# zhazorken/beom

Measured on AMD Instinct MI355X. Metric: cell-layer updates/s, higher is better.
Workload: dtype f64

## Files before the change

### beom_amd/csrc/beom_dev.h

```cpp
#pragma once
#include <hip/hip_runtime.h>
#include <stdint.h>

#include "../../include/beom_hip.h"

struct DevView {
    int ndeg, nlay, lm, mm, nsal, variant;
    int mm_glob;
    long long n1;
    int L, M, xper, yper;
    int P;
    long long ncell;
    int embedded;
    const int32_t *pk_of;
    const unsigned char *reg4;
    int reg_nx;
    const unsigned char *ngt;
    int ngt_nx;
    int joff, Mg, slab;
    int nstrip, jlo0, jhi0, jlo1, jhi1;
    const int32_t *neig, *subc;
    const double *mk_u, *mk_v, *mk_n, *mkpe, *mkpi, *fcor, *h_th, *h_to;
    const double *nudg, *fnud, *hdot, *tide, *bodf, *taus;
    double *hlay, *u, *v, *h_u, *h_v;
    double *rs[2];
    double *dmx[4], *dmy[4];
    double *u_alt, *v_alt, *hu_alt, *hv_alt;
    double *v_cc, *v_ll, *tt3d, *tb3d, *tu3d;
    double *mont, *rvor, *pvor, *dive, *d2hx, *d2hy;
    double *pcd, *qlr;
    int keep_diag;
    int keep_visc;
    int zero_visc;
    int lean_d2h;
    double *delu, *delv, *uu4, *vv4; double svis;
    const int32_t *woff;
    const int32_t *segm; int nseg;
    double *pi_s, *pi_rhs, *pi_prev;
    const double *Ow, *Os, *Osum_;
    const int32_t *sor_order, *sor_dstart;
    const int32_t *lid_rhs_start, *lid_rhs_ent;
    int sor_ndiag;
    double dl, dt, grav, rho0, beta, epsi, gamm, del1, del2, hmin, hsal, bvis, dvis, bdrg, tdrg,
        qdrg, hsbl, hbbl, uadv, ocrp, rgld, invf, w_ti;
    double rhon[BEOM_MAX_LAYERS];
    double i_dl, i_gr, i_ns, i_r0, i_r1, i_rn[BEOM_MAX_LAYERS];
    int has_hdot, has_tide, has_bodf, has_nudg, has_stress, has_wind, has_hto;
    int vel_targets_zero;
    const double *fnud_vel;
    int stress_fold, has_bot, has_top;
    const double *taus_cells;
    double rho_top, rho_bot;
    double *mo0, *mo1, *mo2;
};

struct TileMap {
    int tr0a, ntra, tr0b, ntrb, total, gx, rpx, tpx, nt, xlast, nlast, rim_first, by_tiles;
    __host__ __device__ __forceinline__ TileMap(const DevView &d, int TX, int TY) {
        gx = (d.L + TX - 1) / TX;
        tr0a = 0; ntra = 0; tr0b = 0; ntrb = 0;
        if (d.jhi0 >= d.jlo0) { tr0a = (d.jlo0 - 1) / TY; ntra = (d.jhi0 - 1) / TY - tr0a + 1; }
        if (d.nstrip > 1 && d.jhi1 >= d.jlo1) { tr0b = (d.jlo1 - 1) / TY; ntrb = (d.jhi1 - 1) / TY - tr0b + 1; }
        total = ntra + ntrb;
        nt = total * gx;
        rpx = (total + 7) / 8;
        rim_first = nt <= 4096;
        by_tiles = !rim_first && (rpx * 8 - total) * 100 > 3 * total;
        tpx = by_tiles ? (nt + 7) / 8 : rpx * gx;
        xlast = total > 0 ? (total - 1) / rpx : 0;
        nlast = total - xlast * rpx;
    }
    __host__ unsigned blocks() const { return (unsigned)(8 * tpx); }
    __device__ __forceinline__ bool locate(int b, int &ty, int &ch) const {
        const int xcd = b & 7, k = b >> 3;
        int vt;
        if (by_tiles) {
            const int v = xcd * tpx + k;
            if (v >= nt) return false;
            vt = v / gx; ch = v - vt * gx;
        } else {
            int rib = k / gx;
            const int c = k - rib * gx;
            ch = c;
            if (rim_first) {
                ch = c == 0 ? 0 : (c == 1 ? gx - 1 : c - 1);
                if (xcd == xlast && rib < nlast) rib = nlast - 1 - rib;
            }
            vt = xcd * rpx + rib;
            if (rib >= rpx || vt >= total) return false;
        }
        ty = vt < ntra ? tr0a + vt : tr0b + (vt - ntra);
        return true;
    }
};
__host__ __device__ __forceinline__ bool row_selected(const DevView &d, int j) {
    return (j >= d.jlo0 && j <= d.jhi0) || (d.nstrip > 1 && j >= d.jlo1 && j <= d.jhi1);
}
__device__ __forceinline__ bool tile_regular(const DevView &d, int x0, int y0, int ny) {
    if (!d.embedded) return true;
    const int tx = (x0 - 1) >> 6, t4 = (y0 - 1) >> 2;
    if (tx < 0 || tx >= d.reg_nx || t4 < 0 || (t4 + (ny >> 2) - 1) * 4 >= d.M) return false;
    bool r = d.reg4[(long long)t4 * d.reg_nx + tx] != 0;
    if (ny > 4) r = r && d.reg4[(long long)(t4 + 1) * d.reg_nx + tx] != 0;
    return r;
}
__device__ __forceinline__ bool slot_is_cell(const DevView &d, int ip) { return !d.embedded || d.pk_of[ip] != 0; }

__device__ __forceinline__ bool cell_slot(const DevView &d, long long ip) {
    if (ip > d.ncell) return false;
    if (d.P == 0 || ip == 0) return true;
    if (d.embedded) return d.pk_of[ip] != 0;
    return (int)((ip - 1) % d.P) < d.L;
}
__device__ __forceinline__ long long packed_index0(const DevView &d, long long ip) {
    if (d.P == 0) return ip - 1;
    if (d.embedded) return (long long)d.pk_of[ip] - 1;
    const long long r = (ip - 1) / d.P;
    return r * d.L + ((ip - 1) - r * d.P);
}

#define BEOM_BLOCK 256

template <int K> struct NbOff {
    static constexpr int di = (K == 1 || K == 2 || K == 8) ? 1 : ((K == 4 || K == 5 || K == 6) ? -1 : 0);
    static constexpr int dj = (K == 2 || K == 3 || K == 4) ? 1 : ((K == 6 || K == 7 || K == 8) ? -1 : 0);
};

struct CellPackedInt {
    static constexpr bool kLanesAreRowNeighbours = true;
    static constexpr bool kHasIJ = false;
    int ipnt, dN, dS;
    const DevView *dv;
    template <int K> __device__ __forceinline__ int nb() const {
        constexpr int di = NbOff<K>::di, dj = NbOff<K>::dj;
        return ipnt + di + (dj > 0 ? dN : (dj < 0 ? -dS : 0));
    }
// ... 134 lines not shown
```

### beom_amd/csrc/beom_engine.hip

```cpp
#include <hip/hip_runtime.h>

#include <cmath>
#include <cstdarg>
#include <cstdio>
#include <cstdlib>
#include <cstring>
#include <algorithm>
#include <string>
#include <type_traits>
#include <utility>
#include <vector>

#include "beom_dev.h"
#include "beom_kernels.h"
#include "beom_integrals.h"
#include "beom_series.h"
#include "beom_tracers.h"
#include "beom_tracers_lim.h"
#include "beom_floats.h"
#include "beom_moments.h"
#include "beom_tracer_moments.h"
#include "beom_dense_host.h"
#include "beom_plan.h"

// ... 39 lines not shown
        hipEvent_t a; (void)hipEventCreate(&a); (void)hipEventRecord(a, st); ev.push_back(a); cls.push_back(c);
    }
    void end() { if (!open) return; hipEvent_t b; (void)hipEventCreate(&b); (void)hipEventRecord(b, st); ev.push_back(b); open = false; }
};

struct AccumKind {
    int n1, n2, nsq;
    bool per_tracer;
    const char *bad_args, *no_tracer, *none, *no_sq;
};
constexpr AccumKind kFieldMoments{3, 5, 5, false,
    "beom_set_moments: level %d, stride %d (level 0..3, stride >= 1)", nullptr,
    "beom_download_moments: the handle keeps no moments (beom_set_moments)",
    "beom_download_moments: the second moments are kept at level 3, this handle has level %d"};
constexpr AccumKind kTracerMoments{2, 4, 1, true,
    "beom_set_tracer_moments: level %d, stride %d (level 0..3, stride >= 1)",
    "beom_set_tracer_moments: the handle carries no tracer (beom_set_tracers comes first)",
    "beom_download_tracer_moments: the handle keeps no tracer moments (beom_set_tracer_moments)",
    "beom_download_tracer_moments: the second moment is kept at level 3, this handle has level %d"};
struct Accum {
    const AccumKind *kind;
    int level = 0, stride = 1;
    long long count = 0, launches = 0;
    int first = 0, last = 0;
    double *ref[5] = {}, *sum[5] = {}, *sq[5] = {};
    std::vector<void *> allocs;
};
static bool accum_due(const Accum &A, int tstp) { return A.level > 0 && tstp % A.stride == 0; }
static void accum_note_sample(Accum &A, int tstp) {
    if (A.count == 0) A.first = tstp;
    A.last = tstp;
    ++A.count;
    ++A.launches;
}

struct beom_engine {
    beom_params P;
    int device = 0;
    hipStream_t stream = nullptr;
    hipStream_t own_stream = nullptr;
    StepTimer *timer = nullptr;
    DevView d{};
    bool dense = false;
    std::vector<void *> allocs;
    const int32_t *slot_of_dev = nullptr;
    bool embedded = false;
    void *stage = nullptr;
    size_t stage_bytes = 0;
    dim3 grid_cells0, grid_cells_layers_flat;
    bool wind = false, bot = false, top = false;
    bool fold_stress = true, fold_static_ok = false;
    bool up_tt = false, up_tb = false, up_tu = false;
    bool last_folded = false;
    bool last_uv_fused = false;
    float *h0r4_dev = nullptr, *out4[3] = {nullptr, nullptr, nullptr};
    float *diag4[3] = {nullptr, nullptr, nullptr};
    double *scan_dev = nullptr;
    int any_u = 0, any_v = 0;
    long long uniform_waves = 0, total_waves = 0;
    bool obc = false;
    bool obc_set = false;
    bool fuse = true;
    bool fuse_uv = true;
    bool lean_visc = true;
    bool visc_all_zero = true;
    bool lean_d2h = true;
    std::vector<int32_t> subc_host, neig_host, dev_index;
    bool lid = false, lid_ready = false;
    int lid_dstep = 2, lid_nring = 0, lid_maxwidth = 1;
    double *lid_ring = nullptr;
    unsigned long long *lid_maxd = nullptr;
    long long lid_sweeps = 0, lid_solves = 0, lid_launches = 0;
    int lid_last = 0;
    int profile_stride = 1;
    bool profile_rotate = false;
    StepPlan split{};
    bool tile4 = false;
    bool mont_history = true;
    bool mont_keep = false;
    int mont_levels_valid = 0;
    bool hist_stale = false;
    bool last_mont_hist = false;
    bool plain_sweeps = true;
    int last_plain = 0;
    double *integ_part = nullptr, *integ_rows = nullptr;
    int integ_count = 0;
    int32_t *integ_cellmap = nullptr;
    int integ_xper = 0, integ_yper = 0;
    int ntrc = 0;
    int trc_scheme = 1;
    double *trc_q = nullptr, *trc_q_alt = nullptr, *trc_rq[2] = {nullptr, nullptr}, *trc_ctrg = nullptr;
    std::vector<void *> trc_allocs;
    long long nflt = 0;
    bool flt_ready = false;
    double *flt_x = nullptr, *flt_y = nullptr, *flt_k1x = nullptr, *flt_k1y = nullptr, *flt_xs = nullptr, *flt_ys = nullptr;
    int32_t *flt_layer = nullptr, *flt_rej = nullptr;
    unsigned long long *flt_first_dry = nullptr;
    double *flt_rec = nullptr;
    int flt_nrec = 0, flt_stride = 1;
    std::vector<int> flt_rec_tstp;
    long long flt_launches = 0;
    bool cellmap_known = false;
    std::vector<void *> flt_allocs;
    bool flt_band = false;
    FloatBand flt_fb{};
    unsigned long long *flt_in_s = nullptr, *flt_in_n = nullptr;
    int flt_xper = 0, flt_yper = 0;
    double flt_fmm = 0.0;
    long long flt_handovers = 0;
    Accum mom{&kFieldMoments};
    bool mom_by_caller = false;
    int last_tstp = 0;
    Accum tmom{&kTracerMoments};
    int ser_level = 0, ser_stride = 1, ser_nrec = 0, ser_jlo = 1, ser_rows = 0;
    bool ser_by_caller = false;
    double *ser_rec = nullptr;
    std::vector<int> ser_tstp;
    std::vector<void *> ser_allocs;
    char last_err[512] = {0};
};
static int hist_sync(beom_engine *E);
static int leave_mont_history(beom_engine *E);

namespace {

template <class T>
int alloc_plain(beom_engine *E, std::vector<void *> &owner, T **p, size_t n, char *errm, int errm_len, bool zero = true) {
    void *q = nullptr;
    HIP_TRY(hipMalloc(&q, n * sizeof(T)));
    owner.push_back(q);
    if (zero) HIP_TRY(hipMemsetAsync(q, 0, n * sizeof(T), E->stream));
    *p = (T *)q;
    return 0;
}
constexpr size_t kLead = 15;
template <class T>
int alloc_aligned(beom_engine *E, std::vector<void *> &owner, T **p, size_t n, char *errm, int errm_len, bool zero = true) {
    const int rc = alloc_plain(E, owner, p, n + kLead + 1, errm, errm_len, zero);
    if (!rc) *p += kLead;
    return rc;
}
void free_list(std::vector<void *> &owner) {
    for (void *p : owner) (void)hipFree(p);
    owner.clear();
}
template <class T>
int dev_alloc(beom_engine *E, T **p, size_t n, char *errm, int errm_len, bool zero = true) {
    return sizeof(T) == 8 ? alloc_aligned(E, E->allocs, p, n, errm, errm_len, zero) : alloc_plain(E, E->allocs, p, n + 1, errm, errm_len, zero);
}
size_t state_cells(const beom_engine *E) { return (size_t)E->d.nlay * (size_t)E->d.n1; }
size_t tracer_cells(const beom_engine *E) { return (size_t)E->ntrc * state_cells(E); }

template <class T, bool REMAP = false>
int slice_to_device(beom_engine *E, T *dev, const T *host, int inner, int K, int m, char *errm, int errm_len) {
    const DevView &d = E->d;
    const size_t n = ((size_t)d.ndeg + 1) * inner * K;
    if (n * sizeof(T) > E->stage_bytes) { set_err(errm, errm_len, "internal: staging buffer too small"); return -11; }
    if (host) HIP_TRY(hipMemcpyAsync(E->stage, host, n * sizeof(T), hipMemcpyHostToDevice, E->stream));
    const long long work = ((long long)d.ndeg + 1) * inner;
    if (E->embedded) {
        const long long all = (d.ncell + 1) * inner;
        hipLaunchKernelGGL((k_fill_sentinel<T>), dim3((unsigned)((all + BEOM_BLOCK - 1) / BEOM_BLOCK)), dim3(BEOM_BLOCK), 0, E->stream,
                           dev, (const T *)E->stage, d.ncell + 1, inner, K, m);
    }
    hipLaunchKernelGGL((k_repack<T, true, REMAP>), dim3((unsigned)((work + BEOM_BLOCK - 1) / BEOM_BLOCK)), dim3(BEOM_BLOCK), 0, E->stream,
                       dev, (T *)E->stage, (long long)d.ndeg, d.L, d.P ? d.P : d.L, inner, K, m, E->slot_of_dev);
    return 0;
}
template <class T>
int slice_to_host(beom_engine *E, const T *dev, T *host, int inner, int K, char *errm, int errm_len) {
    (void)dev;
    const DevView &d = E->d;
    const size_t n = ((size_t)d.ndeg + 1) * inner * K;
    HIP_TRY(hipMemcpyAsync(host, E->stage, n * sizeof(T), hipMemcpyDeviceToHost, E->stream));
    HIP_TRY(hipStreamSynchronize(E->stream));
    return 0;
}
template <class T>
void slice_gather(beom_engine *E, const T *dev, int inner, int K, int m) {
    const DevView &d = E->d;
    const long long work = ((long long)d.ndeg + 1) * inner;
    hipLaunchKernelGGL((k_repack<T, false, false>), dim3((unsigned)((work + BEOM_BLOCK - 1) / BEOM_BLOCK)), dim3(BEOM_BLOCK), 0, E->stream,
                       const_cast<T *>(dev), (T *)E->stage, (long long)d.ndeg, d.L, d.P ? d.P : d.L, inner, K, m, E->slot_of_dev);
}

template <class T, bool REMAP = false>
int dev_upload(beom_engine *E, const T **dst, const T *src, size_t outer, int inner, char *errm, int errm_len) {
    const DevView &d = E->d;
    T *q = nullptr;
    int rc = dev_alloc(E, &q, outer * (size_t)d.n1 * inner, errm, errm_len, true);
    if (rc) return rc;
    const size_t n1h = (size_t)d.ndeg + 1;
    if (src)
        for (size_t o = 0; o < outer; ++o)
            if ((rc = slice_to_device<T, REMAP>(E, q + o * (size_t)d.n1 * inner, src + o * n1h * inner, inner, 1, 0, errm, errm_len))) return rc;
    *dst = q;
    return 0;
}

bool any_nonzero(const double *a, size_t n) {
    if (!a) return false;
    for (size_t i = 0; i < n; ++i)
        if (a[i] != 0.0) return true;
    return false;
}

int check_create_args(const beom_params *prm, const beom_handle *out, int device, const beom_dense::Grid &g,
                      const beom_statics &st, char *errm, int errm_len) {
    if (!prm || !out) { set_err(errm, errm_len, "beom_create: null argument"); return -1; }
    if (prm->abi_version != BEOM_ABI_VERSION) { set_err(errm, errm_len, "beom_create: ABI version mismatch (%d vs %d)", prm->abi_version, BEOM_ABI_VERSION); return -2; }
    if (prm->nlay < 1 || prm->nlay > BEOM_MAX_LAYERS || prm->ndeg < 1 || prm->lm < 1 || prm->mm < 1) { set_err(errm, errm_len, "beom_create: bad sizes"); return -3; }
    if (prm->rgld > 0.5 && (prm->variant == 1 || prm->slab_mm > 0 || prm->ocrp < 0.5)) {
        set_err(errm, errm_len, "beom_create: rgld = 1 (rigid lid, private_mod.f95:1705-1838) needs variant 0, ocrp = 1 and a whole frame (no bands)");
        return -5;
    }
    if (prm->variant == 1 && prm->nlay < 3) { set_err(errm, errm_len, "beom_create: variant 1 (private_mod3d.f95) needs nlay >= 3"); return -7; }
    if (!g.neig || !g.subc || !g.mk_u || !g.mk_v || !g.mk_n || !g.mkpe || !g.mkpi || !st.fcor || !st.h_th || !st.nudg || !st.fnud) { set_err(errm, errm_len, "beom_create: null static array"); return -1; }
    int ndev = 0;
    HIP_TRY(hipGetDeviceCount(&ndev));
    if (ndev <= 0 || device < 0 || device >= ndev) { set_err(errm, errm_len, "beom_create: no usable HIP device (%d visible, asked for %d); there is no CPU fallback", ndev, device); return -8; }
    HIP_TRY(hipSetDevice(device));
    if (prm->slab_mm > 0 && (prm->slab_row0 < 0 || prm->slab_row0 + prm->mm + 1 > prm->slab_mm + 1)) { set_err(errm, errm_len, "beom_create: slab rows outside the global frame"); return -3; }
    return 0;
}

void fill_view(DevView &d, const beom_params &prm, const beom_statics &st) {
    const size_t n1h = (size_t)prm.ndeg + 1, nl = (size_t)prm.nlay;
    d.ndeg = prm.ndeg; d.nlay = prm.nlay; d.lm = prm.lm; d.mm = prm.mm; d.nsal = prm.nsal;
    d.variant = prm.variant; d.n1 = (long long)n1h; d.ncell = prm.ndeg;
    d.L = prm.lm + 1; d.M = prm.mm + 1;
    d.dl = prm.dl; d.dt = prm.dt; d.grav = prm.grav; d.rho0 = prm.rho0; d.beta = prm.beta;
    d.epsi = prm.epsi; d.gamm = prm.gamm; d.del1 = prm.del1; d.del2 = prm.del2; d.hmin = prm.hmin;
    d.hsal = prm.hsal; d.bvis = prm.bvis; d.dvis = prm.dvis; d.bdrg = prm.bdrg; d.tdrg = prm.tdrg;
    d.qdrg = prm.qdrg; d.hsbl = prm.hsbl; d.hbbl = prm.hbbl; d.uadv = prm.uadv; d.ocrp = prm.ocrp;
    d.rgld = prm.rgld; d.invf = prm.invf; d.w_ti = prm.w_ti; d.svis = prm.svis;
    d.mm_glob = prm.slab_mm > 0 ? prm.slab_mm : prm.mm;
    for (int i = 0; i < BEOM_MAX_LAYERS; ++i) d.rhon[i] = prm.rhon[i];
    d.i_dl = 1.0 / prm.dl;
    d.i_gr = 1.0 / prm.grav;
    d.i_ns = 1.0 / (double)(prm.nsal - 1);
    d.i_r0 = 1.0 / prm.rho0;
    d.i_r1 = 1.0 / prm.rhon[0];
    for (int i = 0; i < prm.nlay; ++i) d.i_rn[i] = 1.0 / prm.rhon[i];
    d.nstrip = 1; d.jlo0 = 1; d.jhi0 = d.M; d.jlo1 = 1; d.jhi1 = 0;
    d.slab = prm.slab_mm > 0 ? 1 : 0;
    d.joff = d.slab ? prm.slab_row0 : 0;
    d.Mg = d.slab ? prm.slab_mm + 1 : d.M;
    d.has_hdot = any_nonzero(st.hdot, nl * n1h);
    d.has_tide = any_nonzero(st.tide, 6 * n1h);
    d.has_bodf = any_nonzero(st.bodf, 2 * nl);
    d.has_nudg = any_nonzero(st.nudg, 3 * n1h);
    d.has_hto = any_nonzero(st.h_to, n1h);
    d.vel_targets_zero = beom_dense::vel_targets_zero(st.fnud, n1h, nl);
    d.rho_top = prm.rhon[0]; d.rho_bot = prm.rhon[nl - 1];
}

void choose_paths(beom_engine *E, const beom_dense::Grid &g, const beom_statics &st) {
    const beom_params &prm = E->P;
    DevView &d = E->d;
    const size_t n1h = (size_t)prm.ndeg + 1, nl = (size_t)prm.nlay;
    for (size_t i = 0; i < n1h; ++i) { if (g.mk_u[i] > 0.5) E->any_u = 1; if (g.mk_v[i] > 0.5) E->any_v = 1; }
    E->tile4 = E->dense && (long long)((d.L + 63) / 64) * ((d.M + 7) / 8) <= 5000;
    if (getenv("BEOM_TILE4")) E->tile4 = E->dense && atoi(getenv("BEOM_TILE4")) != 0;
    if (E->lid) E->fuse = E->fuse_uv = false;
    if (st.taus) for (size_t i = 0; i < 2 * n1h; ++i) if (std::fabs(st.taus[i]) > 1.e-7) { E->wind = true; break; }
    E->bot = prm.bdrg > 1.e-7;
    E->top = prm.tdrg > 1.e-7;
    d.has_wind = E->wind; d.has_bot = E->bot; d.has_top = E->top;
    d.has_stress = E->wind || E->bot || E->top;
    bool neg0 = false;
    if (st.bodf) for (size_t i = 0; i < 2 * nl; ++i) if (st.bodf[i] == 0.0 && std::signbit(st.bodf[i])) neg0 = true;
    E->fold_static_ok = E->dense && prm.ocrp < 0.5 && !E->lid && d.has_stress && !neg0;
}

template <class T>
int upload_table(beom_engine *E, const T **dst, const std::vector<T> &v, size_t n, bool zero, char *errm, int errm_len) {
    T *q = nullptr;
    const int rc = dev_alloc(E, &q, n, errm, errm_len, zero);
    if (rc) return rc;
    HIP_TRY(hipMemcpyAsync(q, v.data(), v.size() * sizeof(T), hipMemcpyHostToDevice, E->stream));
    HIP_TRY(hipStreamSynchronize(E->stream));
    *dst = q;
    return 0;
}

int upload_statics(beom_engine *E, const beom_dense::Layout &lay, const beom_dense::WaveTable &wt,
                   const std::vector<unsigned char> &ngt, const beom_dense::Grid &g, const beom_statics &st,
                   char *errm, int errm_len) {
    DevView &d = E->d;
    const size_t n1h = (size_t)d.ndeg + 1, nl = (size_t)d.nlay;
    E->stage_bytes = n1h * 32;
    HIP_TRY(hipMalloc(&E->stage, E->stage_bytes));
    int rc;
    if (E->embedded) {
        if ((rc = upload_table(E, &E->slot_of_dev, lay.slot_of, lay.slot_of.size(), false, errm, errm_len))) return rc;
        if ((rc = upload_table(E, &d.pk_of, lay.pk_of, (size_t)d.n1, true, errm, errm_len))) return rc;
        if ((rc = upload_table(E, &d.reg4, lay.reg4, lay.reg4.size(), false, errm, errm_len))) return rc;
    }
    if ((rc = dev_upload<int32_t, true>(E, &d.neig, g.neig, 1, 8, errm, errm_len))) return rc;
    if ((rc = dev_upload(E, &d.subc, g.subc, 2, 1, errm, errm_len))) return rc;
    auto up = [&](const double **dst, const double *src, size_t outer, int inner = 1) {
        if (!rc) rc = dev_upload(E, dst, src, outer, inner, errm, errm_len);
    };
    up(&d.mk_u, g.mk_u, 1); up(&d.mk_v, g.mk_v, 1); up(&d.mk_n, g.mk_n, 1); up(&d.mkpe, g.mkpe, 1); up(&d.mkpi, g.mkpi, 1);
    up(&d.fcor, st.fcor, 1); up(&d.h_th, st.h_th, 1); up(&d.h_to, st.h_to, 1);
    up(&d.nudg, st.nudg, 3); up(&d.fnud, st.fnud, 3 * nl); up(&d.hdot, st.hdot, nl);
    up(&d.tide, st.tide, 3, 2); up(&d.taus, st.taus, 2);
    d.fnud_vel = (rc || d.vel_targets_zero) ? nullptr : d.fnud + d.n1 * (long long)d.nlay;
    std::vector<double> tc(2 * n1h, 0.0);
    if (st.taus) { std::memcpy(tc.data(), st.taus, 2 * n1h * sizeof(double)); tc[0] = 0.0; tc[n1h] = 0.0; }
    up(&d.taus_cells, tc.data(), 2);
    if (rc) return rc;
    double *q = nullptr;
    if ((rc = dev_alloc(E, &q, 2 * nl, errm, errm_len, true))) return rc;
    if (st.bodf) HIP_TRY(hipMemcpyAsync(q, st.bodf, 2 * nl * sizeof(double), hipMemcpyHostToDevice, E->stream));
    d.bodf = q;
    if (wt.uniform > 0 && (rc = upload_table(E, &d.woff, wt.woff, wt.woff.size(), false, errm, errm_len))) return rc;
    if (!ngt.empty()) {
        if ((rc = upload_table(E, &d.ngt, ngt, ngt.size(), false, errm, errm_len))) return rc;
        d.ngt_nx = (d.L + 63) / 64;
    }
    return 0;
}

int alloc_state(beom_engine *E, char *errm, int errm_len) {
    DevView &d = E->d;
    const size_t n = (size_t)d.nlay * (size_t)d.n1;
    int rc = 0;
    auto al = [&](std::initializer_list<double **> arrays, size_t len) {
        for (double **a : arrays) if (!rc) rc = dev_alloc(E, a, len, errm, errm_len);
    };
    al({&d.hlay, &d.u, &d.v, &d.h_u, &d.h_v, &d.rs[0], &d.rs[1], &d.dmx[0], &d.dmx[1], &d.dmx[2], &d.dmy[0], &d.dmy[1], &d.dmy[2]}, n);
    if (E->dense) al({&d.dmx[3], &d.dmy[3], &d.u_alt, &d.v_alt, &d.hu_alt, &d.hv_alt}, n);
    al({&d.v_cc, &d.v_ll}, n);
    al({&d.tt3d, &d.tb3d, &d.tu3d}, 2 * n);
    al({&d.pcd, &d.qlr, &d.mont, &d.rvor, &d.pvor, &d.dive, &d.d2hx, &d.d2hy}, n);
    E->mont_keep = E->dense && !E->lid && !d.slab && E->P.g_fb != 0.0 && d.nlay <= 8 && !(E->P.svis > 0.0);
    if (E->mont_keep) al({&d.mo0, &d.mo1, &d.mo2}, n);
    if (E->P.svis > 0.0) al({&d.delu, &d.delv, &d.uu4, &d.vv4}, n);
    if (E->lid) al({&d.pi_s, &d.pi_rhs, &d.pi_prev}, (size_t)d.n1);
    if (rc) return rc;
    if (E->P.bvis != 0.0) {
        std::vector<double> b(n, E->P.bvis);
        HIP_TRY(hipMemcpyAsync(d.v_cc, b.data(), b.size() * sizeof(double), hipMemcpyHostToDevice, E->stream));
        HIP_TRY(hipMemcpyAsync(d.v_ll, b.data(), b.size() * sizeof(double), hipMemcpyHostToDevice, E->stream));
        HIP_TRY(hipStreamSynchronize(E->stream));
    }
    return 0;
}

int setup(beom_engine *E, const beom_dense::Grid &g, const beom_statics &st, char *errm, int errm_len) {
    const beom_params &prm = E->P;
    DevView &d = E->d;
    HIP_TRY(hipStreamCreateWithFlags(&E->own_stream, hipStreamNonBlocking));
    E->stream = E->own_stream;
    fill_view(d, prm, st);
    beom_dense::Layout lay = beom_dense::plan_layout(prm, d.L, d.M, d.joff, d.Mg, d.slab, g);
    E->dense = lay.dense; E->embedded = lay.embedded;
    d.xper = lay.xper; d.yper = lay.yper; d.embedded = lay.embedded ? 1 : 0; d.reg_nx = lay.reg_nx;
    E->dev_index = std::move(lay.dev_index);
    E->lid = prm.rgld > 0.5;
    if (E->lid) {
        const size_t n1h = (size_t)prm.ndeg + 1;
        E->subc_host.assign(g.subc, g.subc + 2 * n1h);
        E->neig_host.assign(g.neig, g.neig + 8 * n1h);
    }
    if (E->dense) {
        d.P = lay.P;
        d.ncell = (long long)d.P * d.M;
        d.n1 = (d.ncell + 1 + 15) / 16 * 16;
    }
    beom_dense::WaveTable wt;
    if (!E->dense) wt = beom_dense::plan_wave_table(prm.ndeg, g);
    E->uniform_waves = wt.uniform; E->total_waves = wt.total;
    const std::vector<unsigned char> ngt = E->dense && d.has_nudg ? beom_dense::plan_nudging_tiles(lay, d.L, d.M, prm.ndeg, st.nudg)
                                                                  : std::vector<unsigned char>();
    int rc;
    if ((rc = upload_statics(E, lay, wt, ngt, g, st, errm, errm_len))) return rc;
    choose_paths(E, g, st);
    if ((rc = alloc_state(E, errm, errm_len))) return rc;
    const unsigned gx = (unsigned)((d.ncell + BEOM_BLOCK - 1) / BEOM_BLOCK);
    const unsigned gx0 = (unsigned)((d.ncell + 1 + BEOM_BLOCK - 1) / BEOM_BLOCK);
    E->grid_cells_layers_flat = dim3(gx, (unsigned)prm.nlay, 1);
    E->grid_cells0 = dim3(gx0, 1, 1);
    HIP_TRY(hipStreamSynchronize(E->stream));
    return 0;
}

}

extern "C" {

int beom_abi_version(void) { return BEOM_ABI_VERSION; }

int beom_device_count(char *errm, int errm_len) {
    int n = 0;
    HIP_TRY(hipGetDeviceCount(&n));
    return n;
}

int beom_device_pci_bus_id(int device, char *out, int out_len) {
    if (!out || out_len < 16) return -1;
    return hipDeviceGetPCIBusId(out, out_len, device) == hipSuccess ? 0 : -9;
}

int beom_create(const beom_params *prm, int device, const int32_t *neig, const int32_t *subc,
                const double *mk_u, const double *mk_v, const double *mk_n, const double *mkpe,
                const double *mkpi, const double *fcor, const double *h_th, const double *h_to,
                const double *nudg, const double *fnud, const double *hdot, const double *tide,
                const double *bodf, const double *taus, beom_handle *out, char *errm, int errm_len) {
    const beom_dense::Grid g{neig, subc, mk_u, mk_v, mk_n, mkpe, mkpi};
    const beom_statics st{fcor, h_th, h_to, nudg, fnud, hdot, tide, bodf, taus};
    int rc = check_create_args(prm, out, device, g, st, errm, errm_len);
    if (rc) return rc;
    beom_engine *E = new beom_engine();
    E->P = *prm;
    E->device = device;
    if ((rc = setup(E, g, st, errm, errm_len))) {
        beom_destroy(E);
        return rc;
    }
    *out = E;
    return 0;
}

int beom_destroy(beom_handle E) {
    if (!E) return 0;
    (void)hipSetDevice(E->device);
    if (E->stream) (void)hipStreamSynchronize(E->stream);
    for (std::vector<void *> *l : {&E->allocs, &E->trc_allocs, &E->flt_allocs, &E->mom.allocs, &E->tmom.allocs, &E->ser_allocs}) free_list(*l);
    if (E->stage) (void)hipFree(E->stage);
    if (E->timer) { for (hipEvent_t ev : E->timer->ev) (void)hipEventDestroy(ev); delete E->timer; }
    if (E->own_stream) (void)hipStreamDestroy(E->own_stream);
    delete E;
    return 0;
}

static int copy_in(beom_engine *E, double *dst, const double *src, size_t outer, char *errm, int errm_len) {
    if (!src) return 0;
    const size_t n1h = (size_t)E->d.ndeg + 1;
    for (size_t o = 0; o < outer; ++o) {
        const int rc = slice_to_device<double>(E, dst + o * (size_t)E->d.n1, src + o * n1h, 1, 1, 0, errm, errm_len);
        if (rc) return rc;
    }
    return 0;
}
static int copy_out(beom_engine *E, double *dst, const double *src, size_t outer, char *errm, int errm_len) {
    if (!dst) return 0;
    const size_t n1h = (size_t)E->d.ndeg + 1;
    for (size_t o = 0; o < outer; ++o) {
        slice_gather<double>(E, src + o * (size_t)E->d.n1, 1, 1, 0);
        const int rc = slice_to_host<double>(E, src, dst + o * n1h, 1, 1, errm, errm_len);
        if (rc) return rc;
    }
    return 0;
}

static int hist_in(beom_engine *E, double *const *dev, int K, const double *src, char *errm, int errm_len, int outer = 0) {
    if (!src) return 0;
    const size_t n1h = (size_t)E->d.ndeg + 1;
    if (!outer) outer = E->d.nlay;
    for (int l = 0; l < outer; ++l)
        for (int m = 0; m < K; ++m) {
            const int rc = slice_to_device<double>(E, dev[m] + (size_t)l * E->d.n1, m == 0 ? src + (size_t)l * n1h * K : nullptr, 1, K, m,
                                                   errm, errm_len);
            if (rc) return rc;
        }
    return 0;
}
static int hist_out(beom_engine *E, double *const *dev, int K, double *dst, char *errm, int errm_len, int outer = 0) {
    if (!dst) return 0;
    const size_t n1h = (size_t)E->d.ndeg + 1;
    if (!outer) outer = E->d.nlay;
    for (int l = 0; l < outer; ++l) {
        for (int m = 0; m < K; ++m) slice_gather<double>(E, dev[m] + (size_t)l * E->d.n1, 1, K, m);
        const int rc = slice_to_host<double>(E, dev[0], dst + (size_t)l * n1h * K, 1, K, errm, errm_len);
        if (rc) return rc;
    }
    return 0;
}

int beom_upload_state(beom_handle E, const double *hlay, const double *u, const double *v,
                      const double *h_u, const double *h_v, const double *rs_h, const double *dmdx,
                      const double *dmdy, const double *v_cc, const double *v_ll, const double *tt3d,
                      const double *tb3d, const double *tu3d, char *errm, int errm_len) {
    if (!E) { set_err(errm, errm_len, "null handle"); return -1; }
    HIP_TRY(hipSetDevice(E->device));
    DevView &d = E->d;
    const size_t nl = (size_t)d.nlay, n = ((size_t)d.ndeg + 1) * nl;
    int rc;
    if ((rc = leave_mont_history(E))) { set_err(errm, errm_len, "beom_upload_state: the history arrays could not be brought up to date"); return rc; }
    if ((rc = copy_in(E, d.hlay, hlay, nl, errm, errm_len))) return rc;
    if ((rc = copy_in(E, d.u, u, nl, errm, errm_len))) return rc;
    if ((rc = copy_in(E, d.v, v, nl, errm, errm_len))) return rc;
    if ((rc = copy_in(E, d.h_u, h_u, nl, errm, errm_len))) return rc;
    if ((rc = copy_in(E, d.h_v, h_v, nl, errm, errm_len))) return rc;
    if ((rc = copy_in(E, d.v_cc, v_cc, nl, errm, errm_len))) return rc;
    if ((rc = copy_in(E, d.v_ll, v_ll, nl, errm, errm_len))) return rc;
    if ((rc = copy_in(E, d.tt3d, tt3d, 2 * nl, errm, errm_len))) return rc;
    if ((rc = copy_in(E, d.tb3d, tb3d, 2 * nl, errm, errm_len))) return rc;
    if ((rc = copy_in(E, d.tu3d, tu3d, 2 * nl, errm, errm_len))) return rc;
    if ((rc = hist_in(E, d.rs, 2, rs_h, errm, errm_len))) return rc;
    if ((rc = hist_in(E, d.dmx, 3, dmdx, errm, errm_len))) return rc;
    if ((rc = hist_in(E, d.dmy, 3, dmdy, errm, errm_len))) return rc;
    if (any_nonzero(tt3d, 2 * n)) E->up_tt = true;
    if (any_nonzero(tb3d, 2 * n)) E->up_tb = true;
    if (any_nonzero(tu3d, 2 * n)) E->up_tu = true;
    if (E->up_tt || E->up_tb || E->up_tu) d.has_stress = 1;
    for (const double *a : {v_cc, v_ll})
        if (a) for (size_t i = 0; i < n && E->visc_all_zero; ++i) { uint64_t b; memcpy(&b, &a[i], 8); if (b != 0) E->visc_all_zero = false; }
    HIP_TRY(hipStreamSynchronize(E->stream));
    HIP_TRY(hipGetLastError());
    return 0;
}

int beom_download_state(beom_handle E, double *hlay, double *u, double *v, double *h_u, double *h_v,
                        double *rs_h, double *dmdx, double *dmdy, double *v_cc, double *v_ll,
                        double *tt3d, double *tb3d, double *tu3d, char *errm, int errm_len) {
    if (!E) { set_err(errm, errm_len, "null handle"); return -1; }
    HIP_TRY(hipSetDevice(E->device));
    DevView &d = E->d;
    const size_t nl = (size_t)d.nlay;
    int rc;
    if ((rc = hist_sync(E))) { set_err(errm, errm_len, "beom_download_state: the history arrays could not be brought up to date"); return rc; }
    if ((rc = copy_out(E, hlay, d.hlay, nl, errm, errm_len))) return rc;
    if ((rc = copy_out(E, u, d.u, nl, errm, errm_len))) return rc;
    if ((rc = copy_out(E, v, d.v, nl, errm, errm_len))) return rc;
    if ((rc = copy_out(E, h_u, d.h_u, nl, errm, errm_len))) return rc;
    if ((rc = copy_out(E, h_v, d.h_v, nl, errm, errm_len))) return rc;
    if ((rc = copy_out(E, v_cc, d.v_cc, nl, errm, errm_len))) return rc;
    if ((rc = copy_out(E, v_ll, d.v_ll, nl, errm, errm_len))) return rc;
    if ((rc = copy_out(E, tt3d, d.tt3d, 2 * nl, errm, errm_len))) return rc;
    if ((rc = copy_out(E, tb3d, d.tb3d, 2 * nl, errm, errm_len))) return rc;
    if ((rc = copy_out(E, tu3d, d.tu3d, 2 * nl, errm, errm_len))) return rc;
    if ((rc = hist_out(E, d.rs, 2, rs_h, errm, errm_len))) return rc;
    if ((rc = hist_out(E, d.dmx, 3, dmdx, errm, errm_len))) return rc;
    if ((rc = hist_out(E, d.dmy, 3, dmdy, errm, errm_len))) return rc;
    HIP_TRY(hipStreamSynchronize(E->stream));
    HIP_TRY(hipGetLastError());
    return 0;
}

int beom_download_scratch(beom_handle E, double *mont, double *rvor, double *pvor, double *dive,
                          double *d2hx, double *d2hy, char *errm, int errm_len) {
    if (!E) { set_err(errm, errm_len, "null handle"); return -1; }
    HIP_TRY(hipSetDevice(E->device));
    DevView &d = E->d;
    const size_t nl = (size_t)d.nlay;
    int rc;
    if ((rc = copy_out(E, mont, d.mont, nl, errm, errm_len))) return rc;
    if ((rc = copy_out(E, rvor, d.rvor, nl, errm, errm_len))) return rc;
    if ((rc = copy_out(E, pvor, d.pvor, nl, errm, errm_len))) return rc;
    if ((rc = copy_out(E, dive, d.dive, nl, errm, errm_len))) return rc;
    if ((rc = copy_out(E, d2hx, d.d2hx, nl, errm, errm_len))) return rc;
    if ((rc = copy_out(E, d2hy, d.d2hy, nl, errm, errm_len))) return rc;
    HIP_TRY(hipStreamSynchronize(E->stream));
    return 0;
}

int beom_set_rigid_lid(beom_handle E, const double *Ow, const double *Os, const double *Osum_, const double *pi_s,
                       char *errm, int errm_len) {
    if (!E) { set_err(errm, errm_len, "null handle"); return -1; }
    if (!E->lid) { set_err(errm, errm_len, "beom_set_rigid_lid: the handle was created with rgld = 0"); return -5; }
    HIP_TRY(hipSetDevice(E->device));
    DevView &d = E->d;
    int rc;
    if (!E->lid_ready) {
        if (!Ow || !Os || !Osum_) { set_err(errm, errm_len, "beom_set_rigid_lid: the operators Ow, Os, Osum_ are needed on the first call"); return -1; }
        if ((long long)d.n1 >= (1ll << 29)) { set_err(errm, errm_len, "beom_set_rigid_lid: frame too large for the lid's tables"); return -3; }
        const beom_dense::LidPlan lp = beom_dense::plan_lid(d.ndeg, d.lm, d.mm_glob, d.n1, E->subc_host, E->neig_host, E->dev_index);
        if ((rc = dev_upload(E, &d.Ow, Ow, 1, 1, errm, errm_len))) return rc;
        if ((rc = dev_upload(E, &d.Os, Os, 1, 1, errm, errm_len))) return rc;
        if ((rc = dev_upload(E, &d.Osum_, Osum_, 1, 1, errm, errm_len))) return rc;
        if ((rc = upload_table(E, &d.sor_order, lp.order, lp.order.size(), false, errm, errm_len))) return rc;
        if ((rc = upload_table(E, &d.sor_dstart, lp.start, lp.start.size(), false, errm, errm_len))) return rc;
        d.sor_ndiag = (int)lp.start.size() - 1;
        E->lid_dstep = lp.dstep;
        E->lid_maxwidth = lp.maxwidth;
        E->lid_nring = (int)std::max<long long>(17, std::min<long long>(kLidBatch, (6ll << 30) / ((long long)d.n1 * 8))) + 1;
        if ((rc = dev_alloc(E, &E->lid_ring, (size_t)E->lid_nring * d.n1, errm, errm_len, true))) return rc;
        if ((rc = dev_alloc(E, &E->lid_maxd, (size_t)kLidBatch, errm, errm_len, true))) return rc;
        if ((rc = upload_table(E, &d.lid_rhs_start, lp.rhs_start, lp.rhs_start.size(), false, errm, errm_len))) return rc;
        if ((rc = upload_table(E, &d.lid_rhs_ent, lp.rhs_ent, lp.rhs_ent.size(), false, errm, errm_len))) return rc;
        E->lid_ready = true;
    }
    if (pi_s && (rc = slice_to_device<double>(E, d.pi_s, pi_s, 1, 1, 0, errm, errm_len))) return rc;
    HIP_TRY(hipStreamSynchronize(E->stream));
    HIP_TRY(hipGetLastError());
    return 0;
}

int beom_download_pressure(beom_handle E, double *pi_s, char *errm, int errm_len) {
    if (!E) { set_err(errm, errm_len, "null handle"); return -1; }
    if (!E->lid) { set_err(errm, errm_len, "beom_download_pressure: the handle was created with rgld = 0"); return -5; }
    HIP_TRY(hipSetDevice(E->device));
    const int rc = copy_out(E, pi_s, E->d.pi_s, 1, errm, errm_len);
    if (rc) return rc;
    HIP_TRY(hipGetLastError());
    return 0;
}

int beom_sync(beom_handle E, char *errm, int errm_len) {
    if (!E) { set_err(errm, errm_len, "null handle"); return -1; }
    HIP_TRY(hipSetDevice(E->device));
    HIP_TRY(hipStreamSynchronize(E->stream));
    HIP_TRY(hipGetLastError());
    return 0;
}

}

static inline void rot2(double *(&a)[2]) { double *t = a[0]; a[0] = a[1]; a[1] = t; }
static inline void rot3(double *(&a)[4]) { double *t = a[0]; a[0] = a[1]; a[1] = a[2]; a[2] = t; }
static inline void rot4(double *(&a)[4]) { double *t = a[0]; a[0] = a[1]; a[1] = a[2]; a[2] = a[3]; a[3] = t; }
static inline void swp(double *&a, double *&b) { double *t = a; a = b; b = t; }

static void rotate_mont(beom_engine *E) {
    if (!E->mont_keep) return;
    DevView &d = E->d;
    double *t = d.mo0; d.mo0 = d.mo1; d.mo1 = d.mo2; d.mo2 = d.mont; d.mont = t;
}
static int hist_sync(beom_engine *E) {
    if (!E->hist_stale) return 0;
    if (hipSetDevice(E->device) != hipSuccess) return -9;
    hipLaunchKernelGGL(k_hist_from_mont, CellDense::grid(E->d, E->d.nlay), dim3(BEOM_BLOCK), 0, E->stream, E->d);
    E->hist_stale = false;
    return hipGetLastError() == hipSuccess ? 0 : -10;
}
static int leave_mont_history(beom_engine *E) {
    const int rc = hist_sync(E);
    E->mont_levels_valid = 0;
    return rc;
}

#define LAUNCH_CTX(KERNEL_G, KERNEL_D, nz, ...)                                                            \
    do {                                                                                                  \
        if (E->dense) hipLaunchKernelGGL(KERNEL_D, CellDense::grid(E->d, (nz)), dim3(BEOM_BLOCK), 0, E->stream, __VA_ARGS__); \
        else hipLaunchKernelGGL(KERNEL_G, CellGather::grid(E->d, (nz)), dim3(BEOM_BLOCK), 0, E->stream, __VA_ARGS__);         \
    } while (0)

template <class F>
static void pick(F &&f) { f(); }
template <class F, class... R>
static void pick(F &&f, bool b, R... rest) {
    if (b) pick([&](auto... c) { f(std::true_type{}, c...); }, rest...);
    else pick([&](auto... c) { f(std::false_type{}, c...); }, rest...);
}
template <int FROM, int TO, class F>
static void pick_int(int v, F &&f) {
    if (FROM == TO || v == FROM) f(std::integral_constant<int, FROM>{});
    else if constexpr (FROM != TO) pick_int<FROM + (TO > FROM ? 1 : -1), TO>(v, f);
}

static void launch_rebuild(beom_engine *E) {
    LAUNCH_CTX(k_rebuild_fluxes<CellGather>, k_rebuild_fluxes<CellDense>, E->d.nlay, E->d);
}
static int forcing(const DevView &d) { return d.has_nudg ? (d.has_tide ? 2 : 1) : 0; }
static void launch_h(beom_engine *E, double gene, double ramp, double ctim, bool rotate = true) {
    int nz = (E->d.variant == 1) ? 1 : E->d.nlay;
    if (E->d.has_nudg) nz = 1;
    pick_int<2, 0>(forcing(E->d), [&](auto fo) { LAUNCH_CTX((k_update_h<CellGather, fo>), (k_update_h<CellDense, fo>), nz, E->d, gene, ramp, ctim, 0); });
    if (rotate) rot2(E->d.rs);
}
static void launch_tracers(beom_engine *E, double gene, double ramp, double ctim) {
    TrcView tv{E->ntrc, E->trc_ctrg ? 1 : 0, E->trc_q, E->trc_q_alt, E->trc_rq[0], E->trc_rq[1], E->trc_ctrg};
    const int nz = E->d.nlay;
    if (E->trc_scheme == 2) pick_int<2, 0>(forcing(E->d), [&](auto fo) {
        if (!E->dense) hipLaunchKernelGGL((k_tracers_lim<CellGather, fo>), CellGather::grid(E->d, nz), dim3(BEOM_BLOCK), 0, E->stream, E->d, tv, gene, ramp, ctim);
        else if (E->tile4) hipLaunchKernelGGL((k_tracers_lim<TrcTiled<1>, fo>), tracers_lim_grid<1>(E->d), dim3(BEOM_BLOCK), 0, E->stream, E->d, tv, gene, ramp, ctim);
        else hipLaunchKernelGGL((k_tracers_lim<TrcTiled<2>, fo>), tracers_lim_grid<2>(E->d), dim3(BEOM_BLOCK), 0, E->stream, E->d, tv, gene, ramp, ctim);
    });
    else pick_int<2, 0>(forcing(E->d), [&](auto fo) { LAUNCH_CTX((k_tracers<CellGather, fo>), (k_tracers<CellDense, fo>), nz, E->d, tv, gene, ramp, ctim); });
    swp(E->trc_q, E->trc_q_alt);
    rot2(E->trc_rq);
}
static FloatView float_view(const beom_engine *E, double *rec) {
    const DevView &d = E->d;
    return FloatView{E->nflt, E->flt_x, E->flt_y, E->flt_layer, E->flt_rej, E->flt_k1x, E->flt_k1y, E->flt_xs, E->flt_ys,
                     E->integ_cellmap, d.dt * d.i_dl, (double)d.lm, (double)d.mm, E->integ_xper, E->integ_yper, rec};
}
static void launch_floats(beom_engine *E, int mode, double *rec) {
    const DevView &d = E->d;
    FloatView f = float_view(E, rec);
    if (E->flt_band) {
        f.fmm = E->flt_fmm; f.xper = E->flt_xper; f.yper = E->flt_yper; f.cellmap = nullptr;
        const dim3 g((unsigned)((E->nflt + BEOM_BLOCK - 1) / BEOM_BLOCK)), b(BEOM_BLOCK);
        pick_int<1, 3>(mode, [&](auto m) { hipLaunchKernelGGL(k_floats_band<m>, g, b, 0, E->stream, d, f, E->flt_fb); });
        ++E->flt_launches;
        return;
    }
    const dim3 g((unsigned)((E->nflt + BEOM_BLOCK - 1) / BEOM_BLOCK)), b(BEOM_BLOCK);
    pick_int<1, 3>(mode, [&](auto m) {
        if (E->dense) hipLaunchKernelGGL((k_floats<CellDense, m>), g, b, 0, E->stream, d, f);
        else hipLaunchKernelGGL((k_floats<CellGather, m>), g, b, 0, E->stream, d, f);
    });
    ++E->flt_launches;
}
static void launch_floats_after(beom_engine *E, int tstp, bool then_stage1) {
    double *rec = nullptr;
    if (E->flt_nrec > 0 && tstp % E->flt_stride == 0 && (int)E->flt_rec_tstp.size() < E->flt_nrec) {
        rec = E->flt_rec + 3 * (size_t)E->nflt * E->flt_rec_tstp.size();
        E->flt_rec_tstp.push_back(tstp);
    }
    launch_floats(E, then_stage1 ? 3 : 2, rec);
}
static void launch_moments(beom_engine *E, int tstp) {
    const DevView &d = E->d;
    double *const *r = E->mom.ref, *const *s = E->mom.sum, *const *q = E->mom.sq;
    const MomentView m{(long long)d.nlay * d.n1, d.hlay, d.u, d.v, d.h_u, d.h_v, r[0], r[1], r[2], r[3], r[4],
                       s[0], s[1], s[2], s[3], s[4], q[0], q[1], q[2], q[3], q[4]};
    const long long pairs = (m.n - 1) / 2;
    const dim3 g((unsigned)std::max<long long>(1, std::min<long long>((pairs + BEOM_BLOCK - 1) / BEOM_BLOCK, 2048))), b(BEOM_BLOCK);
    pick_int<1, 3>(E->mom.level, [&](auto lv) {
        pick([&](auto first) { hipLaunchKernelGGL((k_moments<lv, first>), g, b, 0, E->stream, m); }, E->mom.count == 0);
    });
    accum_note_sample(E->mom, tstp);
}
static void launch_tracer_moments(beom_engine *E, int tstp) {
    double *const *r = E->tmom.ref, *const *s = E->tmom.sum;
    const TrcMomentView m{E->ntrc, E->trc_q, r[0], r[1], r[2], r[3], s[0], s[1], s[2], s[3], E->tmom.sq[0]};
    const int nz = E->d.nlay;
    pick_int<1, 3>(E->tmom.level, [&](auto lv) {
        pick([&](auto first) { LAUNCH_CTX((k_tracer_moments<CellGather, lv, first>), (k_tracer_moments<CellDense, lv, first>), nz, E->d, m); },
             E->tmom.count == 0);
    });
    accum_note_sample(E->tmom, tstp);
}
static bool series_due(const beom_engine *E, int tstp) {
    return E->ser_level > 0 && tstp % E->ser_stride == 0 && (int)E->ser_tstp.size() < E->ser_nrec;
}
static void launch_series(beom_engine *E, int tstp) {
    const DevView &d = E->d;
    const int count = (E->ser_level >= 2 ? 6 : 4) * d.nlay + 1, nch = (d.L + 63) / 64;
    int nchp2 = 1, width = 1;
    while (nchp2 < nch) nchp2 <<= 1;
    while (width < d.L && width < 64) width <<= 1;
    double *rec = E->ser_rec + E->ser_tstp.size() * (size_t)E->ser_rows * count;
    const dim3 g((unsigned)nch, (unsigned)((E->ser_rows + BEOM_TILE_Y - 1) / BEOM_TILE_Y), 1), b(BEOM_BLOCK);
    const int32_t *map = E->dense ? nullptr : E->integ_cellmap;
    auto go = [&](auto kern) { hipLaunchKernelGGL(kern, g, b, 0, E->stream, d, E->ser_jlo, E->ser_rows, width, E->integ_xper, E->integ_yper, map, E->integ_part); };
    if (E->ser_level == 1) { if (E->dense) go(k_integral_rows<true>); else go(k_integral_rows<false>); }
    else if (E->dense) go(k_series_rows<true>); else go(k_series_rows<false>);
    hipLaunchKernelGGL(k_integral_chunks, dim3((unsigned)E->ser_rows), dim3(64), 0, E->stream,
                       (const double *)E->integ_part, rec, count, nch, nchp2);
    E->ser_tstp.push_back(tstp);
}
static void launch_mont(beom_engine *E, int ilay) {
    if (ilay == 0 && E->d.nlay <= 8) {
        if (E->dense) pick_int<1, 8>(E->d.nlay, [&](auto n) { hipLaunchKernelGGL((k_update_mont_all<CellDense, n>), CellDense::grid(E->d, 1), dim3(BEOM_BLOCK), 0, E->stream, E->d); });
        else pick_int<1, 8>(E->d.nlay, [&](auto n) { hipLaunchKernelGGL((k_update_mont_all<CellGather, n>), CellGather::grid(E->d, 1), dim3(BEOM_BLOCK), 0, E->stream, E->d); });
        return;
    }
    const int nz = ilay ? 1 : E->d.nlay;
    LAUNCH_CTX(k_update_mont<CellGather>, k_update_mont<CellDense>, nz, E->d, ilay);
}
static bool biharm_tiled(const beom_engine *E) { return E->dense && E->P.svis > 0.0; }
static void launch_visc(beom_engine *E, int ilay) {
    const int nz = ilay ? 1 : E->d.nlay;
    LAUNCH_CTX(k_update_visc<CellGather>, k_update_visc<CellDense>, nz, E->d, ilay);
    if (E->d.svis > 0.0 && biharm_tiled(E) && ilay == 0) {
        if (E->tile4) hipLaunchKernelGGL(k_biharm_tiled<1>, biharm_tiled_grid<1>(E->d), dim3(BEOM_BLOCK), 0, E->stream, E->d);
        else hipLaunchKernelGGL(k_biharm_tiled<2>, biharm_tiled_grid<2>(E->d), dim3(BEOM_BLOCK), 0, E->stream, E->d);
    } else if (E->d.svis > 0.0) {
        const dim3 g = ilay ? E->grid_cells0 : E->grid_cells_layers_flat;
        hipLaunchKernelGGL(k_biharm_lap, g, dim3(BEOM_BLOCK), 0, E->stream, E->d, ilay);
        hipLaunchKernelGGL(k_biharm_flux, g, dim3(BEOM_BLOCK), 0, E->stream, E->d, ilay);
    }
}
template <bool XDIR>
static void launch_uv(beom_engine *E, int ilay, double gene, double ramp, double ctim, bool prod = false) {
    const int nz = ilay ? 1 : E->d.nlay;
    const int copy_hist = ilay ? 1 : 0;
    if (prod) hipLaunchKernelGGL((k_update_uv<CellDense, XDIR, true>), CellDense::grid(E->d, nz), dim3(BEOM_BLOCK), 0, E->stream, E->d, ilay, gene, ramp, ctim, copy_hist);
    else LAUNCH_CTX((k_update_uv<CellGather, XDIR>), (k_update_uv<CellDense, XDIR>), nz, E->d, ilay, gene, ramp, ctim, copy_hist);
    if (!copy_hist) { if (XDIR) rot3(E->d.dmx); else rot3(E->d.dmy); }
}
template <int Q>
static void raw_mont_visc(beom_engine *E, const StepPlan &p) {
    const dim3 g = mont_visc_grid<Q>(E->d), b(BEOM_BLOCK);
    pick_int<1, 8>(E->d.nlay, [&](auto n) {
        pick([&](auto pl, auto le) { hipLaunchKernelGGL((k_mont_visc<Q, n, le, pl>), g, b, 0, E->stream, E->d); }, p.mont.plain, p.leith);
    });
}
template <int Q>
static void raw_uv_fused(beom_engine *E, const StepPlan &p) {
    const dim3 g = uv_fused_grid<Q>(E->d), b(TileGeom<Q>::BLOCK);
    pick([&](auto fx, auto pl, auto hm, auto sf, auto zv, auto pr) {
        if constexpr (!beom_plan::uv_form_exists(sf, pr, zv, hm, pl)) { fprintf(stderr, "beom: the plan names a form of the u+v sweep that does not exist\n"); std::abort(); }
        else if constexpr (sf) hipLaunchKernelGGL((k_uv_fused_sf<Q, fx, pr, zv>), g, b, 0, E->stream, E->d, p.gene, p.ramp, p.ctim);
        else hipLaunchKernelGGL((k_uv_fused<Q, fx, pr, zv, hm, pl>), g, b, 0, E->stream, E->d, p.gene, p.ramp, p.ctim);
    }, p.uv.first_x, p.uv.plain, p.uv.hm, p.stress_fold, p.uv.zv, p.uv.prod);
}
static void launch_mont_visc(beom_engine *E, const StepPlan &p) { if (E->tile4) raw_mont_visc<1>(E, p); else raw_mont_visc<2>(E, p); }
static void uv_fused_swap(beom_engine *E, bool first_x, bool hm = false) {
    DevView &d = E->d;
    swp(d.u, d.u_alt); swp(d.v, d.v_alt);
    if (first_x) swp(d.h_v, d.hv_alt); else swp(d.h_u, d.hu_alt);
    if (hm) { E->hist_stale = true; return; }
    if (first_x) { rot4(d.dmx); rot3(d.dmy); }
    else         { rot4(d.dmy); rot3(d.dmx); }
}
static void launch_uv_fused(beom_engine *E, const StepPlan &p, bool swap = true) {
    if (E->tile4) raw_uv_fused<1>(E, p); else raw_uv_fused<2>(E, p);
    if (swap) uv_fused_swap(E, p.uv.first_x, p.uv.hm);
}
static void launch_lid_fluxes(beom_engine *E, bool first3) {
    if (first3) { launch_rebuild(E); return; }
    const dim3 g((unsigned)((E->d.ncell + BEOM_BLOCK - 1) / BEOM_BLOCK), (unsigned)E->d.nlay, 1);
    hipLaunchKernelGGL(k_rgld_upstream_fluxes, g, dim3(BEOM_BLOCK), 0, E->stream, E->d);
}
static void launch_lid_h_epilogue(beom_engine *E) {
    hipLaunchKernelGGL(k_rgld_h_epilogue, dim3((unsigned)((E->d.ncell + BEOM_BLOCK - 1) / BEOM_BLOCK)), dim3(BEOM_BLOCK), 0, E->stream, E->d);
}
static int lid_solve(beom_engine *E) {
    DevView &d = E->d;
    const int maxiters = 1000;
    const double pi_tol = 1.e-5;
    const int R = E->lid_nring, D = E->lid_dstep, nlev = d.sor_ndiag;
    const size_t bytes = (size_t)d.n1 * sizeof(double);
    if (hipMemcpyAsync(E->lid_ring, d.pi_s, bytes, hipMemcpyDeviceToDevice, E->stream) != hipSuccess) return -1;
    int s0 = 1, batch = std::min(R - 1, std::max(16, E->lid_last * 5 / 4 + 8)), chosen = 0;
    unsigned long long maxd[kLidBatch];
    while (!chosen) {
        const int nb = std::min(batch, maxiters - s0 + 1);
        if (hipMemsetAsync(E->lid_maxd, 0, nb * sizeof(unsigned long long), E->stream) != hipSuccess) return -1;
        const dim3 g((unsigned)((E->lid_maxwidth + BEOM_BLOCK - 1) / BEOM_BLOCK), (unsigned)nb, 1);
        const int tend = nlev - 1 + (nb - 1) * D;
        for (int t = 0; t <= tend; ++t)
            hipLaunchKernelGGL(k_rgld_gs_front, g, dim3(BEOM_BLOCK), 0, E->stream, d, E->lid_ring, R, s0, t, D, E->lid_maxd);
        E->lid_launches += tend + 1;
        if (hipMemcpyAsync(maxd, E->lid_maxd, nb * sizeof(unsigned long long), hipMemcpyDeviceToHost, E->stream) != hipSuccess) return -1;
        if (hipStreamSynchronize(E->stream) != hipSuccess) return -1;
        for (int b = 0; b < nb && !chosen; ++b) {
            double m; memcpy(&m, &maxd[b], sizeof(double));
            if (!(m > pi_tol) || s0 + b == maxiters) chosen = s0 + b;
        }
        s0 += nb;
        batch = R - 1;
    }
    E->lid_sweeps += chosen; ++E->lid_solves; E->lid_last = chosen;
    if (hipMemcpyAsync(d.pi_s, E->lid_ring + (size_t)(chosen % R) * d.n1, bytes, hipMemcpyDeviceToDevice, E->stream) != hipSuccess) return -1;
    return 0;
}
static void launch_lid_pressure(beom_engine *E) {
    const dim3 g1((unsigned)((E->d.ncell + BEOM_BLOCK - 1) / BEOM_BLOCK)), g((unsigned)((E->d.ncell + BEOM_BLOCK - 1) / BEOM_BLOCK), (unsigned)E->d.nlay, 1);
    hipLaunchKernelGGL(k_rgld_rhs, g1, dim3(BEOM_BLOCK), 0, E->stream, E->d);
    if (lid_solve(E)) snprintf(E->last_err, sizeof(E->last_err), "the lid's pressure iteration failed: %s", hipGetErrorString(hipGetLastError()));
    hipLaunchKernelGGL(k_rgld_correct, g, dim3(BEOM_BLOCK), 0, E->stream, E->d);
}
static void launch_stress(beom_engine *E) {
    if (!(E->wind || E->bot || E->top)) return;
    const dim3 g((unsigned)((E->d.ncell + BEOM_BLOCK - 1) / BEOM_BLOCK));
    hipLaunchKernelGGL(k_stress, g, dim3(BEOM_BLOCK), 0, E->stream, E->d, (int)E->wind, (int)E->bot, (int)E->top);
}

extern "C" {

#define NEED(E) do { if (!(E)) return -1; if (hipSetDevice((E)->device) != hipSuccess) return -9; } while (0)

#define LAUNCHED() (hipGetLastError() == hipSuccess ? 0 : -10)
#define NEED_ARRAYS(E) do { NEED(E); if (leave_mont_history(E)) return -10; } while (0)
int beom_update_h(beom_handle E, double gene, double ramp, double ctim) { NEED_ARRAYS(E); launch_h(E, gene, ramp, ctim); return LAUNCHED(); }
int beom_update_tracers(beom_handle E, double gene, double ramp, double ctim) { NEED_ARRAYS(E); if (E->ntrc < 1) return -3; launch_tracers(E, gene, ramp, ctim); return LAUNCHED(); }
int beom_update_mont_rvor_pvor_dive_kine(beom_handle E, int ilay) { NEED_ARRAYS(E); if (ilay < 0 || ilay > E->d.nlay) return -3; launch_mont(E, ilay); return LAUNCHED(); }
int beom_update_viscosity(beom_handle E, int ilay) { NEED_ARRAYS(E); if (ilay < 0 || ilay > E->d.nlay) return -3; launch_visc(E, ilay); return LAUNCHED(); }
int beom_update_u(beom_handle E, int ilay, double gene, double ramp, double ctim) { NEED_ARRAYS(E); if (ilay < 0 || ilay > E->d.nlay) return -3; launch_uv<true>(E, ilay, gene, ramp, ctim); return LAUNCHED(); }
int beom_update_v(beom_handle E, int ilay, double gene, double ramp, double ctim) { NEED_ARRAYS(E); if (ilay < 0 || ilay > E->d.nlay) return -3; launch_uv<false>(E, ilay, gene, ramp, ctim); return LAUNCHED(); }
int beom_rebuild_fluxes(beom_handle E) { NEED_ARRAYS(E); launch_rebuild(E); return LAUNCHED(); }
int beom_distribute_stress(beom_handle E) { NEED_ARRAYS(E); launch_stress(E); return LAUNCHED(); }
#undef NEED_ARRAYS
#undef LAUNCHED

}

static StepFacts facts_of(const beom_engine *E) {
    const DevView &d = E->d;
    StepFacts f;
    f.dense = E->dense; f.nlay = d.nlay; f.lid = E->lid;
    f.svis = E->P.svis; f.dvis = E->P.dvis; f.bvis = E->P.bvis; f.g_fb = E->P.g_fb; f.ocrp = d.ocrp;
    f.has_nudg = d.has_nudg; f.has_tide = d.has_tide; f.has_stress = d.has_stress; f.has_bodf = d.has_bodf; f.has_hto = d.has_hto;
    f.wind = E->wind; f.bot = E->bot; f.top = E->top; f.up_tt = E->up_tt; f.up_tb = E->up_tb; f.up_tu = E->up_tu;
    f.fold_static_ok = E->fold_static_ok; f.visc_all_zero = E->visc_all_zero; f.mont_keep = E->mont_keep;
    f.fuse = E->fuse; f.fuse_uv = E->fuse_uv; f.fold_stress = E->fold_stress; f.lean_d2h = E->lean_d2h; f.lean_visc = E->lean_visc;
    f.mont_history = E->mont_history; f.plain_sweeps = E->plain_sweeps; f.keep_diag = d.keep_diag != 0;
    f.mont_levels_valid = E->mont_levels_valid;
    return f;
}
static void apply_plan(beom_engine *E, const StepPlan &p) {
    DevView &d = E->d;
    d.lean_d2h = p.mont.lean_d2h; d.keep_visc = p.mont.keep_visc; d.zero_visc = p.mont.zero_visc; d.stress_fold = p.stress_fold;
    E->last_folded = p.stress_fold;
    E->last_uv_fused = p.uv.fused_uv;
    E->last_mont_hist = p.uv.hm;
    E->last_plain = (p.uv.plain ? 1 : 0) | (p.mont.plain ? 2 : 0);
}

static StepTimer *step_timer(beom_engine *E, int tstp) {
    StepTimer *T = (E->timer && tstp % E->timer->stride == 0) ? E->timer : nullptr;
    if (T) { T->st = E->stream; T->step(tstp); }
    return T;
}
template <class F>
static void timed(StepTimer *T, int c, F &&f) {
    if (T) T->begin(c);
    f();
    if (T) T->end();
}

static void step_front(beom_engine *E, const StepPlan &p, StepTimer *T) {
    if (p.launch_stress) launch_stress(E);
    if (E->lid) launch_lid_fluxes(E, p.first3);
    else if (p.rebuild) launch_rebuild(E);
    if (E->ntrc > 0) timed(T, 7, [&] { launch_tracers(E, p.gene, p.ramp, p.ctim); });
    timed(T, 0, [&] {
        launch_h(E, p.gene, p.ramp, p.ctim);
        if (E->lid) launch_lid_h_epilogue(E);
    });
    timed(T, p.mont.fused ? 5 : 1, [&] {
        if (p.mont.fused) launch_mont_visc(E, p);
        else launch_mont(E, 0);
    });
    if (p.launch_visc) timed(T, 2, [&] { launch_visc(E, 0); });
}

static void one_step(beom_engine *E, const StepPlan &p, int flt = -1) {
    const int tstp = p.tstp;
    if (flt >= 0 && (flt & 1)) launch_floats(E, 1, nullptr);
    if (p.needs_arrays) (void)hist_sync(E);
    rotate_mont(E);
    StepTimer *T = step_timer(E, tstp);
    apply_plan(E, p);
    step_front(E, p, T);
    if (E->mont_keep) E->mont_levels_valid = std::min(E->mont_levels_valid + 1, 3);
    if (p.uv.fused_uv) timed(T, 6, [&] { launch_uv_fused(E, p); });
    else
        for (const bool x : {p.uv.first_x, !p.uv.first_x})
            timed(T, x ? 3 : 4, [&] {
                if (x) launch_uv<true>(E, 0, p.gene, p.ramp, p.ctim, p.uv.prod);
                else launch_uv<false>(E, 0, p.gene, p.ramp, p.ctim, p.uv.prod);
            });
    if (E->obc) {
        const dim3 g((unsigned)((E->d.nseg + BEOM_BLOCK - 1) / BEOM_BLOCK), (unsigned)E->d.nlay, 1);
        hipLaunchKernelGGL(k_no_gradient_obc, g, dim3(BEOM_BLOCK), 0, E->stream, E->d, 0);
        hipLaunchKernelGGL(k_no_gradient_obc, g, dim3(BEOM_BLOCK), 0, E->stream, E->d, 1);
    }
    if (E->lid) { launch_lid_fluxes(E, p.first3); launch_lid_pressure(E); }
    if (flt >= 0) launch_floats_after(E, tstp, !(flt & 2));
    E->last_tstp = tstp; E->split.tstp = 0;
    if (!E->mom_by_caller && accum_due(E->mom, tstp)) launch_moments(E, tstp);
    if (!E->mom_by_caller && accum_due(E->tmom, tstp)) launch_tracer_moments(E, tstp);
    if (!E->ser_by_caller && series_due(E, tstp)) launch_series(E, tstp);
}

template <bool PACK>
static int rows_copy(beom_handle E, int jlo, int nrows, void *dbuf, int jlo2, void *dbuf2) {
    if (!E || !dbuf || jlo < 1 || nrows < 1 || jlo + nrows - 1 > E->d.M) return -3;
    if (dbuf2 && (jlo2 < 1 || jlo2 + nrows - 1 > E->d.M)) return -3;
    if (hipSetDevice(E->device) != hipSuccess) return -9;
    const long long total = 5ll * E->d.nlay * nrows * E->d.L;
    hipLaunchKernelGGL((k_rows_copy<PACK>), dim3((unsigned)((total + BEOM_BLOCK - 1) / BEOM_BLOCK), dbuf2 ? 2u : 1u), dim3(BEOM_BLOCK),
                       0, E->stream, E->d, jlo, nrows, (double *)dbuf, jlo2, (double *)dbuf2);
    if (E->ntrc > 0) {
        const long long tq = (long long)E->ntrc * E->d.nlay * nrows * E->d.L;
        hipLaunchKernelGGL((k_rows_copy_q<PACK>), dim3((unsigned)((tq + BEOM_BLOCK - 1) / BEOM_BLOCK), dbuf2 ? 2u : 1u), dim3(BEOM_BLOCK),
                           0, E->stream, E->d, E->trc_q, E->ntrc, jlo, nrows, (double *)dbuf + total, jlo2, dbuf2 ? (double *)dbuf2 + total : nullptr);
    }
    return hipGetLastError() == hipSuccess ? 0 : -10;
}
static bool recorder_holds(int tstp_first, int nsteps, int stride, size_t held, int nrec, char *errm, int errm_len, const char *fmt) {
    long long due = 0;
    for (int tstp = tstp_first; tstp < tstp_first + nsteps; ++tstp) due += tstp % stride == 0;
    if ((long long)held + due <= nrec) return true;
    set_err(errm, errm_len, fmt, tstp_first, tstp_first + nsteps - 1, due, stride, (long long)held, nrec);
    return false;
}
extern "C" {

int beom_step(beom_handle E, int tstp_first, int nsteps, double tres, double dtd8, double dt_r,
              double rsta, int n_3d, char *errm, int errm_len) {
    if (!E) { set_err(errm, errm_len, "null handle"); return -1; }
    if (tstp_first < 1 || nsteps < 0 || n_3d < 1) { set_err(errm, errm_len, "beom_step: bad arguments"); return -3; }
    if (E->P.flag_nudging && E->P.mcbc < 0.5 && !E->obc && !E->obc_set) { set_err(errm, errm_len, "beom_step: mcbc = 0 with nudging needs beom_set_open_boundaries (no_gradient_obc, private_mod.f95:2613-2679)"); return -6; }
    if (E->lid && !E->lid_ready) { set_err(errm, errm_len, "beom_step: rgld = 1 needs beom_set_rigid_lid (the Poisson operators Ow, Os, Osum_ and the lid pressure, private_mod.f95:505-563)"); return -6; }
    const bool flt = E->nflt > 0 && !E->flt_band;
    if (flt && !E->flt_ready) { set_err(errm, errm_len, "beom_step: the handle's %lld floats have no positions yet (beom_upload_floats)", E->nflt); return -3; }
    if (flt && E->flt_nrec > 0 &&
        !recorder_holds(tstp_first, nsteps, E->flt_stride, E->flt_rec_tstp.size(), E->flt_nrec, errm, errm_len,
                        "beom_step: steps %d..%d would write %lld float records (stride %d) but the recorder holds %lld of %d: "
                        "empty it with beom_download_float_track, or take fewer steps per call")) return -3;
    if (E->ser_level > 0 && !E->ser_by_caller &&
        !recorder_holds(tstp_first, nsteps, E->ser_stride, E->ser_tstp.size(), E->ser_nrec, errm, errm_len,
                        "beom_step: steps %d..%d would write %lld records of the series (stride %d) but the recorder holds %lld of %d: "
                        "empty it with beom_download_series, or take fewer steps per call")) return -3;
    HIP_TRY(hipSetDevice(E->device));
    for (int tstp = tstp_first; tstp < tstp_first + nsteps; ++tstp)
        one_step(E, beom_plan::plan_step(facts_of(E), tstp, tres, dtd8, dt_r, rsta, n_3d),
                 flt ? (tstp == tstp_first ? 1 : 0) | (tstp == tstp_first + nsteps - 1 ? 2 : 0) : -1);
    HIP_TRY(hipGetLastError());
    return 0;
}

int beom_profile_start(beom_handle E) {
    if (!E) return -1;
    if (E->timer) { for (hipEvent_t ev : E->timer->ev) (void)hipEventDestroy(ev); delete E->timer; }
    E->timer = new StepTimer();
    E->timer->st = E->stream;
    E->timer->stride = E->profile_stride;
    E->timer->rotate = E->profile_rotate;
    return 0;
}

int beom_profile_stop(beom_handle E, double *ms, int *launches, char *errm, int errm_len) {
    if (!E || !ms || !launches) { set_err(errm, errm_len, "null argument"); return -1; }
    if (!E->timer) { set_err(errm, errm_len, "beom_profile_stop without beom_profile_start"); return -3; }
    HIP_TRY(hipSetDevice(E->device));
    HIP_TRY(hipStreamSynchronize(E->stream));
    StepTimer &T = *E->timer;
    for (int c = 0; c < 8; ++c) { ms[c] = 0.0; launches[c] = 0; }
    for (size_t k = 0; k < T.cls.size(); ++k) {
        float t = 0.f;
        (void)hipEventElapsedTime(&t, T.ev[2 * k], T.ev[2 * k + 1]);
        ms[T.cls[k]] += (double)t;
        launches[T.cls[k]] += 1;
    }
    for (hipEvent_t ev : T.ev) (void)hipEventDestroy(ev);
    delete E->timer;
    E->timer = nullptr;
    HIP_TRY(hipGetLastError());
    return 0;
}

int beom_profile_steps(beom_handle E, int tstp_first, int nsteps, double tres, double dtd8, double dt_r,
                       double rsta, int n_3d, double *ms, int *launches, char *errm, int errm_len) {
    int rc = beom_profile_start(E);
    if (rc) { set_err(errm, errm_len, "null handle"); return rc; }
    rc = beom_step(E, tstp_first, nsteps, tres, dtd8, dt_r, rsta, n_3d, errm, errm_len);
    if (rc) return rc;
    return beom_profile_stop(E, ms, launches, errm, errm_len);
}

static void set_rows(DevView &d, int n, int lo0, int hi0, int lo1 = 1, int hi1 = 0) {
// ... 147 lines not shown
    if (E->integ_part) {
        HIP_TRY(hipStreamSynchronize(E->stream));
        for (double **p : {&E->integ_part, &E->integ_rows}) {
            E->allocs.erase(std::remove(E->allocs.begin(), E->allocs.end(), (void *)*p), E->allocs.end());
            (void)hipFree(*p);
            *p = nullptr;
        }
        E->integ_count = 0;
    }
    HIP_TRY(hipMalloc((void **)&E->integ_part, (size_t)d.M * nch * count * sizeof(double)));
    E->allocs.push_back(E->integ_part);
    HIP_TRY(hipMalloc((void **)&E->integ_rows, (size_t)d.M * count * sizeof(double)));
    E->allocs.push_back(E->integ_rows);
    E->integ_count = count;
    return 0;
}

int beom_integral_rows(beom_handle E, int jlo, int nrows, double *rows, char *errm, int errm_len) {
    if (!E || !rows) { set_err(errm, errm_len, "beom_integral_rows: null argument"); return -1; }
    DevView &d = E->d;
    if (jlo < 1 || nrows < 1 || jlo + nrows - 1 > d.M) { set_err(errm, errm_len, "beom_integral_rows: rows %d..%d outside 1..%d", jlo, jlo + nrows - 1, d.M); return -3; }
    HIP_TRY(hipSetDevice(E->device));
    const int count = 4 * d.nlay + 1, nch = (d.L + 63) / 64, nchp2 = pow2_ceil(nch);
    const int width = std::min(64, pow2_ceil(d.L));
    if (nchp2 / 64 > kIntegralMaxGroups) { set_err(errm, errm_len, "beom_integral_rows: rows of more than %d columns", 64 * 64 * kIntegralMaxGroups); return -4; }
    if (const int rc = ensure_integ_scratch(E, count, errm, errm_len)) return rc;
    if (const int rc = ensure_cellmap(E, errm, errm_len)) return rc;
    const dim3 g((unsigned)nch, (unsigned)((nrows + BEOM_TILE_Y - 1) / BEOM_TILE_Y), 1), b(BEOM_BLOCK);
    if (E->dense) hipLaunchKernelGGL(k_integral_rows<true>, g, b, 0, E->stream, d, jlo, nrows, width, E->integ_xper, E->integ_yper,
                                     (const int32_t *)nullptr, E->integ_part);
    else hipLaunchKernelGGL(k_integral_rows<false>, g, b, 0, E->stream, d, jlo, nrows, width, E->integ_xper, E->integ_yper,
                            (const int32_t *)E->integ_cellmap, E->integ_part);
    const long long nt = (long long)nrows * count;
    hipLaunchKernelGGL(k_integral_chunks, dim3((unsigned)nrows), dim3(64), 0, E->stream,
                       (const double *)E->integ_part, E->integ_rows, count, nch, nchp2);
    HIP_TRY(hipMemcpyAsync(rows, E->integ_rows, (size_t)nt * sizeof(double), hipMemcpyDeviceToHost, E->stream));
    HIP_TRY(hipStreamSynchronize(E->stream));
    HIP_TRY(hipGetLastError());
    return 0;
}

int beom_integral_combine(const double *rows, int nrows_total, int count, double *out) {
    if (!rows || !out || nrows_total < 1 || count < 1) return -1;
    const int n2 = pow2_ceil(nrows_total);
    std::vector<double> w((size_t)n2);
    for (int k = 0; k < count; ++k) {
        for (int r = 0; r < n2; ++r) w[(size_t)r] = r < nrows_total ? rows[(size_t)r * count + k] : 0.0;
        for (int n = n2; n > 1; n >>= 1)
            for (int m = 0; m < n / 2; ++m) w[(size_t)m] = w[(size_t)(2 * m)] + w[(size_t)(2 * m + 1)];
        out[k] = w[0];
    }
    return 0;
}

int beom_integrals(beom_handle E, double *out, char *errm, int errm_len) {
    if (!E || !out) { set_err(errm, errm_len, "beom_integrals: null argument"); return -1; }
    const int count = 4 * E->d.nlay + 1, M = E->d.M;
    std::vector<double> rows((size_t)M * count);
    const int rc = beom_integral_rows(E, 1, M, rows.data(), errm, errm_len);
    if (rc) return rc;
    return beom_integral_combine(rows.data(), M, count, out);
}

int beom_series_count(int nlay, int level) { return (level >= 2 ? 6 : 4) * nlay + 1; }

static void series_free(beom_engine *E) {
    free_list(E->ser_allocs);
    E->ser_level = 0; E->ser_stride = 1; E->ser_nrec = 0; E->ser_jlo = 1; E->ser_rows = 0; E->ser_by_caller = false;
    E->ser_rec = nullptr;
    E->ser_tstp.clear();
}

static int series_set(beom_engine *E, const char *who, int level, int stride, int nrec, int jlo, int nrows, bool by_caller,
                      char *errm, int errm_len) {
    if (!E) { set_err(errm, errm_len, "null handle"); return -1; }
    if (level < 0 || level > 2 || (level > 0 && (stride < 1 || nrec < 1))) {
        set_err(errm, errm_len, "%s: level %d, stride %d, %d records (level 0..2, stride >= 1, records >= 1)", who, level, stride, nrec);
        return -3;
    }
    const DevView &d = E->d;
    if (level > 0 && (jlo < 1 || nrows < 1 || jlo + nrows - 1 > d.M)) { set_err(errm, errm_len, "%s: rows %d..%d outside 1..%d", who, jlo, jlo + nrows - 1, d.M); return -3; }
    if (level > 0 && pow2_ceil((d.L + 63) / 64) / 64 > kIntegralMaxGroups) { set_err(errm, errm_len, "%s: rows of more than %d columns", who, 64 * 64 * kIntegralMaxGroups); return -4; }
    HIP_TRY(hipSetDevice(E->device));
    HIP_TRY(hipStreamSynchronize(E->stream));
    series_free(E);
    if (level == 0) return 0;
    const int count = beom_series_count(d.nlay, level);
    int rc = ensure_integ_scratch(E, count, errm, errm_len);
    if (!rc) rc = ensure_cellmap(E, errm, errm_len);
    if (!rc) rc = alloc_aligned(E, E->ser_allocs, &E->ser_rec, (size_t)nrec * nrows * count, errm, errm_len);
    if (rc) { series_free(E); return rc; }
    E->ser_level = level; E->ser_stride = stride; E->ser_nrec = nrec; E->ser_jlo = jlo; E->ser_rows = nrows; E->ser_by_caller = by_caller;
    HIP_TRY(hipStreamSynchronize(E->stream));
    return 0;
}

int beom_set_series(beom_handle E, int level, int stride, int nrec, char *errm, int errm_len) {
    return series_set(E, "beom_set_series", level, stride, nrec, 1, E ? E->d.M : 0, false, errm, errm_len);
}

int beom_band_set_series(beom_handle E, int level, int stride, int nrec, int jlo, int nrows, char *errm, int errm_len) {
    return series_set(E, "beom_band_set_series", level, stride, nrec, jlo, nrows, true, errm, errm_len);
}

int beom_sample_series(beom_handle E) {
    if (!E) return -1;
    if (E->ser_level < 1 || (int)E->ser_tstp.size() >= E->ser_nrec) return -3;
    if (hipSetDevice(E->device) != hipSuccess) return -9;
    launch_series(E, E->last_tstp);
    return hipGetLastError() == hipSuccess ? 0 : -10;
}

int beom_download_series(beom_handle E, double *rows, int *tstp, int *count, char *errm, int errm_len) {
    if (!E) { set_err(errm, errm_len, "null handle"); return -1; }
    if (E->ser_level < 1) { set_err(errm, errm_len, "beom_download_series: the handle keeps no series (beom_set_series)"); return -3; }
    HIP_TRY(hipSetDevice(E->device));
    const size_t n = E->ser_tstp.size(), per = (size_t)E->ser_rows * beom_series_count(E->d.nlay, E->ser_level);
    if (rows && n) {
        HIP_TRY(hipMemcpyAsync(rows, E->ser_rec, n * per * sizeof(double), hipMemcpyDeviceToHost, E->stream));
        HIP_TRY(hipStreamSynchronize(E->stream));
        HIP_TRY(hipGetLastError());
    }
    if (tstp) std::copy(E->ser_tstp.begin(), E->ser_tstp.end(), tstp);
    if (count) *count = (int)n;
    E->ser_tstp.clear();
    return 0;
}

static void accum_free(Accum &A);
static void free_tracers(beom_engine *E) {
    free_list(E->trc_allocs);
    E->ntrc = 0;
    E->trc_q = E->trc_q_alt = E->trc_rq[0] = E->trc_rq[1] = E->trc_ctrg = nullptr;
}
int beom_set_tracers(beom_handle E, int ntrc, char *errm, int errm_len) {
    if (!E) { set_err(errm, errm_len, "null handle"); return -1; }
    if (ntrc < 0 || ntrc > BEOM_MAX_TRACERS) { set_err(errm, errm_len, "beom_set_tracers: %d tracers (0..%d)", ntrc, BEOM_MAX_TRACERS); return -3; }
    if (ntrc > 0 && E->P.variant == 1) { set_err(errm, errm_len, "beom_set_tracers: variant 1 changes the thickness in an epilogue (private_mod3d.f95:1635-1683) that the tracer scheme does not follow"); return -6; }
    if (ntrc > 0 && E->lid) { set_err(errm, errm_len, "beom_set_tracers: rgld = 1 changes the thickness in the lid's misfit epilogue (private_mod.f95:1648-1700), which the tracer scheme does not follow"); return -6; }
    HIP_TRY(hipSetDevice(E->device));
    HIP_TRY(hipStreamSynchronize(E->stream));
    if (ntrc != E->ntrc) accum_free(E->tmom);
    free_tracers(E);
    if (ntrc == 0) return 0;
    E->ntrc = ntrc;
    int rc = 0;
    for (double **a : {&E->trc_q, &E->trc_q_alt, &E->trc_rq[0], &E->trc_rq[1]})
        if ((rc = alloc_aligned(E, E->trc_allocs, a, tracer_cells(E), errm, errm_len))) { free_tracers(E); return rc; }
    HIP_TRY(hipStreamSynchronize(E->stream));
    return 0;
}

int beom_set_tracer_scheme(beom_handle E, int scheme, char *errm, int errm_len) {
    if (scheme != 1 && scheme != 2) { set_err(errm, errm_len, "beom_set_tracer_scheme: scheme %d (1 = upstream, 2 = limited)", scheme); return -3; }
    if (!E) { set_err(errm, errm_len, "null handle"); return -1; }
    E->trc_scheme = scheme;
    return 0;
}

int beom_upload_tracers(beom_handle E, const double *q, const double *rq, const double *ctrg, char *errm, int errm_len) {
    if (!E) { set_err(errm, errm_len, "null handle"); return -1; }
    if (E->ntrc < 1) { set_err(errm, errm_len, "beom_upload_tracers: the handle carries no tracer (beom_set_tracers)"); return -3; }
    HIP_TRY(hipSetDevice(E->device));
    const int outer = E->ntrc * E->d.nlay;
    int rc;
    if (ctrg && !E->trc_ctrg && (rc = alloc_aligned(E, E->trc_allocs, &E->trc_ctrg, tracer_cells(E), errm, errm_len))) return rc;
    if ((rc = copy_in(E, E->trc_q, q, (size_t)outer, errm, errm_len))) return rc;
    if ((rc = copy_in(E, E->trc_ctrg, ctrg, (size_t)outer, errm, errm_len))) return rc;
    if ((rc = hist_in(E, E->trc_rq, 2, rq, errm, errm_len, outer))) return rc;
    HIP_TRY(hipStreamSynchronize(E->stream));
    HIP_TRY(hipGetLastError());
    return 0;
}

int beom_download_tracers(beom_handle E, double *q, double *rq, char *errm, int errm_len) {
    if (!E) { set_err(errm, errm_len, "null handle"); return -1; }
    if (E->ntrc < 1) { set_err(errm, errm_len, "beom_download_tracers: the handle carries no tracer (beom_set_tracers)"); return -3; }
    HIP_TRY(hipSetDevice(E->device));
    const int outer = E->ntrc * E->d.nlay;
    int rc;
    if ((rc = copy_out(E, q, E->trc_q, (size_t)outer, errm, errm_len))) return rc;
    if ((rc = hist_out(E, E->trc_rq, 2, rq, errm, errm_len, outer))) return rc;
    HIP_TRY(hipStreamSynchronize(E->stream));
    HIP_TRY(hipGetLastError());
    return 0;
}

static void free_floats(beom_engine *E) {
    free_list(E->flt_allocs);
    E->nflt = 0; E->flt_ready = false; E->flt_nrec = 0; E->flt_stride = 1;
    E->flt_rec_tstp.clear();
    E->flt_x = E->flt_y = E->flt_k1x = E->flt_k1y = E->flt_xs = E->flt_ys = E->flt_rec = nullptr;
    E->flt_layer = E->flt_rej = nullptr;
    E->flt_first_dry = nullptr;
    E->flt_band = false; E->flt_fb = FloatBand{}; E->flt_in_s = E->flt_in_n = nullptr; E->flt_handovers = 0;
}
int beom_set_floats(beom_handle E, int64_t n, int nrec, int stride, char *errm, int errm_len) {
    if (!E) { set_err(errm, errm_len, "null handle"); return -1; }
    if (n < 0 || nrec < 0 || stride < 1) { set_err(errm, errm_len, "beom_set_floats: %lld floats, %d records, stride %d (n >= 0, nrec >= 0, stride >= 1)", (long long)n, nrec, stride); return -3; }
    if (n > 0 && (double)n * 3.0 * (double)std::max(nrec, 1) >= 9.0e15) { set_err(errm, errm_len, "beom_set_floats: %lld floats x %d records is too much", (long long)n, nrec); return -3; }
    if (n > 0 && E->d.slab) {
        set_err(errm, errm_len, "beom_set_floats: this handle holds one band of rows (slab_mm = %d): a float leaves its band, and floats do not "
                "migrate between devices yet; carry them on a single handle of the whole frame", E->P.slab_mm);
        return -6;
    }
    HIP_TRY(hipSetDevice(E->device));
    HIP_TRY(hipStreamSynchronize(E->stream));
    free_floats(E);
    if (n == 0) return 0;
    int rc = ensure_cellmap(E, errm, errm_len);
    if (rc) return rc;
    E->nflt = (long long)n;
    const size_t m = (size_t)n;
    for (double **a : {&E->flt_x, &E->flt_y, &E->flt_k1x, &E->flt_k1y, &E->flt_xs, &E->flt_ys})
        if ((rc = alloc_plain(E, E->flt_allocs, a, m, errm, errm_len))) { free_floats(E); return rc; }
    for (int32_t **a : {&E->flt_layer, &E->flt_rej})
        if ((rc = alloc_plain(E, E->flt_allocs, a, m, errm, errm_len))) { free_floats(E); return rc; }
    if ((rc = alloc_plain(E, E->flt_allocs, &E->flt_first_dry, 1, errm, errm_len))) { free_floats(E); return rc; }
    if (nrec > 0 && (rc = alloc_plain(E, E->flt_allocs, &E->flt_rec, 3 * m * (size_t)nrec, errm, errm_len))) { free_floats(E); return rc; }
    E->flt_nrec = nrec; E->flt_stride = stride;
    HIP_TRY(hipStreamSynchronize(E->stream));
    return 0;
}
// ... 135 lines not shown
    HIP_TRY(hipGetLastError());
    return 0;
}

int beom_band_floats_commit(beom_handle E, const int32_t *layer, char *errm, int errm_len) {
    if (!E || !layer) { set_err(errm, errm_len, "beom_band_floats_commit: null argument"); return -1; }
    if (!E->flt_band) { set_err(errm, errm_len, "beom_band_floats_commit: the handle carries no band floats"); return -3; }
    HIP_TRY(hipSetDevice(E->device));
    const size_t n = (size_t)E->nflt, box = sizeof(unsigned long long) * kFloatRecordWords;
    HIP_TRY(hipMemcpyAsync(E->flt_x, E->flt_xs, n * sizeof(double), hipMemcpyDeviceToDevice, E->stream));
    HIP_TRY(hipMemcpyAsync(E->flt_y, E->flt_ys, n * sizeof(double), hipMemcpyDeviceToDevice, E->stream));
    HIP_TRY(hipMemcpyAsync(E->flt_layer, layer, n * sizeof(int32_t), hipMemcpyHostToDevice, E->stream));
    HIP_TRY(hipMemsetAsync(E->flt_rej, 0, n * sizeof(int32_t), E->stream));
    HIP_TRY(hipMemsetAsync(E->flt_k1x, 0, n * sizeof(double), E->stream));
    HIP_TRY(hipMemsetAsync(E->flt_k1y, 0, n * sizeof(double), E->stream));
    HIP_TRY(hipMemsetAsync(E->flt_fb.stats, 0, 4 * sizeof(unsigned long long), E->stream));
    for (unsigned long long *q : {E->flt_fb.box_s, E->flt_fb.box_n, E->flt_in_s, E->flt_in_n})
        if (q) HIP_TRY(hipMemsetAsync(q, 0, box, E->stream));
    HIP_TRY(hipStreamSynchronize(E->stream));
    E->flt_ready = true;
    return 0;
}

int beom_band_floats_launch(beom_handle E, int mode) {
    if (!E) return -1;
    if (hipSetDevice(E->device) != hipSuccess) return -9;
    if (!E->flt_band || !E->flt_ready || mode < 1 || mode > 3) return -3;
    launch_floats(E, mode, nullptr);
    return hipGetLastError() == hipSuccess ? 0 : -10;
}

int beom_band_floats_boxes(beom_handle E, void **out_s, void **out_n, void **in_s, void **in_n, size_t *bytes) {
    if (!E || !E->flt_band) return -3;
    if (out_s) *out_s = E->flt_fb.box_s;
    if (out_n) *out_n = E->flt_fb.box_n;
    if (in_s) *in_s = E->flt_in_s;
    if (in_n) *in_n = E->flt_in_n;
    if (bytes) *bytes = sizeof(unsigned long long) * kFloatRecordWords * ((size_t)E->flt_fb.capacity + 1);
    return 0;
}

int beom_band_floats_ingest(beom_handle E) {
    if (!E) return -1;
    if (hipSetDevice(E->device) != hipSuccess) return -9;
    if (!E->flt_band || !E->flt_ready) return -3;
    FloatView f = float_view(E, nullptr);
    const dim3 g((unsigned)((E->flt_fb.capacity + BEOM_BLOCK - 1) / BEOM_BLOCK), 2u), b(BEOM_BLOCK);
    hipLaunchKernelGGL(k_floats_ingest, g, b, 0, E->stream, f, E->flt_fb, E->flt_in_s, E->flt_in_n);
    return hipGetLastError() == hipSuccess ? 0 : -10;
}

int beom_band_floats_download(beom_handle E, double *x, double *y, int32_t *layer, int32_t *rejected, unsigned long long *stats3,
                              char *errm, int errm_len) {
    if (!E) { set_err(errm, errm_len, "null handle"); return -1; }
    if (!E->flt_band) { set_err(errm, errm_len, "beom_band_floats_download: the handle carries no band floats"); return -3; }
    HIP_TRY(hipSetDevice(E->device));
    const size_t n = (size_t)E->nflt;
    unsigned long long st[3] = {0, 0, 0};
    if (x) HIP_TRY(hipMemcpyAsync(x, E->flt_x, n * sizeof(double), hipMemcpyDeviceToHost, E->stream));
    if (y) HIP_TRY(hipMemcpyAsync(y, E->flt_y, n * sizeof(double), hipMemcpyDeviceToHost, E->stream));
    if (layer) HIP_TRY(hipMemcpyAsync(layer, E->flt_layer, n * sizeof(int32_t), hipMemcpyDeviceToHost, E->stream));
    if (rejected) HIP_TRY(hipMemcpyAsync(rejected, E->flt_rej, n * sizeof(int32_t), hipMemcpyDeviceToHost, E->stream));
    HIP_TRY(hipMemcpyAsync(st, E->flt_fb.stats, sizeof(st), hipMemcpyDeviceToHost, E->stream));
    HIP_TRY(hipStreamSynchronize(E->stream));
    HIP_TRY(hipGetLastError());
    E->flt_handovers = (long long)st[2];
    if (stats3) for (int q = 0; q < 3; ++q) stats3[q] = st[q];
    return 0;
}

static void accum_free(Accum &A) {
    free_list(A.allocs);
    A.level = 0; A.stride = 1; A.count = 0; A.first = A.last = 0;
    for (int f = 0; f < 5; ++f) A.ref[f] = A.sum[f] = A.sq[f] = nullptr;
}

static int accum_set(beom_engine *E, Accum beom_engine::*which, int level, int stride, char *errm, int errm_len) {
    if (!E) { set_err(errm, errm_len, "null handle"); return -1; }
    Accum &A = E->*which;
    const AccumKind &K = *A.kind;
    if (level < 0 || level > 3 || stride < 1) { set_err(errm, errm_len, K.bad_args, level, stride); return -3; }
    if (K.no_tracer && level > 0 && E->ntrc < 1) { set_err(errm, errm_len, "%s", K.no_tracer); return -3; }
    HIP_TRY(hipSetDevice(E->device));
    HIP_TRY(hipStreamSynchronize(E->stream));
    accum_free(A);
    if (level == 0) return 0;
    int rc = 0;
    const size_t n = K.per_tracer ? tracer_cells(E) : state_cells(E);
    const int nq = level >= 2 ? K.n2 : K.n1;
    for (int f = 0; f < nq && !rc; ++f) {
        rc = alloc_aligned(E, A.allocs, &A.ref[f], n, errm, errm_len);
        if (!rc) rc = alloc_aligned(E, A.allocs, &A.sum[f], n, errm, errm_len);
    }
    for (int m = 0; m < K.nsq && !rc && level >= 3; ++m) rc = alloc_aligned(E, A.allocs, &A.sq[m], n, errm, errm_len);
    if (rc) { accum_free(A); return rc; }
    A.level = level; A.stride = stride;
    HIP_TRY(hipStreamSynchronize(E->stream));
    return 0;
}

static int accum_reset(Accum &A) {
    if (A.level < 1) return -3;
    A.count = 0; A.first = A.last = 0;
    return 0;
}

static int accum_download(beom_engine *E, Accum beom_engine::*which, double *ref, double *sum, double *sq, long long *count,
                          int *tstp_first, int *tstp_last, char *errm, int errm_len) {
    if (!E) { set_err(errm, errm_len, "null handle"); return -1; }
    const Accum &A = E->*which;
    if (A.level < 1) { set_err(errm, errm_len, "%s", A.kind->none); return -3; }
    if (sq && A.level < 3) { set_err(errm, errm_len, A.kind->no_sq, A.level); return -3; }
    HIP_TRY(hipSetDevice(E->device));
    const size_t rows = (size_t)(A.kind->per_tracer ? E->ntrc : 1) * (size_t)E->d.nlay, slab = ((size_t)E->d.ndeg + 1) * rows;
    const int nq = A.level >= 2 ? A.kind->n2 : A.kind->n1, nsq = A.kind->nsq;
    if (count) *count = A.count;
    if (tstp_first) *tstp_first = A.first;
    if (tstp_last) *tstp_last = A.last;
    if (A.count == 0) {
        if (ref) std::fill(ref, ref + nq * slab, 0.0);
        if (sum) std::fill(sum, sum + nq * slab, 0.0);
        if (sq) std::fill(sq, sq + nsq * slab, 0.0);
        return 0;
    }
    int rc;
    for (int f = 0; f < nq; ++f) {
        if (ref && (rc = copy_out(E, ref + f * slab, A.ref[f], rows, errm, errm_len))) return rc;
        if (sum && (rc = copy_out(E, sum + f * slab, A.sum[f], rows, errm, errm_len))) return rc;
    }
    for (int m = 0; m < nsq && sq; ++m)
        if ((rc = copy_out(E, sq + m * slab, A.sq[m], rows, errm, errm_len))) return rc;
    HIP_TRY(hipStreamSynchronize(E->stream));
    HIP_TRY(hipGetLastError());
    return 0;
}

int beom_set_moments(beom_handle E, int level, int stride, char *errm, int errm_len) {
    return accum_set(E, &beom_engine::mom, level, stride, errm, errm_len);
}
int beom_set_tracer_moments(beom_handle E, int level, int stride, char *errm, int errm_len) {
    return accum_set(E, &beom_engine::tmom, level, stride, errm, errm_len);
}

int beom_reset_moments(beom_handle E) { return E ? accum_reset(E->mom) : -1; }
int beom_reset_tracer_moments(beom_handle E) { return E ? accum_reset(E->tmom) : -1; }

static int accum_sample(beom_engine *E, Accum beom_engine::*which, void (*launch)(beom_engine *, int)) {
    if (!E) return -1;
    const Accum &A = E->*which;
    if (A.level < 1 || (A.kind->per_tracer && E->ntrc < 1)) return -3;
    if (hipSetDevice(E->device) != hipSuccess) return -9;
    launch(E, E->last_tstp);
    return hipGetLastError() == hipSuccess ? 0 : -10;
}
int beom_sample_moments(beom_handle E) { return accum_sample(E, &beom_engine::mom, launch_moments); }
int beom_sample_tracer_moments(beom_handle E) { return accum_sample(E, &beom_engine::tmom, launch_tracer_moments); }

int beom_download_moments(beom_handle E, double *ref, double *sum, double *sq, long long *count, int *tstp_first, int *tstp_last,
                          char *errm, int errm_len) {
    return accum_download(E, &beom_engine::mom, ref, sum, sq, count, tstp_first, tstp_last, errm, errm_len);
}
int beom_download_tracer_moments(beom_handle E, double *ref, double *sum, double *sq, long long *count, int *tstp_first, int *tstp_last,
                                 char *errm, int errm_len) {
    return accum_download(E, &beom_engine::tmom, ref, sum, sq, count, tstp_first, tstp_last, errm, errm_len);
}

int beom_set_open_boundaries(beom_handle E, int nseg, const int32_t *segm, char *errm, int errm_len) {
    if (!E || nseg < 0 || (nseg > 0 && !segm)) { set_err(errm, errm_len, "beom_set_open_boundaries: bad arguments"); return -1; }
    HIP_TRY(hipSetDevice(E->device));
    if (nseg == 0) {
        E->d.segm = nullptr; E->d.nseg = 0; E->obc = false; E->obc_set = true;
        return 0;
    }
    auto S = [&](int is, int col) { return segm[(size_t)is + (size_t)nseg * (col - 1)]; };
    for (int pass = 0; pass < 2; ++pass) {
        std::vector<long long> wr, rd;
        for (int is = 0; is < nseg; ++is) {
            const bool ns = S(is, 5) == 1, ew = S(is, 4) == 1;
            const int comp = pass == 0 ? (ns ? 0 : (ew ? 1 : -1)) : (ns ? 1 : (ew ? 0 : -1));
            if (comp < 0) continue;
            const int ip = pass == 0 ? S(is, 10) : S(is, 1), in = pass == 0 ? S(is, 16) : S(is, 13);
            if (ip == -1) continue;
            if (ip < 1 || ip > E->d.ndeg || in < 0 || in > E->d.ndeg) { set_err(errm, errm_len, "beom_set_open_boundaries: index out of range"); return -3; }
            wr.push_back(2ll * ip + comp);
            rd.push_back(2ll * in + comp);
        }
        std::vector<long long> w2 = wr;
        std::sort(w2.begin(), w2.end());
        if (std::adjacent_find(w2.begin(), w2.end()) != w2.end()) { set_err(errm, errm_len, "beom_set_open_boundaries: two segments update the same point (serial order would matter)"); return -7; }
        for (long long r : rd)
            if (std::binary_search(w2.begin(), w2.end(), r)) { set_err(errm, errm_len, "beom_set_open_boundaries: a segment reads a point another segment updates in the same pass (serial order would matter)"); return -7; }
    }
    std::vector<int32_t> sg(segm, segm + (size_t)nseg * 18);
    if (E->embedded) {
        for (int col : {1, 7, 10, 13, 16})
            for (int is = 0; is < nseg; ++is) {
                int32_t &q = sg[(size_t)is + (size_t)nseg * (col - 1)];
                if (q > 0) { if ((size_t)q >= E->dev_index.size()) { set_err(errm, errm_len, "beom_set_open_boundaries: index out of range"); return -3; } q = E->dev_index[(size_t)q]; }
            }
    } else if (E->d.P)
        for (int col : {1, 7, 10, 13, 16})
            for (int is = 0; is < nseg; ++is) {
                int32_t &q = sg[(size_t)is + (size_t)nseg * (col - 1)];
                if (q > 0) q = (int32_t)(1 + (long long)((q - 1) / E->d.L) * E->d.P + (q - 1) % E->d.L);
            }
    int32_t *dev = nullptr;
    HIP_TRY(hipMalloc((void **)&dev, (size_t)nseg * 18 * sizeof(int32_t)));
    E->allocs.push_back(dev);
    HIP_TRY(hipMemcpy(dev, sg.data(), (size_t)nseg * 18 * sizeof(int32_t), hipMemcpyHostToDevice));
    E->d.segm = dev;
    E->d.nseg = nseg;
    E->obc = E->P.flag_nudging && E->P.mcbc < 0.5;
    E->obc_set = true;
    return 0;
}

int beom_info(beom_handle E, const char *what) {
    if (!E || !what) return -1;
    if (!strcmp(what, "stress_folded")) return E->last_folded ? 1 : 0;
    if (!strcmp(what, "tile_rows")) return E->dense ? (E->tile4 ? 4 : 8) : 0;
    if (!strcmp(what, "biharm_tiled")) return biharm_tiled(E) ? 1 : 0;
    if (!strcmp(what, "uv_fused")) return E->last_uv_fused ? 1 : 0;
    if (!strcmp(what, "mont_history")) return E->last_mont_hist ? 1 : 0;
    if (!strcmp(what, "plain_sweeps")) return E->last_plain;
    if (!strcmp(what, "vel_targets_zero")) return E->d.vel_targets_zero;
    if (!strcmp(what, "tracers")) return E->ntrc;
    if (!strcmp(what, "tracer_scheme")) return E->trc_scheme;
    if (!strcmp(what, "floats")) return (int)std::min<long long>(E->nflt, 2000000000ll);
    if (!strcmp(what, "float_records")) return (int)E->flt_rec_tstp.size();
    if (!strcmp(what, "float_launches")) return (int)std::min<long long>(E->flt_launches, 2000000000ll);
    if (!strcmp(what, "float_handovers")) return (int)std::min<long long>(E->flt_handovers, 2000000000ll);
    if (!strcmp(what, "tracer_moments")) return E->tmom.level;
    if (!strcmp(what, "tracer_moment_samples")) return (int)std::min<long long>(E->tmom.count, 2000000000ll);
    if (!strcmp(what, "tracer_moment_launches")) return (int)std::min<long long>(E->tmom.launches, 2000000000ll);
    if (!strcmp(what, "series")) return E->ser_level;
    if (!strcmp(what, "series_records")) return (int)E->ser_tstp.size();
    if (!strcmp(what, "moments")) return E->mom.level;
    if (!strcmp(what, "moment_samples")) return (int)std::min<long long>(E->mom.count, 2000000000ll);
    if (!strcmp(what, "moment_launches")) return (int)std::min<long long>(E->mom.launches, 2000000000ll);
    if (!strcmp(what, "lid_sweeps")) return (int)std::min<long long>(E->lid_sweeps, 2000000000ll);
    if (!strcmp(what, "lid_solves")) return (int)std::min<long long>(E->lid_solves, 2000000000ll);
    if (!strcmp(what, "lid_launches")) return (int)std::min<long long>(E->lid_launches, 2000000000ll);
    if (!strcmp(what, "lid_sweep_distance")) return E->lid_dstep;
    return -3;
}

int beom_set_option(beom_handle E, const char *name, int value) {
    if (!E || !name) return -1;
    if (!strncmp(name, "fuse", 4) && hist_sync(E)) return -10;
    if (!strcmp(name, "fuse")) { E->fuse = value != 0; E->fuse_uv = value != 0; }
    else if (!strcmp(name, "fuse_mont_visc")) E->fuse = value != 0 && !E->lid;
    else if (!strcmp(name, "fuse_uv")) E->fuse_uv = value != 0 && !E->lid;
    else if (!strcmp(name, "keep_diag")) E->d.keep_diag = value != 0;
    else if (!strcmp(name, "fold_stress")) E->fold_stress = value != 0;
    else if (!strcmp(name, "profile_stride")) E->profile_stride = value > 0 ? value : 1;
    else if (!strcmp(name, "profile_rotate")) E->profile_rotate = value != 0;
    else if (!strcmp(name, "lean_d2h")) E->lean_d2h = value != 0;
    else if (!strcmp(name, "lean_visc")) E->lean_visc = value != 0;
    else if (!strcmp(name, "mont_history")) E->mont_history = value != 0;
    else if (!strcmp(name, "plain_sweeps")) E->plain_sweeps = value != 0;
    else if (!strcmp(name, "moments_by_caller")) E->mom_by_caller = value != 0;
    else return -3;
    return 0;
}

int beom_set_stream(beom_handle E, void *hip_stream, int use_own) {
    if (!E) return -1;
    E->stream = use_own ? E->own_stream : (hipStream_t)hip_stream;
    return 0;
}

int beom_is_dense(beom_handle E) { return (E && E->dense) ? (E->embedded ? 2 : 1) : 0; }

int beom_device_field(beom_handle E, const char *name, void **dptr, int64_t *stride_layer,
                      int64_t *stride_row, int64_t *row0_offset) {
    if (!E || !name || !dptr) return -1;
    const DevView &d = E->d;
    double *p = nullptr;
    if (!strcmp(name, "hlay")) p = d.hlay;
    else if (!strcmp(name, "u")) p = d.u;
    else if (!strcmp(name, "v")) p = d.v;
    else if (!strcmp(name, "h_u")) p = d.h_u;
    else if (!strcmp(name, "h_v")) p = d.h_v;
    else return -3;
    *dptr = p;
    if (stride_layer) *stride_layer = d.n1;
    if (stride_row) *stride_row = d.P ? d.P : (E->dense ? d.L : 0);
    if (row0_offset) *row0_offset = 1;
    return 0;
}

}
```

### beom_amd/csrc/beom_kernels.h

```cpp
#pragma once

#define LL(a, ip, il) (a)[(long long)(ip) + d.n1 * (long long)((il) - 1)]
#define FNUD_(ip, il, iv) d.fnud[(long long)(ip) + d.n1 * ((long long)((il) - 1) + (long long)d.nlay * ((iv) - 1))]
#define FNUDV_(ip, il, iv) d.fnud_vel[(long long)(ip) + d.n1 * ((long long)((il) - 1) + (long long)d.nlay * ((iv) - 2))]
#define NUDG_(ip, iv) d.nudg[(long long)(ip) + d.n1 * ((iv) - 1)]
#define TIDE_(m, ip, iv) d.tide[((m) - 1) + 2 * ((long long)(ip) + d.n1 * ((iv) - 1))]
#define T3_(a, ip, id, il) (a)[(long long)(ip) + d.n1 * ((long long)((id) - 1) + 2 * (long long)((il) - 1))]

__device__ __forceinline__ double powi_dev(double x, int n) {
    double r = x;
    for (int q = 1; q < n; ++q) r = r * x;
    return r;
}

template <class C>
__device__ __forceinline__ void body_rebuild_fluxes(const C &c, const DevView &d) {
    const int ipnt = c.ipnt, ilay = blockIdx.y + 1;
    const int c5 = c.template nb<5>(), c7 = c.template nb<7>();
    const double h0 = LL(d.hlay, ipnt, ilay);
    LL(d.h_u, ipnt, ilay) = LL(d.u, ipnt, ilay) * (h0 + LL(d.hlay, c5, ilay)) / (1.0 + c.mk_u());
    LL(d.h_v, ipnt, ilay) = LL(d.v, ipnt, ilay) * (h0 + LL(d.hlay, c7, ilay)) / (1.0 + c.mk_v());
}
template <class CTX>
__global__ __launch_bounds__(BEOM_BLOCK) void k_rebuild_fluxes(DevView d) {
    CTX c;
    if (!c.init(d)) return;
    if (c.wave_is_interior()) body_rebuild_fluxes(c.as_interior(), d);
    else body_rebuild_fluxes(c, d);
}

template <int FORCE, class C>
__device__ __forceinline__ void body_update_h(const C &c, const DevView &d, double gene, double ramp,
                                                         double ctim, int copy_hist) {
    constexpr bool FORCED = FORCE > 0;
    const int ipnt = c.ipnt;
    const int c1 = c.template nb<1>(), c3 = c.template nb<3>();
    const double i_dl = d.i_dl;
    const double mkn = c.mk_n();
    const double ng = FORCED ? nudg_rate<1>(c, d) : 0.0;
    const int ilay_hi = gridDim.y == 1 ? d.nlay : (int)blockIdx.y + 1;
    const int ilay_lo = gridDim.y == 1 ? 1 : (int)blockIdx.y + 1;
    for (int ilay = ilay_hi; ilay >= ilay_lo; --ilay) {
        double hold = LL(d.hlay, ipnt, ilay);
        const bool lazy_hfor = FORCE == 1 && d.variant == 0;
        const double hfor0 = (FORCED && !(lazy_hfor && ng == 0.0)) ? FNUD_(ipnt, ilay, 1) : 0.0;
        const double hu0 = LL(d.h_u, ipnt, ilay);
        double huE;
        if (C::kLanesAreRowNeighbours) {
            huE = __shfl_down(hu0, 1, 64);
            if ((threadIdx.x & 63) == 63) huE = LL(d.h_u, c1, ilay);
        } else {
            huE = LL(d.h_u, c1, ilay);
        }
        double rs_3 = (hu0 - huE) * i_dl
                    + (LL(d.h_v, ipnt, ilay) - LL(d.h_v, c3, ilay)) * i_dl
                    + (d.has_hdot ? LL(d.hdot, ipnt, ilay) : 0.0);
        rs_3 = rs_3 * mkn;
        const double r2 = LL(d.rs[1], ipnt, ilay);
        double rhsi;
        if (gene != 0.0) {
            const double r1 = LL(d.rs[0], ipnt, ilay);
            rhsi = ((1.5 + d.beta) * rs_3 - (0.5 + 2.0 * d.beta) * r2 + d.beta * r1) * d.dt * gene
                 + rs_3 * d.dt * (1.0 - gene);
        } else {
            rhsi = rs_3 * d.dt;
        }
        hold = hold + rhsi;
        double hnew = 0.0 + hold;
        if (FORCED) {
            double hfor = hfor0;
            if (FORCE > 1) {
                const double vecl = (ilay == 1) ? 1.0 : 0.0;
                hfor = hfor + ramp * TIDE_(1, ipnt, 1) * vecl * cos(TIDE_(2, ipnt, 1) - d.w_ti * ctim);
            }
            if (lazy_hfor && ng == 0.0) {
                hnew = hold;
                if (hold == 0.0) hnew = FNUD_(ipnt, ilay, 1) * ng + (1.0 - ng) * hold;
            } else if (d.variant == 0) {
                hnew = hfor * ng + (1.0 - ng) * hold;
            } else {
                const double hfor1 = 0.0, hfor2 = 800.0, hfor3 = 0.0;
                const int isub = c.isub();
                const int half = d.lm / 2;
                const double h3v = (ilay == 3) ? hold : LL(d.hlay, ipnt, 3);
                double hl = hold;
                if (h3v > 20.0 * d.hsal && isub > half) {
                    if (ilay == 1)      hl = hl + 0.0 * ng + fmax(hfor1 * ng + (-ng) * hl, 0.0);
                    else if (ilay == 2) hl = hl + 0.0 * ng + fmax(hfor2 * ng + (-ng) * hl, 0.0);
                    else if (ilay == 3) hl = hl - 0.0 * ng + fmin(hfor3 * ng + (-ng) * hl, 0.0);
                } else if (h3v < 20.0 * d.hsal && isub > half) {
                    if (ilay == 1)      hl = hl + 0.0 * ng + 1.0 * fmax(hfor2 * ng + (-ng) * hl, 0.0);
                    else if (ilay == 2) hl = hl - 0.0 * ng + 1.0 * fmin(hfor1 * ng + (-ng) * hl, 0.0);
                }
                if (isub < half) hl = hfor * ng + (1.0 - ng) * hold;
                hnew = hl;
            }
        }
        LL(d.hlay, ipnt, ilay) = hnew;
        if (copy_hist) {
            LL(d.rs[0], ipnt, ilay) = r2;
            LL(d.rs[1], ipnt, ilay) = rs_3;
        } else {
            LL(d.rs[0], ipnt, ilay) = rs_3;
        }
    }
}
template <class CTX, int FORCE>
__global__ __launch_bounds__(BEOM_BLOCK) void k_update_h(DevView d, double gene, double ramp,
                                                         double ctim, int copy_hist) {
    CTX c;
    if (!c.init(d)) return;
    if (c.wave_is_interior()) body_update_h<FORCE>(c.as_interior(), d, gene, ramp, ctim, copy_hist);
    else body_update_h<FORCE>(c, d, gene, ramp, ctim, copy_hist);
}

template <class C>
__device__ __forceinline__ void body_update_mont(const C &c, const DevView &d, int ilay_only) {
    const int ipnt = c.ipnt;
    const int ilay = ilay_only ? ilay_only : (int)blockIdx.y + 1;
    const int c1 = c.template nb<1>(), c3 = c.template nb<3>(), c5 = c.template nb<5>(),
              c6 = c.template nb<6>(), c7 = c.template nb<7>();
    const double i_dl = d.i_dl, i_gr = d.i_gr, i_ns = d.i_ns;
    const double hs_8 = d.hsal;
    const double u_le = LL(d.u, ipnt, ilay), u_ri = LL(d.u, c1, ilay);
    const double v_bo = LL(d.v, ipnt, ilay), v_to = LL(d.v, c3, ilay);
    const double mkn = c.mk_n();
    const double h0 = LL(d.hlay, ipnt, ilay);
    double mpot = -0.0;
    if (d.ocrp != 0.0) {
        mpot = h0 + d.hmin * (1.0 - mkn);
        mpot = powi_dev(d.hsal / mpot, d.nsal - 1);
        mpot = mpot * (-d.ocrp * i_ns * d.hsal * mkn);
    }
    mpot = mpot - (d.has_hto ? d.h_to[ipnt] : 0.0);
    const double i_rn = d.i_rn[ilay - 1];
    for (int i = 1; i <= ilay - 1; ++i)
        mpot = mpot - (d.rhon[ilay - 1] - d.rhon[i - 1]) * i_rn * LL(d.hlay, ipnt, i);
    if (d.rgld < 0.5) {
        double hcol = 0.0;
        for (int i = 1; i <= d.nlay; ++i) hcol = hcol + LL(d.hlay, ipnt, i);
        mpot = hcol - d.h_th[ipnt] + mpot;
    }
    LL(d.mont, ipnt, ilay) = mpot + 0.25 * d.uadv * i_gr
                                  * (u_ri * u_ri + u_le * u_le + v_to * v_to + v_bo * v_bo);
    const double rv = (v_bo - LL(d.v, c5, ilay) - u_le + LL(d.u, c7, ilay)) * i_dl * c.mkpe();
    LL(d.rvor, ipnt, ilay) = rv;
    const double hE = LL(d.hlay, c1, ilay), hW = LL(d.hlay, c5, ilay),
                 hN = LL(d.hlay, c3, ilay), hS = LL(d.hlay, c7, ilay);
    const double mk1 = c.template mk_n_nb<1>(c1), mk3 = c.template mk_n_nb<3>(c3), mk5 = c.template mk_n_nb<5>(c5),
                 mk6 = c.template mk_n_nb<6>(c6), mk7 = c.template mk_n_nb<7>(c7);
    double d2x = (hE + hW - h0 * 2.0) * mk1 * mk5 * mkn;
    double d2y = (hN + hS - h0 * 2.0) * mk3 * mk7 * mkn;
    if (d.ocrp > 0.5) {
        if (hE < 2.0 * hs_8 || hW < 2.0 * hs_8 || h0 < 2.0 * hs_8) d2x = 0.0;
        if (hN < 2.0 * hs_8 || hS < 2.0 * hs_8 || h0 < 2.0 * hs_8) d2y = 0.0;
    }
    LL(d.d2hx, ipnt, ilay) = d2x;
    LL(d.d2hy, ipnt, ilay) = d2y;
    const double have = h0 + hW + LL(d.hlay, c6, ilay) + hS;
    LL(d.pvor, ipnt, ilay) = (d.fcor[ipnt] + rv * d.uadv) * c.mkpi() * (mkn + mk5 + mk6 + mk7) / have;
    LL(d.dive, ipnt, ilay) = (u_ri - u_le + v_to - v_bo) * i_dl;
}
template <class CTX>
__global__ __launch_bounds__(BEOM_BLOCK) void k_update_mont(DevView d, int ilay_only) {
    CTX c;
    if (!c.init(d)) return;
    if (c.wave_is_interior()) body_update_mont(c.as_interior(), d, ilay_only);
    else body_update_mont(c, d, ilay_only);
}

template <int NL, class C>
__device__ __forceinline__ void body_update_mont_all(const C &c, const DevView &d) {
    const int ipnt = c.ipnt;
    const int c1 = c.template nb<1>(), c3 = c.template nb<3>(), c5 = c.template nb<5>(),
              c6 = c.template nb<6>(), c7 = c.template nb<7>();
    const double i_dl = d.i_dl, i_gr = d.i_gr, i_ns = d.i_ns;
    const double hs_8 = d.hsal;
    const double mkn = c.mk_n(), mkpe = c.mkpe(), mkpi = c.mkpi();
    const double mk1 = c.template mk_n_nb<1>(c1), mk3 = c.template mk_n_nb<3>(c3), mk5 = c.template mk_n_nb<5>(c5),
                 mk6 = c.template mk_n_nb<6>(c6), mk7 = c.template mk_n_nb<7>(c7);
    const double fcor = d.fcor[ipnt], h_th = d.h_th[ipnt];
    const double h_to = d.has_hto ? d.h_to[ipnt] : 0.0;
    double h[NL];
#pragma unroll
    for (int l = 0; l < NL; ++l) h[l] = LL(d.hlay, ipnt, l + 1);
    double hcol = 0.0;
#pragma unroll
    for (int l = 0; l < NL; ++l) hcol = hcol + h[l];
#pragma unroll
    for (int l = 0; l < NL; ++l) {
        const int ilay = l + 1;
        const double u_le = LL(d.u, ipnt, ilay), u_ri = LL(d.u, c1, ilay);
        const double v_bo = LL(d.v, ipnt, ilay), v_to = LL(d.v, c3, ilay);
        const double h0 = h[l];
        double mpot = -0.0;
        if (d.ocrp != 0.0) {
// ... 298 lines not shown
    CTX c;
    if (!c.init(d)) return;
    if (c.wave_is_interior()) body_update_visc(c.as_interior(), d, ilay_only);
    else body_update_visc(c, d, ilay_only);
}

struct UVio {
    const double *vel_in; double *vel_out;
    double *hp_out;
    const double *dm0, *dm1, *dm2;
    double *dm_out;
};

template <int Q>
using UVstage = double[TileGeom<Q>::SROWS][TileGeom<Q>::SLDX];
template <int Q>
using UVhstage = double[TileGeom<Q>::HROWS][TileGeom<Q>::HLDX];

struct ShGlobal {
    const DevView &d; int ipnt, cb, ca, ilay;
    __device__ __forceinline__ double hlay_s() const { return LL(d.hlay, ipnt, ilay); }
    __device__ __forceinline__ double hlay_b() const { return LL(d.hlay, cb, ilay); }
    __device__ __forceinline__ double mont_s() const { return LL(d.mont, ipnt, ilay); }
    __device__ __forceinline__ double mont_b() const { return LL(d.mont, cb, ilay); }
    __device__ __forceinline__ double pvor_s() const { return LL(d.pvor, ipnt, ilay); }
    __device__ __forceinline__ double pvor_a() const { return LL(d.pvor, ca, ilay); }
    __device__ __forceinline__ double pcd_s() const { return LL(d.pcd, ipnt, ilay); }
    __device__ __forceinline__ double pcd_b() const { return LL(d.pcd, cb, ilay); }
    __device__ __forceinline__ double qlr_s() const { return LL(d.qlr, ipnt, ilay); }
    __device__ __forceinline__ double qlr_a() const { return LL(d.qlr, ca, ilay); }
    template <bool XDIR> __device__ __forceinline__ double d2h_s() const { return LL(XDIR ? d.d2hx : d.d2hy, ipnt, ilay); }
    template <bool XDIR> __device__ __forceinline__ double d2h_b() const { return LL(XDIR ? d.d2hx : d.d2hy, cb, ilay); }
};
template <int Q, bool XDIR>
struct ShLds {
    const UVstage<Q> *s; const double (*h)[TileGeom<Q>::HLDX];
    int r, c;
    double ocrp, hs2;
    static constexpr int RB = XDIR ? 0 : -1, CB = XDIR ? -1 : 0;
    static constexpr int RA = XDIR ? 1 : 0, CA = XDIR ? 0 : 1;
    __device__ __forceinline__ double hlay_s() const { return h[r + 1][c + 1]; }
    __device__ __forceinline__ double hlay_b() const { return h[r + 1 + RB][c + 1 + CB]; }
    __device__ __forceinline__ double mont_s() const { return s[0][r][c]; }
    __device__ __forceinline__ double mont_b() const { return s[0][r + RB][c + CB]; }
    __device__ __forceinline__ double pvor_s() const { return s[1][r][c]; }
    __device__ __forceinline__ double pvor_a() const { return s[1][r + RA][c + CA]; }
    __device__ __forceinline__ double pcd_s() const { return s[2][r][c]; }
    __device__ __forceinline__ double pcd_b() const { return s[2][r + RB][c + CB]; }
    __device__ __forceinline__ double qlr_s() const { return s[3][r][c]; }
    __device__ __forceinline__ double qlr_a() const { return s[3][r + RA][c + CA]; }
    __device__ __forceinline__ double d2h_at(int rr, int cc) const {
        const double h0 = h[rr][cc];
        const double hp = XDIR ? h[rr][cc + 1] : h[rr + 1][cc];
        const double hm = XDIR ? h[rr][cc - 1] : h[rr - 1][cc];
        double v = (hp + hm - h0 * 2.0) * 1.0 * 1.0 * 1.0;
        if (ocrp > 0.5) { if (hp < hs2 || hm < hs2 || h0 < hs2) v = 0.0; }
        return v;
    }
    template <bool X> __device__ __forceinline__ double d2h_s() const { return d2h_at(r + 1, c + 1); }
    template <bool X> __device__ __forceinline__ double d2h_b() const { return d2h_at(r + 1 + RB, c + 1 + CB); }
};

template <bool XDIR, bool TOP, class C>
__device__ __forceinline__ double fold_drag(const C &c, const DevView &d, int ilay, double vel_self) {
    const int ipnt = c.ipnt;
    double other;
    if (XDIR) other = 0.25 * LL(d.v, ipnt, ilay) + 0.25 * LL(d.v, c.template nb<3>(), ilay) + 0.25 * LL(d.v, c.template nb<4>(), ilay)
                      + 0.25 * LL(d.v, c.template nb<5>(), ilay);
    else      other = 0.25 * LL(d.u, ipnt, ilay) + 0.25 * LL(d.u, c.template nb<1>(), ilay) + 0.25 * LL(d.u, c.template nb<7>(), ilay)
                      + 0.25 * LL(d.u, c.template nb<8>(), ilay);
    const double drg = TOP ? d.tdrg : d.bdrg;
    const double tau = vel_self * drg * (TOP ? d.rho_top : d.rho_bot) * (d.qdrg * sqrt(vel_self * vel_self + other * other) + 1.0 - d.qdrg);
    return tau * 0.5 * (1.0 + 1.0);
}

__device__ __forceinline__ double hist_from_mont(const DevView &d, double m_b, double m_s, double mask) {
    return (m_b - m_s) * d.i_dl * d.grav * mask;
}

template <bool XDIR, bool PROD, bool STORE, bool SF, bool HM, bool PLAIN = false, class C, class SH>
__device__ __forceinline__ double uv_core(const C &c, const DevView &d, int ilay, double gene, double ramp,
                                          double ctim, int copy_hist, const UVio &io,
                                          double q0, double qb, double qa, double qd, const SH &sh,
                                          bool do_store = true, const double *pre = nullptr, bool zv = false) {
    static_assert(!PLAIN || (PROD && !SF), "the plain form exists for the staged (PROD) bodies without the stress fold");
    const int ipnt = c.ipnt;
    const int cb = XDIR ? c.template nb<5>() : c.template nb<7>();
    const int ca = XDIR ? c.template nb<3>() : c.template nb<1>();
    constexpr int IV = XDIR ? 2 : 3;
    constexpr int ID = XDIR ? 1 : 2;
    constexpr int IO = XDIR ? 2 : 1;
    const double i_dl = d.i_dl, i_r0 = d.i_r0, i_r1 = d.i_r1;
    const double mask = XDIR ? c.mk_u() : c.mk_v();
    const double h_self = sh.hlay_s(), m_self = sh.mont_s(), pv0 = sh.pvor_s();
    const double hcen = XDIR ? (sh.hlay_b() + h_self) / (1.0 + mask)
                             : (h_self + sh.hlay_b()) / (1.0 + mask);
    double vold = pre ? pre[0] : LL(io.vel_in, ipnt, ilay);
    double f_ng = 0.0;
    if (!PLAIN && d.has_nudg) f_ng = NUDG_(ipnt, IV);
    const double dmd4 = (sh.mont_b() - m_self) * i_dl * d.grav * mask;
    const double pva = sh.pvor_a();
    double rhsi = dmd4 * (1.0 - gene);
    if (XDIR) rhsi = rhsi + 0.25 * pv0 * (q0 + qb) + 0.25 * pva * (qa + qd);
    else      rhsi = rhsi - 0.25 * pv0 * (q0 + qb) - 0.25 * pva * (qa + qd);
    if (SF) {
        const bool lay_t = ilay == 1, lay_b = ilay == d.nlay;
        if ((lay_t && (d.has_wind || d.has_top)) || (lay_b && d.has_bot)) {
            const double i__h = 1.0 / (hcen + 1.0 - mask);
            if (lay_t && d.has_wind) {
                const double tauw = 0.5 * (d.taus_cells[cb + d.n1 * (ID - 1)] + d.taus_cells[ipnt + d.n1 * (ID - 1)]) * ramp;
                rhsi = rhsi + tauw * i_r0 * i__h;
            } else rhsi = rhsi + 0.0;
            if (lay_b && d.has_bot) rhsi = rhsi - fold_drag<XDIR, false>(c, d, ilay, vold) * i_r0 * i__h;
            if (lay_t && d.has_top) rhsi = rhsi - fold_drag<XDIR, true>(c, d, ilay, vold) * i_r0 * i__h;
        }
    } else if (!PLAIN && d.has_stress) {
        const double i__h = 1.0 / (hcen + 1.0 - mask);
        const double tauw = 0.5 * (T3_(d.tt3d, cb, ID, ilay) + T3_(d.tt3d, ipnt, ID, ilay)) * ramp;
        rhsi = rhsi + tauw * i_r0 * i__h;
        rhsi = rhsi - T3_(d.tb3d, ipnt, ID, ilay) * i_r0 * i__h;
        rhsi = rhsi - T3_(d.tu3d, ipnt, ID, ilay) * i_r0 * i__h;
    }
    rhsi = rhsi + ((!PLAIN && d.has_bodf) ? d.bodf[(ilay - 1) + d.nlay * (ID - 1)] : 0.0);
    if (HM) {
        if (gene != 0.0 || rhsi == 0.0) {
            double h0, h1, h2;
            if (pre) { h0 = pre[5]; h1 = pre[6]; h2 = pre[7]; }
            else {
                h0 = hist_from_mont(d, LL(d.mo0, cb, ilay), LL(d.mo0, ipnt, ilay), mask);
                h1 = hist_from_mont(d, LL(d.mo1, cb, ilay), LL(d.mo1, ipnt, ilay), mask);
                h2 = hist_from_mont(d, LL(d.mo2, cb, ilay), LL(d.mo2, ipnt, ilay), mask);
            }
            rhsi = rhsi + (d.del1 * dmd4 + d.del2 * h2 + d.gamm * h1 + d.epsi * h0) * gene;
        }
    } else if (gene != 0.0 || rhsi == 0.0) {
        const bool p = pre && gene != 0.0;
        rhsi = rhsi + (d.del1 * dmd4 + d.del2 * (p ? pre[7] : LL(io.dm2, ipnt, ilay)) + d.gamm * (p ? pre[6] : LL(io.dm1, ipnt, ilay))
                       + d.epsi * (p ? pre[5] : LL(io.dm0, ipnt, ilay))) * gene;
    }
    if (!PROD && d.svis > 0.0) {
        const double i__h = 1.0 / (hcen + 1.0 - mask);
        if (XDIR) rhsi = rhsi - d.svis * i_dl * (double)(float)(LL(d.uu4, ipnt, ilay) - LL(d.uu4, cb, ilay)
                                                               + LL(d.vv4, ca, ilay) - LL(d.vv4, ipnt, ilay)) * i__h;
        else      rhsi = rhsi - d.svis * i_dl * (LL(d.vv4, ca, ilay) - LL(d.vv4, ipnt, ilay)
                                                - LL(d.uu4, ipnt, ilay) + LL(d.uu4, cb, ilay)) * i__h;
    } else if (PROD && zv) {
        if (rhsi == 0.0 && __builtin_signbit(rhsi)) {
            const int oE = c.template nb<1>() - ipnt, oN = c.template nb<3>() - ipnt,
                      oW = c.template nb<5>() - ipnt, oS = c.template nb<7>() - ipnt;
            auto dive_at = [&](int x) {
                return (LL(d.u, x + oE, ilay) - LL(d.u, x, ilay) + LL(d.v, x + oN, ilay) - LL(d.v, x, ilay)) * d.i_dl;
            };
            auto rvor_at = [&](int x) {
                return (LL(d.v, x, ilay) - LL(d.v, x + oW, ilay) - LL(d.u, x, ilay) + LL(d.u, x + oS, ilay)) * d.i_dl * 1.0;
            };
            const double p0 = 0.0 * dive_at(ipnt), pb = 0.0 * dive_at(cb);
            const double l0 = 0.0 * rvor_at(ipnt), la = 0.0 * rvor_at(ca);
            if (XDIR) rhsi = rhsi + (p0 - pb) * i_dl - (la - l0) * i_dl;
            else      rhsi = rhsi + (p0 - pb) * i_dl + (la - l0) * i_dl;
        }
    } else if (PROD) {
        const double p0 = sh.pcd_s(), pb = sh.pcd_b();
        const double l0 = sh.qlr_s(), la = sh.qlr_a();
        if (XDIR) rhsi = rhsi + (p0 - pb) * i_dl - (la - l0) * i_dl;
        else      rhsi = rhsi + (p0 - pb) * i_dl + (la - l0) * i_dl;
    } else {
        const double vc0 = LL(d.v_cc, ipnt, ilay), vcb = LL(d.v_cc, cb, ilay);
        const double vl0 = LL(d.v_ll, ipnt, ilay), vla = LL(d.v_ll, ca, ilay);
        const double dv0 = LL(d.dive, ipnt, ilay), dvb = LL(d.dive, cb, ilay);
        const double rv0 = LL(d.rvor, ipnt, ilay), rva = LL(d.rvor, ca, ilay);
        if (XDIR) rhsi = rhsi + (vc0 * dv0 - vcb * dvb) * i_dl - (vla * rva - vl0 * rv0) * i_dl;
        else      rhsi = rhsi + (vc0 * dv0 - vcb * dvb) * i_dl + (vla * rva - vl0 * rv0) * i_dl;
    }
    vold = vold + rhsi * mask * d.dt;
    if (PLAIN && vold == 0.0 && !d.fnud_vel) {
        vold = 0.0;
    } else if ((!PLAIN && f_ng != 0.0) || vold == 0.0) {
        const double i__hh = 1.0 / (hcen + 1.0 - mask);
        double vfor = d.fnud_vel ? FNUDV_(ipnt, ilay, IV) : 0.0;
        if (SF) {
            const double lt = ilay == 1 ? 1.0 : 0.0;
            const double t0 = d.has_wind ? d.taus_cells[ipnt + d.n1 * (IO - 1)] * lt : 0.0, tb_ = d.has_wind ? d.taus_cells[cb + d.n1 * (IO - 1)] * lt : 0.0;
            const double ek = 0.5 * (t0 + tb_) * i_r1 * d.invf * i__hh * ramp;
            vfor = XDIR ? vfor + ek : vfor - ek;
        } else if (!PLAIN && d.has_stress) {
            const double ek = 0.5 * (T3_(d.tt3d, ipnt, IO, ilay) + T3_(d.tt3d, cb, IO, ilay))
                              * i_r1 * d.invf * i__hh * ramp;
            vfor = XDIR ? vfor + ek : vfor - ek;
        } else {
            vfor = XDIR ? vfor + 0.0 : vfor - 0.0;
        }
        if (!PLAIN && d.has_tide) vfor = vfor + ramp * TIDE_(1, ipnt, IV) * cos(TIDE_(2, ipnt, IV) - d.w_ti * ctim);
        else vfor = vfor + 0.0;
        vold = vfor * f_ng + vold * (1.0 - f_ng);
    }
    const double hnew = 0.5 * (vold + fabs(vold)) * (hcen - 0.16667 * sh.template d2h_b<XDIR>())
                      + 0.5 * (vold - fabs(vold)) * (hcen - 0.16667 * sh.template d2h_s<XDIR>());
    if (STORE && do_store) {
        LL(io.vel_out, ipnt, ilay) = vold;
        if (PLAIN || d.rgld < 0.5) LL(io.hp_out, ipnt, ilay) = hnew;
        if (HM) {
        } else if (copy_hist) {
            const double m2 = LL(io.dm1, ipnt, ilay), m3 = LL(io.dm2, ipnt, ilay);
            LL(const_cast<double *>(io.dm0), ipnt, ilay) = m2;
            LL(const_cast<double *>(io.dm1), ipnt, ilay) = m3;
            LL(const_cast<double *>(io.dm2), ipnt, ilay) = dmd4;
        } else {
            LL(io.dm_out, ipnt, ilay) = dmd4;
        }
    }
    return hnew;
}

template <bool XDIR, bool PROD, class C>
__device__ __forceinline__ void body_update_uv(const C &c, const DevView &d, int ilay_only, double gene,
                                               double ramp, double ctim, int copy_hist) {
    const int ipnt = c.ipnt;
    const int ilay = ilay_only ? ilay_only : (int)blockIdx.y + 1;
    const int cb = XDIR ? c.template nb<5>() : c.template nb<7>();
    const int ca = XDIR ? c.template nb<3>() : c.template nb<1>();
    const int cd = XDIR ? c.template nb<4>() : c.template nb<8>();
    const double *hq = XDIR ? d.h_v : d.h_u;
    double *const *dm = XDIR ? d.dmx : d.dmy;
    const UVio io{XDIR ? d.u : d.v, XDIR ? d.u : d.v, XDIR ? d.h_u : d.h_v, dm[0], dm[1], dm[2], dm[0]};
    const ShGlobal sh{d, ipnt, cb, ca, ilay};
    uv_core<XDIR, PROD, true, false, false>(c, d, ilay, gene, ramp, ctim, copy_hist, io,
                              LL(hq, ipnt, ilay), LL(hq, cb, ilay), LL(hq, ca, ilay), LL(hq, cd, ilay), sh);
}
template <class CTX, bool XDIR, bool PROD = false>
__global__ __launch_bounds__(BEOM_BLOCK) void k_update_uv(DevView d, int ilay_only, double gene,
                                                          double ramp, double ctim, int copy_hist) {
    CTX c;
    if (!c.init(d)) return;
    if (c.wave_is_interior()) body_update_uv<XDIR, PROD>(c.as_interior(), d, ilay_only, gene, ramp, ctim, copy_hist);
    else body_update_uv<XDIR, PROD>(c, d, ilay_only, gene, ramp, ctim, copy_hist);
}

template <bool FIRST_X, bool PROD, bool STORE, bool INT, bool SF, bool HM = false, bool PLAIN = false, class SH>
__device__ __forceinline__ double uv_first_eval(const DevView &d, const CellDenseT<INT> &c, int ilay, double gene,
                                                double ramp, double ctim, const SH &sh, bool do_store = true,
                                                const double *pre = nullptr, bool zv = false) {
    const int ipnt = c.ipnt;
    const int cb = FIRST_X ? c.template nb<5>() : c.template nb<7>();
    const int ca = FIRST_X ? c.template nb<3>() : c.template nb<1>();
    const int cd = FIRST_X ? c.template nb<4>() : c.template nb<8>();
    const double *hq = FIRST_X ? d.h_v : d.h_u;
    double *const *dm = FIRST_X ? d.dmx : d.dmy;
    const UVio io{FIRST_X ? d.u : d.v, FIRST_X ? d.u_alt : d.v_alt, FIRST_X ? d.h_u : d.h_v,
                  HM ? nullptr : dm[0], HM ? nullptr : dm[1], HM ? nullptr : dm[2], HM ? nullptr : dm[3]};
    if (pre) return uv_core<FIRST_X, PROD, STORE, SF, HM, PLAIN>(c, d, ilay, gene, ramp, ctim, 0, io, pre[1], pre[2], pre[3], pre[4],
                                                      sh, do_store, pre, zv);
    return uv_core<FIRST_X, PROD, STORE, SF, HM, PLAIN>(c, d, ilay, gene, ramp, ctim, 0, io, LL(hq, ipnt, ilay),
                                             LL(hq, cb, ilay), LL(hq, ca, ilay), LL(hq, cd, ilay), sh, do_store);
}

template <bool FIRST_X, bool PROD, bool SF, bool HM = false, bool PLAIN = false>
__device__ __forceinline__ double uv_first_halo(const DevView &d, int a, int b, int ilay, double gene,
                                                double ramp, double ctim) {
    if (d.xper) { if (a == 0) a = d.L - 1; else if (a == d.L) a = 1; }
    if (d.yper && !d.slab) { if (b == 0) b = d.M - 1; else if (b == d.M) b = 1; }
    if (a < 1 || a > d.L || b < 1 || b > d.M) return 0.0;
    if (!slot_is_cell(d, a + (b - 1) * d.P)) return 0.0;
    CellDenseT<false> h;
    h.set_cell(d, a, b);
    const int cb = FIRST_X ? h.template nb<5>() : h.template nb<7>();
    const int ca = FIRST_X ? h.template nb<3>() : h.template nb<1>();
    const ShGlobal sh{d, h.ipnt, cb, ca, ilay};
    return uv_first_eval<FIRST_X, PROD, false, false, SF, HM, PLAIN>(d, h, ilay, gene, ramp, ctim, sh);
}

template <bool FIRST_X, bool HM = false>
__device__ __forceinline__ void uv_pre_load(const DevView &d, const CellDenseT<true> &c, int ilay, double gene,
                                            bool with_q, double (&pre)[8]) {
    const int ipnt = c.ipnt;
    double *const *dm = FIRST_X ? d.dmx : d.dmy;
    pre[0] = LL(FIRST_X ? d.u : d.v, ipnt, ilay);
    if (with_q) {
        const double *hq = FIRST_X ? d.h_v : d.h_u;
        const int cb = FIRST_X ? c.template nb<5>() : c.template nb<7>();
        const int ca = FIRST_X ? c.template nb<3>() : c.template nb<1>();
        const int cd = FIRST_X ? c.template nb<4>() : c.template nb<8>();
        pre[1] = LL(hq, ipnt, ilay); pre[2] = LL(hq, cb, ilay); pre[3] = LL(hq, ca, ilay); pre[4] = LL(hq, cd, ilay);
    }
    if (!HM && gene != 0.0) { pre[5] = LL(dm[0], ipnt, ilay); pre[6] = LL(dm[1], ipnt, ilay); pre[7] = LL(dm[2], ipnt, ilay); }
}
__device__ __forceinline__ void hm_load(const DevView &d, int ip, int ilay, double (&m)[3]) {
    m[0] = LL(d.mo0, ip, ilay); m[1] = LL(d.mo1, ip, ilay); m[2] = LL(d.mo2, ip, ilay);
}
__device__ __forceinline__ void hm_form(const DevView &d, const double (&ms)[3], const double (&mb)[3], double (&pre)[8]) {
    pre[5] = hist_from_mont(d, mb[0], ms[0], 1.0); pre[6] = hist_from_mont(d, mb[1], ms[1], 1.0);
    pre[7] = hist_from_mont(d, mb[2], ms[2], 1.0);
}
template <int TY>
__device__ __forceinline__ void hm_form_w(const DevView &d, const double (&ms)[3], const double (*col)[TY], int row, int lx,
                                          double (&pre)[8]) {
    double mw[3];
#pragma unroll
    for (int k = 0; k < 3; ++k) {
        mw[k] = __shfl_up(ms[k], 1, 64);
        if (lx == 0) mw[k] = col[k][row];
    }
    hm_form(d, ms, mw, pre);
}
template <int TY>
__device__ __forceinline__ double (*hm_side_table())[TY] {
    __shared__ double s_w[3][TY];
    return s_w;
}

template <int Q, bool FIRST_X, bool ZV, bool SF, bool HM, bool PLAIN>
__device__ __forceinline__ void body_uv_fused_staged(const DevView &d, int x0, int y0, int ilay, double gene,
                                                     double ramp, double ctim, double (*s_h)[TileGeom<Q>::LDX], UVstage<Q> *s_f,
                                                     double (*s_hl)[TileGeom<Q>::HLDX]) {
    using G = TileGeom<Q>;
    const int tid = threadIdx.x;
    const int lx = tid & 63, wy = tid >> 6;
    const int i = x0 + lx;
    constexpr int ROFF = FIRST_X ? 1 : 0, COFF = FIRST_X ? 0 : 1;
    constexpr int NST = G::SROWS * (G::TX + 2), NIT = (NST + G::BLOCK - 1) / G::BLOCK;
    const long long lay = d.n1 * (long long)(ilay - 1);
    constexpr int NF = ZV ? 2 : 4;
    const double *src[5] = {d.mont, d.pvor, ZV ? d.hlay : d.pcd, ZV ? d.hlay : d.qlr, d.hlay};
    double fv[NIT][5];
    int frr[NIT], fcc[NIT];
#pragma unroll
    for (int k = 0; k < NIT; ++k) {
        const int idx = tid + k * G::BLOCK;
        const int idc = idx < NST ? idx : tid;
        frr[k] = idc / (G::TX + 2); fcc[k] = idc - frr[k] * (G::TX + 2);
        const long long ip = (long long)(x0 - 1 + fcc[k]) + (long long)(y0 - 2 + frr[k]) * d.P + lay;
#pragma unroll
        for (int f = 0; f < 5; ++f) if (f >= NF && f < 4) fv[k][f] = 0.0; else fv[k][f] = src[f][ip];
    }
    int hrr = -1, hcc = -1;
    if (tid < G::TX + 2) { hrr = 0; hcc = 1 + tid; }
    else if (tid < 2 * (G::TX + 2)) { hrr = G::HROWS - 1; hcc = 1 + tid - (G::TX + 2); }
    else if (tid < 2 * (G::TX + 2) + G::SROWS) { hrr = 1 + tid - 2 * (G::TX + 2); hcc = 0; }
    else if (tid < 2 * (G::TX + 2) + 2 * G::SROWS) { hrr = 1 + tid - 2 * (G::TX + 2) - G::SROWS; hcc = G::HLDX - 1; }
    const double hring = d.hlay[(long long)(x0 - 2 + (hrr >= 0 ? hcc : 2)) + (long long)(y0 - 3 + (hrr >= 0 ? hrr : 2)) * d.P + lay];
    CellDenseT<true> c[Q];
    bool wr[Q];
    double pre[Q][8];
#pragma unroll
    for (int q = 0; q < Q; ++q) {
        const int j = y0 + wy + G::WAVES * q;
        wr[q] = row_selected(d, j);
        c[q].set_cell(d, i, j);
        uv_pre_load<FIRST_X, HM>(d, c[q], ilay, gene, true, pre[q]);
    }
    int rr1 = -1, cc1 = -1;
    if (tid <= G::TX) { rr1 = FIRST_X ? 0 : G::TY; cc1 = tid; }
    else if (tid <= G::TX + G::TY) { rr1 = (tid - G::TX - 1) + ROFF; cc1 = FIRST_X ? G::TX : 0; }
    const int ra = rr1 >= 0 ? (FIRST_X ? x0 : x0 - 1) + cc1 : i;
    const int rb = rr1 >= 0 ? (FIRST_X ? y0 - 1 : y0) + rr1 : y0 + wy;
    CellDenseT<true> hc;
    hc.set_cell(d, ra, rb);
    double preR[8];
    uv_pre_load<FIRST_X, HM>(d, hc, ilay, gene, true, preR);
    double ms[Q][3], mb[Q][3], msR[3], mbR[3];
    double (*s_w)[G::TY] = nullptr;
    const int wrow = tid - (G::TX + 1) - (FIRST_X ? G::TY : 0);
    const bool wfill = wrow >= 0 && wrow < G::TY;
    if constexpr (HM) {
        s_w = hm_side_table<G::TY>();
#pragma unroll
        for (int q = 0; q < Q; ++q) hm_load(d, c[q].ipnt, ilay, ms[q]);
        hm_load(d, hc.ipnt, ilay, msR);
        int ib = FIRST_X ? hc.template nb<5>() : hc.template nb<7>();
        if (FIRST_X && wfill) ib = (x0 - 1) + (y0 + wrow - 1) * d.P;
        hm_load(d, ib, ilay, mbR);
    }
#pragma unroll
    for (int k = 0; k < NIT; ++k) {
        if (tid + k * G::BLOCK < NST) {
#pragma unroll
            for (int f = 0; f < NF; ++f) s_f[f][frr[k]][fcc[k]] = fv[k][f];
            s_hl[frr[k] + 1][fcc[k] + 1] = fv[k][4];
        }
    }
    if (hrr >= 0) s_hl[hrr][hcc] = hring;
    if constexpr (HM) {
        if (wfill) { s_w[0][wrow] = FIRST_X ? mbR[0] : msR[0]; s_w[1][wrow] = FIRST_X ? mbR[1] : msR[1]; s_w[2][wrow] = FIRST_X ? mbR[2] : msR[2]; }
        if (!FIRST_X) {
#pragma unroll
            for (int q = 0; q < Q; ++q) hm_load(d, c[q].template nb<7>(), ilay, mb[q]);
        }
    }
    __syncthreads();
    double pre2[Q][8];
#pragma unroll
    for (int q = 0; q < Q; ++q) {
        uv_pre_load<!FIRST_X, HM>(d, c[q], ilay, gene, false, pre2[q]);
        if (HM && FIRST_X) hm_load(d, c[q].template nb<7>(), ilay, mb[q]);
    }
    const double hs2 = 2.0 * d.hsal;
    auto ring_cell = [&]() {
        if (rr1 >= 0) {
            const ShLds<Q, FIRST_X> sh{s_f, s_hl, rb - (y0 - 1), ra - (x0 - 1), d.ocrp, hs2};
            if (HM) hm_form(d, msR, mbR, preR);
            s_h[rr1][cc1] = uv_first_eval<FIRST_X, true, false, true, SF, HM, PLAIN>(d, hc, ilay, gene, ramp, ctim, sh, true, preR, ZV);
        }
    };
    if (HM) ring_cell();
#pragma unroll
    for (int q = 0; q < Q; ++q) {
        const int r = wy + G::WAVES * q;
        const ShLds<Q, FIRST_X> sh{s_f, s_hl, r + 1, lx + 1, d.ocrp, hs2};
        if constexpr (HM) {
            if (FIRST_X) hm_form_w<G::TY>(d, ms[q], s_w, r, lx, pre[q]);
            else hm_form(d, ms[q], mb[q], pre[q]);
        }
        s_h[r + ROFF][lx + COFF] = uv_first_eval<FIRST_X, true, true, true, SF, HM, PLAIN>(d, c[q], ilay, gene, ramp, ctim, sh, wr[q], pre[q], ZV);
    }
    if (!HM) ring_cell();
    __syncthreads();
    double *const *dm = FIRST_X ? d.dmy : d.dmx;
    const UVio io{FIRST_X ? d.v : d.u, FIRST_X ? d.v_alt : d.u_alt, FIRST_X ? d.hv_alt : d.hu_alt,
                  HM ? nullptr : dm[0], HM ? nullptr : dm[1], HM ? nullptr : dm[2], HM ? nullptr : dm[0]};
#pragma unroll
    for (int q = 0; q < Q; ++q) {
        const int r = wy + G::WAVES * q;
        if constexpr (HM) {
            if (FIRST_X) hm_form(d, ms[q], mb[q], pre2[q]);
            else hm_form_w<G::TY>(d, ms[q], s_w, r, lx, pre2[q]);
        }
        if (!wr[q]) continue;
        double q0, qb, qa, qd;
        if (FIRST_X) {
            q0 = s_h[r + 1][lx]; qb = s_h[r][lx]; qa = s_h[r + 1][lx + 1]; qd = s_h[r][lx + 1];
        } else {
            q0 = s_h[r][lx + 1]; qb = s_h[r][lx]; qa = s_h[r + 1][lx + 1]; qd = s_h[r + 1][lx];
        }
        const ShLds<Q, !FIRST_X> sh{s_f, s_hl, r + 1, lx + 1, d.ocrp, hs2};
        uv_core<!FIRST_X, true, true, SF, HM, PLAIN>(c[q], d, ilay, gene, ramp, ctim, 0, io, q0, qb, qa, qd, sh, true, pre2[q], ZV);
    }
}

template <int Q, bool FIRST_X, bool INT, bool SF>
__device__ __forceinline__ void body_uv_fused(const DevView &d, int x0, int y0, int ilay, double gene,
                                              double ramp, double ctim, double (*s_h)[TileGeom<Q>::LDX]) {
    using G = TileGeom<Q>;
    const int tid = threadIdx.x;
    const int lx = tid & 63, wy = tid >> 6;
    const int i = x0 + lx;
    constexpr int ROFF = FIRST_X ? 1 : 0, COFF = FIRST_X ? 0 : 1;
    CellDenseT<INT> c[Q];
    bool ok[Q], wr[Q];
#pragma unroll
    for (int q = 0; q < Q; ++q) {
        const int r = wy + G::WAVES * q, j = y0 + r;
        ok[q] = (i <= d.L) && (j <= d.M);
        if (!INT && ok[q] && !slot_is_cell(d, i + (j - 1) * d.P)) ok[q] = false;
        wr[q] = ok[q] && row_selected(d, j);
        c[q].set_cell(d, ok[q] ? i : 1, ok[q] ? j : 1);
        double hnew = 0.0;
        if (ok[q]) {
            const int cb = FIRST_X ? c[q].template nb<5>() : c[q].template nb<7>();
            const int ca = FIRST_X ? c[q].template nb<3>() : c[q].template nb<1>();
            const ShGlobal sh{d, c[q].ipnt, cb, ca, ilay};
            hnew = uv_first_eval<FIRST_X, false, true, INT, SF>(d, c[q], ilay, gene, ramp, ctim, sh, wr[q]);
            if (!INT) {
                if ((d.xper && i == d.L) || (d.yper && !d.slab && j == d.M))
                    hnew = uv_first_halo<FIRST_X, false, SF>(d, i, j, ilay, gene, ramp, ctim);
            }
        }
        s_h[r + ROFF][lx + COFF] = hnew;
    }
    {
        int rr = -1, cc = -1;
        if (tid <= G::TX) {
            rr = FIRST_X ? 0 : G::TY; cc = tid;
        } else if (tid <= G::TX + G::TY) {
            rr = (tid - G::TX - 1) + ROFF; cc = FIRST_X ? G::TX : 0;
        }
        if (rr >= 0) {
            const int a = (FIRST_X ? x0 : x0 - 1) + cc;
            const int b = (FIRST_X ? y0 - 1 : y0) + rr;
            s_h[rr][cc] = uv_first_halo<FIRST_X, false, SF>(d, a, b, ilay, gene, ramp, ctim);
        }
    }
    __syncthreads();
    double *const *dm = FIRST_X ? d.dmy : d.dmx;
    const UVio io{FIRST_X ? d.v : d.u, FIRST_X ? d.v_alt : d.u_alt, FIRST_X ? d.hv_alt : d.hu_alt,
                  dm[0], dm[1], dm[2], dm[0]};
#pragma unroll
    for (int q = 0; q < Q; ++q) {
        if (!wr[q]) continue;
        const int r = wy + G::WAVES * q;
        double q0, qb, qa, qd;
        if (FIRST_X) {
            q0 = s_h[r + 1][lx]; qb = s_h[r][lx]; qa = s_h[r + 1][lx + 1]; qd = s_h[r][lx + 1];
        } else {
            q0 = s_h[r][lx + 1]; qb = s_h[r][lx]; qa = s_h[r + 1][lx + 1]; qd = s_h[r + 1][lx];
        }
        const int cb = !FIRST_X ? c[q].template nb<5>() : c[q].template nb<7>();
        const int ca = !FIRST_X ? c[q].template nb<3>() : c[q].template nb<1>();
        const ShGlobal sh{d, c[q].ipnt, cb, ca, ilay};
        uv_core<!FIRST_X, false, true, SF, false>(c[q], d, ilay, gene, ramp, ctim, 0, io, q0, qb, qa, qd, sh);
    }
}

template <int Q, bool XDIR>
struct ShLdsEdge {
    const UVstage<Q> *s; const double (*h)[TileGeom<Q>::SLDX];
    int r, c;
    const DevView &d; int ipnt, cb, ilay;
    static constexpr int RB = XDIR ? 0 : -1, CB = XDIR ? -1 : 0;
    static constexpr int RA = XDIR ? 1 : 0, CA = XDIR ? 0 : 1;
    __device__ __forceinline__ double hlay_s() const { return h[r][c]; }
    __device__ __forceinline__ double hlay_b() const { return h[r + RB][c + CB]; }
    __device__ __forceinline__ double mont_s() const { return s[0][r][c]; }
    __device__ __forceinline__ double mont_b() const { return s[0][r + RB][c + CB]; }
    __device__ __forceinline__ double pvor_s() const { return s[1][r][c]; }
    __device__ __forceinline__ double pvor_a() const { return s[1][r + RA][c + CA]; }
    __device__ __forceinline__ double pcd_s() const { return s[2][r][c]; }
    __device__ __forceinline__ double pcd_b() const { return s[2][r + RB][c + CB]; }
    __device__ __forceinline__ double qlr_s() const { return s[3][r][c]; }
// ... 31 lines not shown
#pragma unroll
        for (int k = 0; k < NIT; ++k) {
            if (tid + k * G::BLOCK < NST) {
#pragma unroll
                for (int f = 0; f < 4; ++f) s_f[f][frr[k]][fcc[k]] = fv[k][f];
                s_hs[frr[k]][fcc[k]] = fv[k][4];
            }
        }
    }
    CellDenseT<false> c[Q];
    bool ok[Q], wr[Q];
#pragma unroll
    for (int q = 0; q < Q; ++q) {
        const int j = y0 + wy + G::WAVES * q;
        ok[q] = (i <= d.L) && (j <= d.M);
        if (ok[q] && !slot_is_cell(d, i + (j - 1) * d.P)) ok[q] = false;
        wr[q] = ok[q] && row_selected(d, j);
        c[q].set_cell(d, ok[q] ? i : 1, ok[q] ? j : 1);
    }
    __syncthreads();
#pragma unroll
    for (int q = 0; q < Q; ++q) {
        const int r = wy + G::WAVES * q, j = y0 + r;
        double hnew = 0.0;
        if (ok[q]) {
            const int cb = FIRST_X ? c[q].template nb<5>() : c[q].template nb<7>();
            if ((d.xper && i == d.L) || (d.yper && !d.slab && j == d.M)) {
                const int ca = FIRST_X ? c[q].template nb<3>() : c[q].template nb<1>();
                const ShGlobal sh{d, c[q].ipnt, cb, ca, ilay};
                (void)uv_first_eval<FIRST_X, true, true, false, SF, HM, PLAIN>(d, c[q], ilay, gene, ramp, ctim, sh, wr[q]);
                hnew = uv_first_halo<FIRST_X, true, SF, HM, PLAIN>(d, i, j, ilay, gene, ramp, ctim);
            } else {
                const ShLdsEdge<Q, FIRST_X> sh{s_f, s_hs, r + 1, lx + 1, d, c[q].ipnt, cb, ilay};
                hnew = uv_first_eval<FIRST_X, true, true, false, SF, HM, PLAIN>(d, c[q], ilay, gene, ramp, ctim, sh, wr[q]);
            }
        }
        s_h[r + ROFF][lx + COFF] = hnew;
    }
    {
        int rr = -1, cc = -1;
        if (tid <= G::TX) { rr = FIRST_X ? 0 : G::TY; cc = tid; }
        else if (tid <= G::TX + G::TY) { rr = (tid - G::TX - 1) + ROFF; cc = FIRST_X ? G::TX : 0; }
        if (rr >= 0) {
            const int ga = (FIRST_X ? x0 : x0 - 1) + cc, gb = (FIRST_X ? y0 - 1 : y0) + rr;
            int a = ga, b = gb;
            double val = 0.0;
            if (halo_target<false>(d, a, b) && slot_is_cell(d, a + (b - 1) * d.P)) {
                if (a != ga || b != gb) {
                    val = uv_first_halo<FIRST_X, true, SF, HM, PLAIN>(d, ga, gb, ilay, gene, ramp, ctim);
                } else {
                    CellDenseT<false> h;
                    h.set_cell(d, a, b);
                    const int cb = FIRST_X ? h.template nb<5>() : h.template nb<7>();
                    const ShLdsEdge<Q, FIRST_X> sh{s_f, s_hs, gb - (y0 - 1), ga - (x0 - 1), d, h.ipnt, cb, ilay};
                    val = uv_first_eval<FIRST_X, true, false, false, SF, HM, PLAIN>(d, h, ilay, gene, ramp, ctim, sh);
                }
            }
            s_h[rr][cc] = val;
        }
    }
    __syncthreads();
    double *const *dm = FIRST_X ? d.dmy : d.dmx;
    const UVio io{FIRST_X ? d.v : d.u, FIRST_X ? d.v_alt : d.u_alt, FIRST_X ? d.hv_alt : d.hu_alt,
                  HM ? nullptr : dm[0], HM ? nullptr : dm[1], HM ? nullptr : dm[2], HM ? nullptr : dm[0]};
#pragma unroll
    for (int q = 0; q < Q; ++q) {
        if (!wr[q]) continue;
        const int r = wy + G::WAVES * q;
        double q0, qb, qa, qd;
        if (FIRST_X) { q0 = s_h[r + 1][lx]; qb = s_h[r][lx]; qa = s_h[r + 1][lx + 1]; qd = s_h[r][lx + 1]; }
        else         { q0 = s_h[r][lx + 1]; qb = s_h[r][lx]; qa = s_h[r + 1][lx + 1]; qd = s_h[r + 1][lx]; }
        const int cb = !FIRST_X ? c[q].template nb<5>() : c[q].template nb<7>();
        if ((d.xper && i == d.L) || (d.yper && !d.slab && y0 + r == d.M)) {
            const int ca = !FIRST_X ? c[q].template nb<3>() : c[q].template nb<1>();
            const ShGlobal sh{d, c[q].ipnt, cb, ca, ilay};
            uv_core<!FIRST_X, true, true, SF, HM, PLAIN>(c[q], d, ilay, gene, ramp, ctim, 0, io, q0, qb, qa, qd, sh);
        } else {
            const ShLdsEdge<Q, !FIRST_X> sh{s_f, s_hs, r + 1, lx + 1, d, c[q].ipnt, cb, ilay};
            uv_core<!FIRST_X, true, true, SF, HM, PLAIN>(c[q], d, ilay, gene, ramp, ctim, 0, io, q0, qb, qa, qd, sh);
        }
    }
}

template <int Q, bool FIRST_X, bool PROD, bool ZV, bool SF, bool HM = false, bool PLAIN = false>
__device__ __forceinline__ void uv_fused_workgroup(const DevView &d, double gene, double ramp, double ctim) {
    static_assert(PROD || !HM, "the history-from-Montgomery form exists for the staged (PROD) bodies only");
    static_assert(!PLAIN || (PROD && !SF), "the plain form exists for the staged (PROD) bodies without the stress fold");
    using G = TileGeom<Q>;
    __shared__ double s_h[G::TY + 1][G::LDX];
    __shared__ UVstage<Q> s_f[PROD ? 4 : 1];
    __shared__ double s_hl[PROD ? G::HROWS : 1][G::HLDX];
    const TileMap tm(d, G::TX, G::TY);
    int ty, ch;
    if (!tm.locate(blockIdx.x, ty, ch)) return;
    const int x0 = ch * G::TX + 1, y0 = ty * G::TY + 1;
    const int ilay = blockIdx.y + 1;
    const bool interior = x0 - 1 >= 2 && x0 + G::TX <= d.L - 2 && y0 - 1 >= 2 && y0 + G::TY <= d.M - 2
                          && y0 - 1 + d.joff >= 2 && y0 + G::TY + d.joff <= d.Mg - 2 && tile_regular(d, x0, y0, G::TY);
    if (interior && PROD) body_uv_fused_staged<Q, FIRST_X, ZV, SF, HM, PLAIN>(d, x0, y0, ilay, gene, ramp, ctim, s_h, s_f, s_hl);
    else if (interior) body_uv_fused<Q, FIRST_X, true, SF>(d, x0, y0, ilay, gene, ramp, ctim, s_h);
    else if (PROD) body_uv_fused_edge<Q, FIRST_X, SF, HM, PLAIN>(d, x0, y0, ilay, gene, ramp, ctim, s_h, s_f, s_hl);
    else body_uv_fused<Q, FIRST_X, false, SF>(d, x0, y0, ilay, gene, ramp, ctim, s_h);
}
template <int Q, bool FIRST_X, bool PROD, bool ZV = false, bool HM = false, bool PLAIN = false>
__global__ __launch_bounds__(TileGeom<Q>::BLOCK) void k_uv_fused(DevView d, double gene, double ramp, double ctim) {
    uv_fused_workgroup<Q, FIRST_X, PROD, ZV, false, HM, PLAIN>(d, gene, ramp, ctim);
}
template <int Q, bool FIRST_X, bool PROD, bool ZV = false>
__global__ __launch_bounds__(TileGeom<Q>::BLOCK) __attribute__((amdgpu_waves_per_eu(3))) void k_uv_fused_sf(DevView d, double gene, double ramp, double ctim) {
    uv_fused_workgroup<Q, FIRST_X, PROD, ZV, true>(d, gene, ramp, ctim);
}
__global__ __launch_bounds__(BEOM_BLOCK) void k_hist_from_mont(DevView d) {
    CellDense c;
    if (!c.init(d)) return;
    const int ipnt = c.ipnt, ilay = blockIdx.y + 1;
    const int c5 = c.template nb<5>(), c7 = c.template nb<7>();
    const double mku = c.mk_u(), mkv = c.mk_v();
    const double s0 = LL(d.mo1, ipnt, ilay), s1 = LL(d.mo2, ipnt, ilay), s2 = LL(d.mont, ipnt, ilay);
    const double w0 = LL(d.mo1, c5, ilay), w1 = LL(d.mo2, c5, ilay), w2 = LL(d.mont, c5, ilay);
    const double t0 = LL(d.mo1, c7, ilay), t1 = LL(d.mo2, c7, ilay), t2 = LL(d.mont, c7, ilay);
    LL(d.dmx[0], ipnt, ilay) = hist_from_mont(d, w0, s0, mku);
    LL(d.dmx[1], ipnt, ilay) = hist_from_mont(d, w1, s1, mku);
    LL(d.dmx[2], ipnt, ilay) = hist_from_mont(d, w2, s2, mku);
    LL(d.dmy[0], ipnt, ilay) = hist_from_mont(d, t0, s0, mkv);
    LL(d.dmy[1], ipnt, ilay) = hist_from_mont(d, t1, s1, mkv);
    LL(d.dmy[2], ipnt, ilay) = hist_from_mont(d, t2, s2, mkv);
}

template <int Q>
static inline dim3 uv_fused_grid(const DevView &d) {
    return dim3(TileMap(d, TileGeom<Q>::TX, TileGeom<Q>::TY).blocks(), (unsigned)d.nlay, 1);
}

template <bool FROM_TOP>
__device__ __forceinline__ void stress_fractions(const DevView &d, int q, double (*lay)[BEOM_BLOCK]) {
    const int nlay = d.nlay, t = threadIdx.x;
    if (FROM_TOP) {
        if (d.ocrp > 0.5) {
            for (int ilay = 1; ilay <= nlay; ++ilay) {
                double hcum = 0.0, sofar = 0.0;
                for (int k = 1; k < ilay; ++k) sofar = sofar + lay[k - 1][t];
                sofar = sofar + 0.0;
                for (int k = 1; k <= ilay; ++k) hcum = hcum + fmax(0.0, LL(d.hlay, q, k) - 1.5 * d.hsal);
                const double x = fmin(hcum, d.hsbl) / d.hsbl - sofar;
                lay[ilay - 1][t] = fmax(x, 0.0);
            }
        } else {
            for (int ilay = 1; ilay <= nlay; ++ilay) lay[ilay - 1][t] = (ilay == 1) ? 1.0 : 0.0;
        }
    } else {
        if (d.ocrp > 0.5) {
            for (int ilay = nlay; ilay >= 1; --ilay) {
                double sofar = 0.0, hcum = 0.0;
                sofar = sofar + 0.0;
                for (int k = ilay + 1; k <= nlay; ++k) sofar = sofar + lay[k - 1][t];
                for (int k = ilay; k <= nlay; ++k) hcum = hcum + LL(d.hlay, q, k);
                const double x = fmin(hcum, d.hbbl) / d.hbbl - sofar;
                lay[ilay - 1][t] = fmax(x, 0.0);
            }
        } else {
            for (int ilay = 1; ilay <= nlay; ++ilay) lay[ilay - 1][t] = (ilay == nlay) ? 1.0 : 0.0;
        }
    }
}
template <bool TOP>
__device__ __forceinline__ void stress_tau(const DevView &d, int ipnt, double &tau_u, double &tau_v) {
    const int nlay = d.nlay;
    int ilay = TOP ? 1 : nlay;
    if (d.ocrp > 0.5) {
        if (!TOP) { for (int k = nlay; k >= 1; --k) if (LL(d.hlay, ipnt, k) > 2.0 * d.hsal) { ilay = k; break; } }
        else      { for (int k = 1; k <= nlay; ++k) if (LL(d.hlay, ipnt, k) > 2.0 * d.hsal) { ilay = k; break; } }
    }
    const int32_t *row = d.neig + 8ll * ipnt;
    const int c1 = row[0], c3 = row[2], c4 = row[3], c5 = row[4], c7 = row[6], c8 = row[7];
    const double uu = LL(d.u, ipnt, ilay), vv = LL(d.v, ipnt, ilay);
    const double vatu = 0.25 * vv + 0.25 * LL(d.v, c3, ilay) + 0.25 * LL(d.v, c4, ilay) + 0.25 * LL(d.v, c5, ilay);
    const double uatv = 0.25 * uu + 0.25 * LL(d.u, c1, ilay) + 0.25 * LL(d.u, c7, ilay) + 0.25 * LL(d.u, c8, ilay);
    const double drg = TOP ? d.tdrg : d.bdrg;
    const double rh = d.rhon[ilay - 1];
    tau_u = uu * drg * rh * (d.qdrg * sqrt(uu * uu + vatu * vatu) + 1.0 - d.qdrg);
    tau_v = vv * drg * rh * (d.qdrg * sqrt(vv * vv + uatv * uatv) + 1.0 - d.qdrg);
}
__global__ __launch_bounds__(BEOM_BLOCK) void k_stress(DevView d, int wind, int bot, int top) {
    __shared__ double s_own[BEOM_MAX_LAYERS][BEOM_BLOCK], s_w[BEOM_MAX_LAYERS][BEOM_BLOCK], s_s[BEOM_MAX_LAYERS][BEOM_BLOCK];
    const int ipnt = blockIdx.x * BEOM_BLOCK + threadIdx.x + 1, t = threadIdx.x;
    if (!cell_slot(d, ipnt)) return;
    const int nlay = d.nlay;
    const int c5 = d.neig[8ll * ipnt + 4], c7 = d.neig[8ll * ipnt + 6];
    if (wind || top) {
// ... 520 lines not shown
```

### beom_amd/csrc/beom_plan.h

```cpp
#pragma once

namespace beom_plan {

struct StepFacts {
    bool dense; int nlay; bool lid;
    double svis, dvis, bvis, g_fb, ocrp;
    bool has_nudg, has_tide, has_stress, has_bodf, has_hto;
    bool wind, bot, top, up_tt, up_tb, up_tu;
    bool fold_static_ok, visc_all_zero, mont_keep;
    bool fuse, fuse_uv, fold_stress, lean_d2h, lean_visc, mont_history, plain_sweeps, keep_diag;
    int mont_levels_valid;
};

struct StepPlan {
    int tstp, n_3d;
    double ctim, ramp, gene;
    bool first3, upst, stress_fold, launch_stress, rebuild, leith, launch_visc, needs_arrays;
    struct Mont { bool fused, keep_visc, lean_d2h, zero_visc, plain; } mont;
    struct Uv { bool fused_uv, first_x, prod, zv, hm, plain; } uv;
};

inline bool fuses_uv(const StepFacts &f) { return f.dense && f.fuse_uv; }

inline bool can_fuse(const StepFacts &f, bool first3) {
    if (!(f.dense && f.fuse && f.nlay <= 8) || f.svis > 0.0) return false;
    if (f.dvis > 1.e-3) return true;
    return !first3;
}

inline StepPlan plan_step(const StepFacts &f, int tstp, double tres, double dtd8, double dt_r, double rsta, int n_3d) {
    StepPlan p{};
    p.tstp = tstp;
    p.ctim = tres + dtd8 * (double)tstp;
    p.first3 = tstp <= 3;
    p.ramp = 1.0;
    bool stress;
    if (p.first3) {
        const double c1 = tres + dtd8 * 1.0;
        if (rsta < 0.5 && c1 < dt_r) p.ramp = c1 / dt_r;
        p.upst = true;
        stress = tstp == 1;
    } else {
        if (rsta < 0.5 && p.ctim < dt_r) p.ramp = p.ctim / dt_r;
        p.upst = (tstp % n_3d) == 0;
        stress = p.upst;
    }
    p.gene = (p.first3 || (f.lid && f.g_fb > 0.5)) ? 0.0 : f.g_fb;
    p.n_3d = n_3d;
    p.rebuild = p.first3;
    p.mont.fused = can_fuse(f, p.first3);
    p.uv.fused_uv = fuses_uv(f);
    p.uv.first_x = tstp % 2 == 0;
    p.stress_fold = f.fold_stress && f.fold_static_ok && p.uv.fused_uv && stress && !p.first3 && p.n_3d == 1 && !f.keep_diag &&
                    (f.wind || !f.up_tt) && (f.bot || !f.up_tb) && (f.top || !f.up_tu);
    p.launch_stress = stress && !p.stress_fold;
    p.leith = f.dvis > 1.e-3 && p.upst;
    p.uv.prod = p.mont.fused;
    if (p.mont.fused) {
        const bool uv_fused_follows = p.uv.fused_uv;
        p.mont.lean_d2h = uv_fused_follows && f.lean_d2h && !f.keep_diag;
        p.mont.keep_visc = p.leith && p.n_3d > 1;
        p.mont.zero_visc = !p.leith && uv_fused_follows && f.lean_visc && f.visc_all_zero && f.dvis == 0.0 && f.bvis == 0.0 &&
                           !f.keep_diag;
        p.mont.plain = f.plain_sweeps && f.ocrp == 0.0 && !f.lid && !f.has_hto && !f.keep_diag && !p.mont.keep_visc;
    }
    p.launch_visc = !p.uv.prod && (p.first3 || p.leith || f.svis > 0.0);
    if (p.uv.fused_uv) {
        p.uv.zv = p.uv.prod && p.mont.zero_visc;
        p.uv.plain = f.plain_sweeps && p.uv.prod && !p.stress_fold && !f.has_nudg && !f.has_tide && !f.has_stress && !f.has_bodf &&
                     !f.lid && f.svis == 0.0;
    }
    p.uv.hm = f.mont_history && f.mont_keep && p.mont.fused && p.uv.fused_uv && p.gene != 0.0 && !p.stress_fold &&
              f.mont_levels_valid >= 3;
    p.needs_arrays = !p.uv.hm;
    return p;
}

constexpr bool uv_form_exists(bool sf, bool prod, bool zv, bool hm, bool plain) { return !((zv || hm || plain) && !prod) && !(sf && (hm || plain)); }

}
```

Measured before the change: 21.09 billion.

## Skip storing second-sweep thickness fluxes and recompute them in the thickness update

```diff
diff --git a/beom_amd/csrc/beom_dev.h b/beom_amd/csrc/beom_dev.h
--- a/beom_amd/csrc/beom_dev.h
+++ b/beom_amd/csrc/beom_dev.h
@@ -52,6 +52,8 @@
     const double *taus_cells;
     double rho_top, rho_bot;
     double *mo0, *mo1, *mo2;
+    double *hlay_alt;
+    int uv_ty;
 };
 
 struct TileMap {
diff --git a/beom_amd/csrc/beom_engine.hip b/beom_amd/csrc/beom_engine.hip
--- a/beom_amd/csrc/beom_engine.hip
+++ b/beom_amd/csrc/beom_engine.hip
@@ -145,6 +145,10 @@
     bool hist_stale = false;
     bool last_mont_hist = false;
     bool plain_sweeps = true;
+    bool lean_fluxes = true;
+    int flux_stale = 0;
+    bool hlay_alt_fresh = false;
+    bool last_lean = false;
     int last_plain = 0;
     double *integ_part = nullptr, *integ_rows = nullptr;
     int integ_count = 0;
@@ -183,6 +187,7 @@
     char last_err[512] = {0};
 };
 static int hist_sync(beom_engine *E);
+static int flux_sync(beom_engine *E);
 static int leave_mont_history(beom_engine *E);
 
 namespace {
@@ -325,6 +330,7 @@
     for (size_t i = 0; i < n1h; ++i) { if (g.mk_u[i] > 0.5) E->any_u = 1; if (g.mk_v[i] > 0.5) E->any_v = 1; }
     E->tile4 = E->dense && (long long)((d.L + 63) / 64) * ((d.M + 7) / 8) <= 5000;
     if (getenv("BEOM_TILE4")) E->tile4 = E->dense && atoi(getenv("BEOM_TILE4")) != 0;
+    d.uv_ty = E->tile4 ? 4 : 8;
     if (E->lid) E->fuse = E->fuse_uv = false;
     if (st.taus) for (size_t i = 0; i < 2 * n1h; ++i) if (std::fabs(st.taus[i]) > 1.e-7) { E->wind = true; break; }
     E->bot = prm.bdrg > 1.e-7;
@@ -400,6 +406,7 @@
     al({&d.pcd, &d.qlr, &d.mont, &d.rvor, &d.pvor, &d.dive, &d.d2hx, &d.d2hy}, n);
     E->mont_keep = E->dense && !E->lid && !d.slab && E->P.g_fb != 0.0 && d.nlay <= 8 && !(E->P.svis > 0.0);
     if (E->mont_keep) al({&d.mo0, &d.mo1, &d.mo2}, n);
+    if (E->mont_keep) al({&d.hlay_alt}, n);
     if (E->P.svis > 0.0) al({&d.delu, &d.delv, &d.uu4, &d.vv4}, n);
     if (E->lid) al({&d.pi_s, &d.pi_rhs, &d.pi_prev}, (size_t)d.n1);
     if (rc) return rc;
@@ -554,6 +561,7 @@
     int rc;
     if ((rc = leave_mont_history(E))) { set_err(errm, errm_len, "beom_upload_state: the history arrays could not be brought up to date"); return rc; }
     if ((rc = copy_in(E, d.hlay, hlay, nl, errm, errm_len))) return rc;
+    if (hlay) E->hlay_alt_fresh = false;
     if ((rc = copy_in(E, d.u, u, nl, errm, errm_len))) return rc;
     if ((rc = copy_in(E, d.v, v, nl, errm, errm_len))) return rc;
     if ((rc = copy_in(E, d.h_u, h_u, nl, errm, errm_len))) return rc;
@@ -684,10 +692,20 @@
     double *t = d.mo0; d.mo0 = d.mo1; d.mo1 = d.mo2; d.mo2 = d.mont; d.mont = t;
 }
 static int hist_sync(beom_engine *E) {
+    if (const int rc = flux_sync(E)) return rc;
     if (!E->hist_stale) return 0;
     if (hipSetDevice(E->device) != hipSuccess) return -9;
     hipLaunchKernelGGL(k_hist_from_mont, CellDense::grid(E->d, E->d.nlay), dim3(BEOM_BLOCK), 0, E->stream, E->d);
     E->hist_stale = false;
+    return hipGetLastError() == hipSuccess ? 0 : -10;
+}
+static int flux_sync(beom_engine *E) {
+    if (!E->flux_stale) return 0;
+    if (hipSetDevice(E->device) != hipSuccess) return -9;
+    const dim3 g = CellDense::grid(E->d, E->d.nlay), b(BEOM_BLOCK);
+    if (E->flux_stale == 1) hipLaunchKernelGGL(k_flux_sync<true>, g, b, 0, E->stream, E->d);
+    else hipLaunchKernelGGL(k_flux_sync<false>, g, b, 0, E->stream, E->d);
+    E->flux_stale = 0;
     return hipGetLastError() == hipSuccess ? 0 : -10;
 }
 static int leave_mont_history(beom_engine *E) {
@@ -724,6 +742,18 @@
     if (E->d.has_nudg) nz = 1;
     pick_int<2, 0>(forcing(E->d), [&](auto fo) { LAUNCH_CTX((k_update_h<CellGather, fo>), (k_update_h<CellDense, fo>), nz, E->d, gene, ramp, ctim, 0); });
     if (rotate) rot2(E->d.rs);
+}
+static void launch_h_from_vel(beom_engine *E, double gene) {
+    DevView &d = E->d;
+    if (!E->hlay_alt_fresh) {
+        (void)hipMemcpyAsync(d.hlay_alt, d.hlay, (size_t)d.nlay * (size_t)d.n1 * sizeof(double), hipMemcpyDeviceToDevice, E->stream);
+        E->hlay_alt_fresh = true;
+    }
+    const dim3 g = CellDense::grid(d, d.nlay), b(BEOM_BLOCK);
+    if (E->flux_stale == 1) hipLaunchKernelGGL(k_update_h_fv<true>, g, b, 0, E->stream, d, gene);
+    else hipLaunchKernelGGL(k_update_h_fv<false>, g, b, 0, E->stream, d, gene);
+    swp(d.hlay, d.hlay_alt);
+    rot2(d.rs);
 }
 static void launch_tracers(beom_engine *E, double gene, double ramp, double ctim) {
     TrcView tv{E->ntrc, E->trc_ctrg ? 1 : 0, E->trc_q, E->trc_q_alt, E->trc_rq[0], E->trc_rq[1], E->trc_ctrg};
@@ -848,6 +878,13 @@
 template <int Q>
 static void raw_uv_fused(beom_engine *E, const StepPlan &p) {
     const dim3 g = uv_fused_grid<Q>(E->d), b(TileGeom<Q>::BLOCK);
+    if constexpr (Q == 2) {
+        if (p.uv.lean) {
+            pick([&](auto fx, auto zv) { hipLaunchKernelGGL((k_uv_fused<Q, fx, true, zv, true, true, true>), g, b, 0, E->stream, E->d, p.gene, p.ramp, p.ctim); },
+                 p.uv.first_x, p.uv.zv);
+            return;
+        }
+    }
     pick([&](auto fx, auto pl, auto hm, auto sf, auto zv, auto pr) {
         if constexpr (!beom_plan::uv_form_exists(sf, pr, zv, hm, pl)) { fprintf(stderr, "beom: the plan names a form of the u+v sweep that does not exist\n"); std::abort(); }
         else if constexpr (sf) hipLaunchKernelGGL((k_uv_fused_sf<Q, fx, pr, zv>), g, b, 0, E->stream, E->d, p.gene, p.ramp, p.ctim);
@@ -866,6 +903,7 @@
 static void launch_uv_fused(beom_engine *E, const StepPlan &p, bool swap = true) {
     if (E->tile4) raw_uv_fused<1>(E, p); else raw_uv_fused<2>(E, p);
     if (swap) uv_fused_swap(E, p.uv.first_x, p.uv.hm);
+    E->flux_stale = p.uv.lean ? (p.uv.first_x ? 2 : 1) : 0;
 }
 static void launch_lid_fluxes(beom_engine *E, bool first3) {
     if (first3) { launch_rebuild(E); return; }
@@ -947,6 +985,9 @@
     f.fuse = E->fuse; f.fuse_uv = E->fuse_uv; f.fold_stress = E->fold_stress; f.lean_d2h = E->lean_d2h; f.lean_visc = E->lean_visc;
     f.mont_history = E->mont_history; f.plain_sweeps = E->plain_sweeps; f.keep_diag = d.keep_diag != 0;
     f.mont_levels_valid = E->mont_levels_valid;
+    f.lean_fluxes = E->lean_fluxes && d.hlay_alt != nullptr && !E->embedded && !E->tile4;
+    f.flux_readers = E->ntrc > 0 || E->mom.level > 0 || E->tmom.level > 0 || E->ser_level > 0 || E->obc;
+    f.flux_stale = E->flux_stale;
     return f;
 }
 static void apply_plan(beom_engine *E, const StepPlan &p) {
@@ -955,6 +996,7 @@
     E->last_folded = p.stress_fold;
     E->last_uv_fused = p.uv.fused_uv;
     E->last_mont_hist = p.uv.hm;
+    E->last_lean = p.uv.lean;
     E->last_plain = (p.uv.plain ? 1 : 0) | (p.mont.plain ? 2 : 0);
 }
 
@@ -976,7 +1018,8 @@
     else if (p.rebuild) launch_rebuild(E);
     if (E->ntrc > 0) timed(T, 7, [&] { launch_tracers(E, p.gene, p.ramp, p.ctim); });
     timed(T, 0, [&] {
-        launch_h(E, p.gene, p.ramp, p.ctim);
+        if (p.h_from_vel) launch_h_from_vel(E, p.gene);
+        else launch_h(E, p.gene, p.ramp, p.ctim);
         if (E->lid) launch_lid_h_epilogue(E);
     });
     timed(T, p.mont.fused ? 5 : 1, [&] {
@@ -990,6 +1033,7 @@
     const int tstp = p.tstp;
     if (flt >= 0 && (flt & 1)) launch_floats(E, 1, nullptr);
     if (p.needs_arrays) (void)hist_sync(E);
+    if (p.flux_sync) (void)flux_sync(E);
     rotate_mont(E);
     StepTimer *T = step_timer(E, tstp);
     apply_plan(E, p);
@@ -1020,6 +1064,8 @@
     if (!E || !dbuf || jlo < 1 || nrows < 1 || jlo + nrows - 1 > E->d.M) return -3;
     if (dbuf2 && (jlo2 < 1 || jlo2 + nrows - 1 > E->d.M)) return -3;
     if (hipSetDevice(E->device) != hipSuccess) return -9;
+    if (flux_sync(E)) return -10;
+    if (!PACK) E->hlay_alt_fresh = false;
     const long long total = 5ll * E->d.nlay * nrows * E->d.L;
     hipLaunchKernelGGL((k_rows_copy<PACK>), dim3((unsigned)((total + BEOM_BLOCK - 1) / BEOM_BLOCK), dbuf2 ? 2u : 1u), dim3(BEOM_BLOCK),
                        0, E->stream, E->d, jlo, nrows, (double *)dbuf, jlo2, (double *)dbuf2);
@@ -1333,6 +1379,7 @@
     if (level > 0 && (jlo < 1 || nrows < 1 || jlo + nrows - 1 > d.M)) { set_err(errm, errm_len, "%s: rows %d..%d outside 1..%d", who, jlo, jlo + nrows - 1, d.M); return -3; }
     if (level > 0 && pow2_ceil((d.L + 63) / 64) / 64 > kIntegralMaxGroups) { set_err(errm, errm_len, "%s: rows of more than %d columns", who, 64 * 64 * kIntegralMaxGroups); return -4; }
     HIP_TRY(hipSetDevice(E->device));
+    if (flux_sync(E)) { set_err(errm, errm_len, "%s: the transports could not be brought up to date", who); return -10; }
     HIP_TRY(hipStreamSynchronize(E->stream));
     series_free(E);
     if (level == 0) return 0;
@@ -1390,6 +1437,7 @@
     if (ntrc > 0 && E->P.variant == 1) { set_err(errm, errm_len, "beom_set_tracers: variant 1 changes the thickness in an epilogue (private_mod3d.f95:1635-1683) that the tracer scheme does not follow"); return -6; }
     if (ntrc > 0 && E->lid) { set_err(errm, errm_len, "beom_set_tracers: rgld = 1 changes the thickness in the lid's misfit epilogue (private_mod.f95:1648-1700), which the tracer scheme does not follow"); return -6; }
     HIP_TRY(hipSetDevice(E->device));
+    if (flux_sync(E)) { set_err(errm, errm_len, "beom_set_tracers: the transports could not be brought up to date"); return -10; }
     HIP_TRY(hipStreamSynchronize(E->stream));
     if (ntrc != E->ntrc) accum_free(E->tmom);
     free_tracers(E);
@@ -1691,6 +1739,7 @@
     if (level < 0 || level > 3 || stride < 1) { set_err(errm, errm_len, K.bad_args, level, stride); return -3; }
     if (K.no_tracer && level > 0 && E->ntrc < 1) { set_err(errm, errm_len, "%s", K.no_tracer); return -3; }
     HIP_TRY(hipSetDevice(E->device));
+    if (flux_sync(E)) { set_err(errm, errm_len, "the transports could not be brought up to date"); return -10; }
     HIP_TRY(hipStreamSynchronize(E->stream));
     accum_free(A);
     if (level == 0) return 0;
@@ -1831,6 +1880,7 @@
     if (!strcmp(what, "biharm_tiled")) return biharm_tiled(E) ? 1 : 0;
     if (!strcmp(what, "uv_fused")) return E->last_uv_fused ? 1 : 0;
     if (!strcmp(what, "mont_history")) return E->last_mont_hist ? 1 : 0;
+    if (!strcmp(what, "lean_fluxes")) return E->last_lean ? 1 : 0;
     if (!strcmp(what, "plain_sweeps")) return E->last_plain;
     if (!strcmp(what, "vel_targets_zero")) return E->d.vel_targets_zero;
     if (!strcmp(what, "tracers")) return E->ntrc;
@@ -1857,6 +1907,7 @@
 int beom_set_option(beom_handle E, const char *name, int value) {
     if (!E || !name) return -1;
     if (!strncmp(name, "fuse", 4) && hist_sync(E)) return -10;
+    if (!strcmp(name, "lean_fluxes") && flux_sync(E)) return -10;
     if (!strcmp(name, "fuse")) { E->fuse = value != 0; E->fuse_uv = value != 0; }
     else if (!strcmp(name, "fuse_mont_visc")) E->fuse = value != 0 && !E->lid;
     else if (!strcmp(name, "fuse_uv")) E->fuse_uv = value != 0 && !E->lid;
@@ -1868,6 +1919,7 @@
     else if (!strcmp(name, "lean_visc")) E->lean_visc = value != 0;
     else if (!strcmp(name, "mont_history")) E->mont_history = value != 0;
     else if (!strcmp(name, "plain_sweeps")) E->plain_sweeps = value != 0;
+    else if (!strcmp(name, "lean_fluxes")) E->lean_fluxes = value != 0;
     else if (!strcmp(name, "moments_by_caller")) E->mom_by_caller = value != 0;
     else return -3;
     return 0;
@@ -1884,6 +1936,7 @@
 int beom_device_field(beom_handle E, const char *name, void **dptr, int64_t *stride_layer,
                       int64_t *stride_row, int64_t *row0_offset) {
     if (!E || !name || !dptr) return -1;
+    if (flux_sync(E)) return -10;
     const DevView &d = E->d;
     double *p = nullptr;
     if (!strcmp(name, "hlay")) p = d.hlay;
diff --git a/beom_amd/csrc/beom_kernels.h b/beom_amd/csrc/beom_kernels.h
--- a/beom_amd/csrc/beom_kernels.h
+++ b/beom_amd/csrc/beom_kernels.h
@@ -11,6 +11,46 @@
     double r = x;
     for (int q = 1; q < n; ++q) r = r * x;
     return r;
+}
+
+__device__ __forceinline__ bool uv_tile_interior(const DevView &d, int x0, int y0, int TY) {
+    return x0 - 1 >= 2 && x0 + 64 <= d.L - 2 && y0 - 1 >= 2 && y0 + TY <= d.M - 2
+           && y0 - 1 + d.joff >= 2 && y0 + TY + d.joff <= d.Mg - 2 && tile_regular(d, x0, y0, TY);
+}
+__device__ __forceinline__ bool uv_tile_deep(const DevView &d, int x0, int y0, int TY) {
+    bool deep = x0 - 1 - 64 >= 2 && x0 + 2 * 64 <= d.L - 2 && y0 - 1 - TY >= 2 && y0 + 2 * TY <= d.M - 2
+                && y0 - 1 - TY + d.joff >= 2 && y0 + 2 * TY + d.joff <= d.Mg - 2;
+    if (deep && d.embedded)
+        for (int dy = -1; dy <= 1; ++dy)
+            for (int dx = -1; dx <= 1; ++dx) deep = deep && tile_regular(d, x0 + dx * 64, y0 + dy * TY, TY);
+    return deep;
+}
+
+__device__ __forceinline__ double d2h_interior(const DevView &d, double hp, double hm, double h0) {
+    double v = (hp + hm - h0 * 2.0) * 1.0 * 1.0 * 1.0;
+    if (d.ocrp > 0.5) { const double hs2 = 2.0 * d.hsal; if (hp < hs2 || hm < hs2 || h0 < hs2) v = 0.0; }
+    return v;
+}
+__device__ __forceinline__ double flux_from_vel(double vel, double hb, double hs, double cb, double cs) {
+    const double hcen = (hb + hs) / (1.0 + 1.0);
+    return 0.5 * (vel + fabs(vel)) * (hcen - 0.16667 * cb) + 0.5 * (vel - fabs(vel)) * (hcen - 0.16667 * cs);
+}
+__device__ __forceinline__ void uv_tile_of_wave(const DevView &d, const CellDense &c, int &x0, int &y0) {
+    x0 = __builtin_amdgcn_readfirstlane(c.i - ((int)threadIdx.x & 63));
+    y0 = ((c.j - 1) & ~(d.uv_ty - 1)) + 1;
+}
+template <bool XS>
+__global__ __launch_bounds__(BEOM_BLOCK) void k_flux_sync(DevView d) {
+    CellDense c;
+    if (!c.init(d)) return;
+    int x0, y0;
+    uv_tile_of_wave(d, c, x0, y0);
+    if (!uv_tile_deep(d, x0, y0, d.uv_ty)) return;
+    const int ipnt = c.ipnt, ilay = blockIdx.y + 1, o = XS ? 1 : d.P;
+    const double h0 = LL(d.hlay, ipnt, ilay), hb = LL(d.hlay, ipnt - o, ilay), hb2 = LL(d.hlay, ipnt - 2 * o, ilay),
+                 ha = LL(d.hlay, ipnt + o, ilay);
+    const double vel = LL(XS ? d.u : d.v, ipnt, ilay);
+    LL(XS ? d.h_u : d.h_v, ipnt, ilay) = flux_from_vel(vel, hb, h0, d2h_interior(d, h0, hb2, hb), d2h_interior(d, ha, hb, h0));
 }
 
 template <class C>
@@ -112,6 +152,79 @@
     if (!c.init(d)) return;
     if (c.wave_is_interior()) body_update_h<FORCE>(c.as_interior(), d, gene, ramp, ctim, copy_hist);
     else body_update_h<FORCE>(c, d, gene, ramp, ctim, copy_hist);
+}
+
+template <bool XS, bool REC, class C>
+__device__ __forceinline__ void body_update_h_fv(const C &c, const DevView &d, double gene) {
+    const int ipnt = c.ipnt;
+    const int c1 = c.template nb<1>(), c3 = c.template nb<3>();
+    const double i_dl = d.i_dl;
+    const double mkn = c.mk_n();
+    const int lane = (int)threadIdx.x & 63;
+    const int ilay_hi = gridDim.y == 1 ? d.nlay : (int)blockIdx.y + 1;
+    const int ilay_lo = gridDim.y == 1 ? 1 : (int)blockIdx.y + 1;
+    for (int ilay = ilay_hi; ilay >= ilay_lo; --ilay) {
+        double hold = LL(d.hlay, ipnt, ilay);
+        double hu0, huE, hv0, hvN;
+        if (REC && XS) {
+            const double u0 = LL(d.u, ipnt, ilay);
+            double uE = __shfl_down(u0, 1, 64), hE = __shfl_down(hold, 1, 64), hE2 = __shfl_down(hold, 2, 64);
+            double hW = __shfl_up(hold, 1, 64), hW2 = __shfl_up(hold, 2, 64);
+            if (lane == 63) { uE = LL(d.u, ipnt + 1, ilay); hE = LL(d.hlay, ipnt + 1, ilay); }
+            if (lane >= 62) hE2 = LL(d.hlay, ipnt + 2, ilay);
+            if (lane == 0) hW = LL(d.hlay, ipnt - 1, ilay);
+            if (lane <= 1) hW2 = LL(d.hlay, ipnt - 2, ilay);
+            const double cW = d2h_interior(d, hold, hW2, hW), c0 = d2h_interior(d, hE, hW, hold), cE = d2h_interior(d, hE2, hold, hE);
+            hu0 = flux_from_vel(u0, hW, hold, cW, c0);
+            huE = flux_from_vel(uE, hold, hE, c0, cE);
+        } else {
+            hu0 = LL(d.h_u, ipnt, ilay);
+            if (C::kLanesAreRowNeighbours) {
+                huE = __shfl_down(hu0, 1, 64);
+                if (lane == 63) huE = LL(d.h_u, c1, ilay);
+            } else {
+                huE = LL(d.h_u, c1, ilay);
+            }
+        }
+        if (REC && !XS) {
+            const int P = c3 - ipnt;
+            const double hS2 = LL(d.hlay, ipnt - 2 * P, ilay), hS = LL(d.hlay, ipnt - P, ilay), hN = LL(d.hlay, c3, ilay),
+                         hN2 = LL(d.hlay, ipnt + 2 * P, ilay);
+            const double v0 = LL(d.v, ipnt, ilay), vN = LL(d.v, c3, ilay);
+            const double cS = d2h_interior(d, hold, hS2, hS), c0 = d2h_interior(d, hN, hS, hold), cN = d2h_interior(d, hN2, hold, hN);
+            hv0 = flux_from_vel(v0, hS, hold, cS, c0);
+            hvN = flux_from_vel(vN, hold, hN, c0, cN);
+        } else {
+            hv0 = LL(d.h_v, ipnt, ilay);
+            hvN = LL(d.h_v, c3, ilay);
+        }
+        double rs_3 = (hu0 - huE) * i_dl
+                    + (hv0 - hvN) * i_dl
+                    + (d.has_hdot ? LL(d.hdot, ipnt, ilay) : 0.0);
+        rs_3 = rs_3 * mkn;
+        const double r2 = LL(d.rs[1], ipnt, ilay);
+        double rhsi;
+        if (gene != 0.0) {
+            const double r1 = LL(d.rs[0], ipnt, ilay);
+            rhsi = ((1.5 + d.beta) * rs_3 - (0.5 + 2.0 * d.beta) * r2 + d.beta * r1) * d.dt * gene
+                 + rs_3 * d.dt * (1.0 - gene);
+        } else {
+            rhsi = rs_3 * d.dt;
+        }
+        hold = hold + rhsi;
+        LL(d.hlay_alt, ipnt, ilay) = 0.0 + hold;
+        LL(d.rs[0], ipnt, ilay) = rs_3;
+    }
+}
+template <bool XS>
+__global__ __launch_bounds__(BEOM_BLOCK) void k_update_h_fv(DevView d, double gene) {
+    CellDense c;
+    if (!c.init(d)) return;
+    int x0, y0;
+    uv_tile_of_wave(d, c, x0, y0);
+    if (uv_tile_interior(d, x0, y0, d.uv_ty)) body_update_h_fv<XS, true>(c.as_interior(), d, gene);
+    else if (c.wave_is_interior()) body_update_h_fv<XS, false>(c.as_interior(), d, gene);
+    else body_update_h_fv<XS, false>(c, d, gene);
 }
 
 template <class C>
@@ -576,7 +689,8 @@
 __device__ __forceinline__ double uv_core(const C &c, const DevView &d, int ilay, double gene, double ramp,
                                           double ctim, int copy_hist, const UVio &io,
                                           double q0, double qb, double qa, double qd, const SH &sh,
-                                          bool do_store = true, const double *pre = nullptr, bool zv = false) {
+                                          bool do_store = true, const double *pre = nullptr, bool zv = false,
+                                          bool store_hp = true) {
     static_assert(!PLAIN || (PROD && !SF), "the plain form exists for the staged (PROD) bodies without the stress fold");
     const int ipnt = c.ipnt;
     const int cb = XDIR ? c.template nb<5>() : c.template nb<7>();
@@ -692,7 +806,7 @@
                       + 0.5 * (vold - fabs(vold)) * (hcen - 0.16667 * sh.template d2h_s<XDIR>());
     if (STORE && do_store) {
         LL(io.vel_out, ipnt, ilay) = vold;
-        if (PLAIN || d.rgld < 0.5) LL(io.hp_out, ipnt, ilay) = hnew;
+        if ((PLAIN || d.rgld < 0.5) && store_hp) LL(io.hp_out, ipnt, ilay) = hnew;
         if (HM) {
         } else if (copy_hist) {
             const double m2 = LL(io.dm1, ipnt, ilay), m3 = LL(io.dm2, ipnt, ilay);
@@ -805,7 +919,7 @@
 template <int Q, bool FIRST_X, bool ZV, bool SF, bool HM, bool PLAIN>
 __device__ __forceinline__ void body_uv_fused_staged(const DevView &d, int x0, int y0, int ilay, double gene,
                                                      double ramp, double ctim, double (*s_h)[TileGeom<Q>::LDX], UVstage<Q> *s_f,
-                                                     double (*s_hl)[TileGeom<Q>::HLDX]) {
+                                                     double (*s_hl)[TileGeom<Q>::HLDX], bool store_hp2 = true) {
     using G = TileGeom<Q>;
     const int tid = threadIdx.x;
     const int lx = tid & 63, wy = tid >> 6;
@@ -926,7 +1040,7 @@
             q0 = s_h[r][lx + 1]; qb = s_h[r][lx]; qa = s_h[r + 1][lx + 1]; qd = s_h[r + 1][lx];
         }
         const ShLds<Q, !FIRST_X> sh{s_f, s_hl, r + 1, lx + 1, d.ocrp, hs2};
-        uv_core<!FIRST_X, true, true, SF, HM, PLAIN>(c[q], d, ilay, gene, ramp, ctim, 0, io, q0, qb, qa, qd, sh, true, pre2[q], ZV);
+        uv_core<!FIRST_X, true, true, SF, HM, PLAIN>(c[q], d, ilay, gene, ramp, ctim, 0, io, q0, qb, qa, qd, sh, true, pre2[q], ZV, store_hp2);
     }
 }
 
@@ -1124,9 +1238,10 @@
     }
 }
 
-template <int Q, bool FIRST_X, bool PROD, bool ZV, bool SF, bool HM = false, bool PLAIN = false>
+template <int Q, bool FIRST_X, bool PROD, bool ZV, bool SF, bool HM = false, bool PLAIN = false, bool LEAN = false>
 __device__ __forceinline__ void uv_fused_workgroup(const DevView &d, double gene, double ramp, double ctim) {
     static_assert(PROD || !HM, "the history-from-Montgomery form exists for the staged (PROD) bodies only");
+    static_assert(!LEAN || (HM && PLAIN), "the lean form exists for the plain history-from-Montgomery sweep only");
     static_assert(!PLAIN || (PROD && !SF), "the plain form exists for the staged (PROD) bodies without the stress fold");
     using G = TileGeom<Q>;
     __shared__ double s_h[G::TY + 1][G::LDX];
@@ -1139,14 +1254,15 @@
     const int ilay = blockIdx.y + 1;
     const bool interior = x0 - 1 >= 2 && x0 + G::TX <= d.L - 2 && y0 - 1 >= 2 && y0 + G::TY <= d.M - 2
                           && y0 - 1 + d.joff >= 2 && y0 + G::TY + d.joff <= d.Mg - 2 && tile_regular(d, x0, y0, G::TY);
-    if (interior && PROD) body_uv_fused_staged<Q, FIRST_X, ZV, SF, HM, PLAIN>(d, x0, y0, ilay, gene, ramp, ctim, s_h, s_f, s_hl);
+    if (interior && PROD) body_uv_fused_staged<Q, FIRST_X, ZV, SF, HM, PLAIN>(d, x0, y0, ilay, gene, ramp, ctim, s_h, s_f, s_hl,
+                                                                              !(LEAN && uv_tile_deep(d, x0, y0, G::TY)));
     else if (interior) body_uv_fused<Q, FIRST_X, true, SF>(d, x0, y0, ilay, gene, ramp, ctim, s_h);
     else if (PROD) body_uv_fused_edge<Q, FIRST_X, SF, HM, PLAIN>(d, x0, y0, ilay, gene, ramp, ctim, s_h, s_f, s_hl);
     else body_uv_fused<Q, FIRST_X, false, SF>(d, x0, y0, ilay, gene, ramp, ctim, s_h);
 }
-template <int Q, bool FIRST_X, bool PROD, bool ZV = false, bool HM = false, bool PLAIN = false>
+template <int Q, bool FIRST_X, bool PROD, bool ZV = false, bool HM = false, bool PLAIN = false, bool LEAN = false>
 __global__ __launch_bounds__(TileGeom<Q>::BLOCK) void k_uv_fused(DevView d, double gene, double ramp, double ctim) {
-    uv_fused_workgroup<Q, FIRST_X, PROD, ZV, false, HM, PLAIN>(d, gene, ramp, ctim);
+    uv_fused_workgroup<Q, FIRST_X, PROD, ZV, false, HM, PLAIN, LEAN>(d, gene, ramp, ctim);
 }
 template <int Q, bool FIRST_X, bool PROD, bool ZV = false>
 __global__ __launch_bounds__(TileGeom<Q>::BLOCK) __attribute__((amdgpu_waves_per_eu(3))) void k_uv_fused_sf(DevView d, double gene, double ramp, double ctim) {
diff --git a/beom_amd/csrc/beom_plan.h b/beom_amd/csrc/beom_plan.h
--- a/beom_amd/csrc/beom_plan.h
+++ b/beom_amd/csrc/beom_plan.h
@@ -10,6 +10,8 @@
     bool fold_static_ok, visc_all_zero, mont_keep;
     bool fuse, fuse_uv, fold_stress, lean_d2h, lean_visc, mont_history, plain_sweeps, keep_diag;
     int mont_levels_valid;
+    bool lean_fluxes, flux_readers;
+    int flux_stale;
 };
 
 struct StepPlan {
@@ -17,7 +19,8 @@
     double ctim, ramp, gene;
     bool first3, upst, stress_fold, launch_stress, rebuild, leith, launch_visc, needs_arrays;
     struct Mont { bool fused, keep_visc, lean_d2h, zero_visc, plain; } mont;
-    struct Uv { bool fused_uv, first_x, prod, zv, hm, plain; } uv;
+    struct Uv { bool fused_uv, first_x, prod, zv, hm, plain, lean; } uv;
+    bool h_from_vel, flux_sync;
 };
 
 inline bool fuses_uv(const StepFacts &f) { return f.dense && f.fuse_uv; }
@@ -73,9 +76,16 @@
     p.uv.hm = f.mont_history && f.mont_keep && p.mont.fused && p.uv.fused_uv && p.gene != 0.0 && !p.stress_fold &&
               f.mont_levels_valid >= 3;
     p.needs_arrays = !p.uv.hm;
+    const bool lean_ok = p.uv.hm && p.uv.plain && !f.flux_readers;
+    p.uv.lean = f.lean_fluxes && lean_ok;
+    p.h_from_vel = f.flux_stale != 0 && lean_ok && f.flux_stale == (p.uv.first_x ? 1 : 2);
+    p.flux_sync = f.flux_stale != 0 && !p.h_from_vel;
     return p;
 }
 
 constexpr bool uv_form_exists(bool sf, bool prod, bool zv, bool hm, bool plain) { return !((zv || hm || plain) && !prod) && !(sf && (hm || plain)); }
+constexpr bool uv_lean_form_exists(bool sf, bool prod, bool zv, bool hm, bool plain, bool lean) {
+    return uv_form_exists(sf, prod, zv, hm, plain) && (!lean || (hm && plain));
+}
 
 }
```

Result: slower. 20.68 billion (-2.0%).
